# synnada-ai/datafusion-upstream

Hardware: AMD Instinct MI355X
Metric: rows/sec hash-join+agg, TPC-H SF100 Q3 (higher is better)
Workload: dtype int64; 1 GPU; TPC-H SF100 Q3 (3-way hash join + group-by SUM + sort), int64 keys, Decimal128(15,2) money, resident in HBM; input_rows=765043119, parallelism=1 GPU

## Files before the change

datafusion-upstream_amd/capi.py:

```python
from __future__ import annotations

import ctypes as C
import os

_HERE = os.path.dirname(os.path.abspath(__file__))
LIB_PATH = os.path.join(_HERE, "libdfgpu.so")

BOOL, INT8, INT16, INT32, INT64, UINT8, UINT16, UINT32, UINT64 = 1, 2, 3, 4, 5, 6, 7, 8, 9
FLOAT32, FLOAT64, DATE32, DECIMAL128, UTF8, DICTIONARY = 10, 11, 12, 13, 14, 15
OP_ADD, OP_SUB, OP_MUL, OP_DIV, OP_REM = 0, 1, 2, 3, 4
OP_EQ, OP_NEQ, OP_LT, OP_LTEQ, OP_GT, OP_GTEQ, OP_DISTINCT, OP_NOT_DISTINCT = 10, 11, 12, 13, 14, 15, 16, 17
OP_AND, OP_OR = 20, 21
JOIN_INNER, JOIN_LEFT, JOIN_RIGHT, JOIN_FULL, JOIN_LEFT_SEMI, JOIN_RIGHT_SEMI, JOIN_LEFT_ANTI, JOIN_RIGHT_ANTI = range(8)
AGG_SUM, AGG_AVG, AGG_COUNT, AGG_MIN, AGG_MAX = range(5)

STATUS_NAMES = {0: "Ok", 1: "Execution", 2: "Internal", 3: "ResourcesExhausted", 4: "NotImplemented", 5: "InvalidArgument"}


class DfgpuError(RuntimeError):

    def __init__(self, status: int, message: str):
        self.status = status
        self.kind = STATUS_NAMES.get(status, str(status))
        super().__init__(f"{self.kind} error: {message}")
# ... 67 lines not shown
    "dfgpu_array_import_arrow": (C.c_int32, [_P, C.POINTER(ArrowArray), C.POINTER(ArrowSchema), _PP]),
    "dfgpu_array_export_arrow": (C.c_int32, [_P, _P, C.POINTER(ArrowArray), C.POINTER(ArrowSchema)]),
    "dfgpu_array_retain": (None, [_P]),
    "dfgpu_array_release": (None, [_P]),
    "dfgpu_array_is_identity": (C.c_int32, [_P]),
    "dfgpu_array_length": (C.c_int64, [_P]),
    "dfgpu_array_null_count": (C.c_int64, [_P, _P]),
    "dfgpu_array_slice": (C.c_int32, [_P, _P, C.c_int64, C.c_int64, _PP]),
    "dfgpu_concat": (C.c_int32, [_P, _PP, C.c_int32, _PP]),
    "dfgpu_list_from_counts": (C.c_int32, [_P, _P, _P, _PP]),
    "dfgpu_list_flatten": (C.c_int32, [_P, _P, C.c_int32, C.c_int32, C.c_int32, _PP, _PP]),
    "dfgpu_array_new_null": (C.c_int32, [_P, C.c_int32, C.c_int32, C.c_int32, C.c_int64, _PP]),
    "dfgpu_array_new_zeros": (C.c_int32, [_P, C.c_int32, C.c_int32, C.c_int32, C.c_int64, _PP]),
    "dfgpu_array_make_dictionary": (C.c_int32, [_P, _P, _P, _PP]),
    "dfgpu_hash_columns": (C.c_int32, [_P, _PP, C.c_int32, C.c_uint64, _PP]),
    "dfgpu_take": (C.c_int32, [_P, _P, _P, _PP]),
    "dfgpu_filter": (C.c_int32, [_P, _P, _P, _PP]),
    "dfgpu_mask_to_indices": (C.c_int32, [_P, _P, _PP]),
    "dfgpu_binary": (C.c_int32, [_P, C.c_int32, _P, C.c_int32, _P, C.c_int32, _PP]),
    "dfgpu_binary_fused2": (C.c_int32, [_P, C.c_int32, _P, C.c_int32, _P, _P, C.c_int32, C.c_int32, _PP]),
    "dfgpu_not": (C.c_int32, [_P, _P, _PP]),
    "dfgpu_is_null": (C.c_int32, [_P, _P, C.c_int32, _PP]),
    "dfgpu_negative": (C.c_int32, [_P, _P, _PP]),
    "dfgpu_cast": (C.c_int32, [_P, _P, C.c_int32, C.c_int32, C.c_int32, _PP]),
    "dfgpu_in_list": (C.c_int32, [_P, _P, _P, C.c_int32, _PP]),
    "dfgpu_join_build": (C.c_int32, [_P, _PP, C.c_int32, _P, C.c_int32, _PP]),
    "dfgpu_join_table_free": (None, [_P]),
    "dfgpu_join_table_num_rows": (C.c_int64, [_P]),
    "dfgpu_join_table_memory": (C.c_int64, [_P]),
    "dfgpu_join_probe": (C.c_int32, [_P, _P, _PP, C.c_int32, _P, _PP, _PP]),
    "dfgpu_join_probe_deferred": (C.c_int32, [_P, _P, _PP, C.c_int32, _P, _PP, _PP]),
    "dfgpu_join_lookup": (C.c_int32, [_P, _P, _PP, C.c_int32, _P, _PP]),
    "dfgpu_join_probe_selection": (C.c_int32, [_P, _P, _PP, C.c_int32, _P, _PP]),
    "dfgpu_join_mark_visited": (C.c_int32, [_P, _P, _P]),
    "dfgpu_join_adjust_indices": (C.c_int32, [_P, _P, _P, C.c_int64, C.c_int64, C.c_int32, _PP, _PP]),
    "dfgpu_join_final_indices": (C.c_int32, [_P, _P, C.c_int32, _PP]),
    "dfgpu_groups_new": (C.c_int32, [_P, C.c_int32, _PP]),
    "dfgpu_groups_free": (None, [_P]),
    "dfgpu_groups_intern": (C.c_int32, [_P, _P, _PP, C.c_int32, _P, _PP]),
    "dfgpu_groups_intern_deferred": (C.c_int32, [_P, _P, _PP, C.c_int32, _P, _PP]),
    "dfgpu_groups_len": (C.c_int64, [_P]),
    "dfgpu_groups_size": (C.c_int64, [_P]),
    "dfgpu_groups_emit": (C.c_int32, [_P, _P, _PP]),
    "dfgpu_groups_emit_deferred": (C.c_int32, [_P, _P, _PP, _PP]),
    "dfgpu_acc_new": (C.c_int32, [_P, C.c_int32, C.c_int32, C.c_int32, C.c_int32, _PP]),
    "dfgpu_acc_free": (None, [_P]),
    "dfgpu_acc_update_batch": (C.c_int32, [_P, _P, _P, _P, _P, C.c_int64]),
    "dfgpu_acc_update_batch_multi": (C.c_int32, [_P, _PP, _PP, _PP, C.c_int32, _P, C.c_int64]),
    "dfgpu_acc_merge_batch": (C.c_int32, [_P, _P, _PP, C.c_int32, _P, _P, C.c_int64]),
    "dfgpu_acc_evaluate": (C.c_int32, [_P, _P, _PP]),
    "dfgpu_acc_state": (C.c_int32, [_P, _P, _PP, C.POINTER(C.c_int32)]),
    "dfgpu_acc_size": (C.c_int64, [_P]),
    "dfgpu_acc_emit_first": (C.c_int32, [_P, _P, C.c_int64, C.c_int32, _PP, C.POINTER(C.c_int32)]),
    "dfgpu_groups_emit_first": (C.c_int32, [_P, _P, C.c_int64, _PP]),
    "dfgpu_array_iota": (C.c_int32, [_P, C.c_int64, _PP]),
    "dfgpu_cross_join_indices": (C.c_int32, [_P, C.c_int64, C.c_int64, C.c_int64, C.c_int32, _PP, _PP]),
    "dfgpu_sort_to_indices": (C.c_int32, [_P, _PP, C.c_char_p, C.c_char_p, C.c_int32, C.c_int64, _PP]),
    "dfgpu_sort_to_indices_keys": (C.c_int32, [_P, _PP, C.c_char_p, C.c_char_p, C.c_int32, C.c_int64, _PP, _PP]),
    "dfgpu_hash_partition": (C.c_int32, [_P, _PP, C.c_int32, C.c_int32, _PP, C.POINTER(C.c_int64)]),
    "dfgpu_comm_unique_id": (C.c_int32, [C.c_char_p]),
    "dfgpu_comm_create_rccl": (C.c_int32, [_P, C.c_char_p, C.c_int32, C.c_int32, _PP]),
    "dfgpu_comm_create_custom": (C.c_int32, [_P, _PP]),
    "dfgpu_comm_free": (None, [_P]),
    "dfgpu_comm_rank": (C.c_int32, [_P]),
    "dfgpu_comm_world": (C.c_int32, [_P]),
    "dfgpu_exchange": (C.c_int32, [_P, _P, _PP, C.c_int32, _PP, C.c_int32, _P, _PP, C.POINTER(C.c_int64)]),
# ... 95 lines not shown
```

datafusion-upstream_amd/csrc/core.hip:

```cpp
#include "device_utils.h"
#include <mutex>

namespace dfgpu {

void fail(dfgpu_status code, const char* fmt, ...) {
  char buf[1024]; va_list ap; va_start(ap, fmt); vsnprintf(buf, sizeof buf, fmt, ap); va_end(ap);
  throw Error(code, buf);
}

struct CtxRefs { std::atomic<int64_t> n{1}; };
static std::mutex g_mu;
static std::vector<std::pair<dfgpu_ctx*, CtxRefs*>> g_ctx;
static CtxRefs* refs_of(dfgpu_ctx* c) { std::lock_guard<std::mutex> l(g_mu); for (auto& p : g_ctx) if (p.first == c) return p.second; return nullptr; }
static void ctx_unref(dfgpu_ctx* c) {
  CtxRefs* r = refs_of(c);
  if (!r || r->n.fetch_sub(1) != 1) return;
  { std::lock_guard<std::mutex> l(g_mu); for (size_t i = 0; i < g_ctx.size(); i++) if (g_ctx[i].first == c) { g_ctx.erase(g_ctx.begin() + i); break; } }
  (void)hipSetDevice(c->device);
  (void)hipStreamSynchronize(c->stream);
  if (c->free_blocks) { for (auto& b : *c->free_blocks) (void)hipFree(b.second); delete c->free_blocks; }
  delete c->alloc_mu;
  if (c->d_flags) (void)hipFree(c->d_flags);
  if (c->d_scratch64) (void)hipFree(c->d_scratch64);
  if (c->h_pinned) (void)hipHostFree(c->h_pinned);
// ... 316 lines not shown
}
__global__ void __launch_bounds__(BLOCK) k_slist_walk(const int32_t* loff, const uint8_t* lbytes, int64_t n, const uint32_t* vstart, uint32_t* cnt, uint32_t* lens, uint32_t* spos, uint32_t* row_of, uint32_t* flags) {
  const int64_t i = (int64_t)blockIdx.x * BLOCK + threadIdx.x; if (i >= n) return;
  int64_t at = loff[i]; const int64_t end = loff[i + 1]; uint32_t k = 0;
  while (at < end) {
    if (at + 4 > end) { atomicOr(flags, DFGPU_FLAG_OOB); break; }
    const uint32_t len = (uint32_t)lbytes[at] | ((uint32_t)lbytes[at + 1] << 8) | ((uint32_t)lbytes[at + 2] << 16) | ((uint32_t)lbytes[at + 3] << 24);
    if (at + 4 + (int64_t)len > end) { atomicOr(flags, DFGPU_FLAG_OOB); break; }
    if (lens) { const uint32_t v = vstart[i] + k; lens[v] = len; spos[v] = (uint32_t)(at + 4); row_of[v] = (uint32_t)i; }
    k++; at += 4 + (int64_t)len;
  }
  if (cnt) cnt[i] = k;
}
__global__ void __launch_bounds__(BLOCK) k_slist_copy(const uint8_t* lbytes, const uint32_t* spos, const int32_t* voff, int64_t nv, uint8_t* out) {
  const int64_t j = (int64_t)blockIdx.x * BLOCK + threadIdx.x; if (j >= nv) return;
  const uint32_t len = (uint32_t)(voff[j + 1] - voff[j]); const uint8_t* src = lbytes + spos[j]; uint8_t* o = out + voff[j];
  for (uint32_t b = 0; b < len; b++) o[b] = src[b];
}

struct CtxOption { const char* name; int64_t (*get)(const dfgpu_ctx*); void (*set)(dfgpu_ctx*, int64_t); };
#define OPT_GET(M) [](const dfgpu_ctx* c) -> int64_t { return (int64_t)c->M; }
#define OPT_BOOL(M) OPT_GET(M), [](dfgpu_ctx* c, int64_t v) { c->M = v != 0; }
#define OPT_INT(M) OPT_GET(M), [](dfgpu_ctx* c, int64_t v) { c->M = v; }
#define OPT_MIN(M, LO) OPT_GET(M), [](dfgpu_ctx* c, int64_t v) { c->M = v < LO ? LO : v; }
#define OPT_RANGE(M, LO, HI) OPT_GET(M), [](dfgpu_ctx* c, int64_t v) { if (v < LO || v > HI) fail(DFGPU_INVALID_ARGUMENT, #M ": " #LO " .. " #HI); c->M = v; }
#define OPT_READ(M) OPT_GET(M), nullptr
static const CtxOption kCtxOptions[] = {
  { "force_hash_collisions", OPT_BOOL(force_hash_collisions) },
  { "first_seen_group_order", OPT_BOOL(first_seen_group_order) },
  { "join_rank_index", OPT_BOOL(join_rank_index) },
  { "join_rank_index_unsorted", OPT_BOOL(join_rank_index_unsorted) },
  { "join_lazy_build_rows", OPT_BOOL(join_lazy_build_rows) },
  { "join_selection_output", OPT_BOOL(join_selection_output) },
  { "join_key_packing", OPT_BOOL(join_key_packing) },
  { "join_swap_small_semi", OPT_BOOL(join_swap_small_semi) },
  { "join_partitioned", OPT_BOOL(join_partitioned) },
  { "join_partitioned_min_build", OPT_INT(join_partitioned_min_build) },
  { "join_partitioned_min_probe", OPT_INT(join_partitioned_min_probe) },
  { "join_partitioned_big", OPT_BOOL(join_partitioned_big) },
  { "join_partitioned_hashed", OPT_BOOL(join_partitioned_hashed) },
  { "join_partitioned_hash_mask", [](const dfgpu_ctx* c) -> int64_t { return c->join_partitioned_hash_mask == ~0ull ? 0 : (int64_t)c->join_partitioned_hash_mask; },
                                  [](dfgpu_ctx* c, int64_t v) { c->join_partitioned_hash_mask = v <= 0 ? ~0ull : (uint64_t)v; } },
  { "join_partition_rows", OPT_INT(join_partition_rows) },
  { "group_run_detection", OPT_BOOL(group_run_detection) },
  { "group_lazy_keys", OPT_BOOL(group_lazy_keys) },
  { "group_dictionary_canon", OPT_BOOL(group_dictionary_canon) },
  { "fused_aggregate_min_rows", OPT_INT(fused_aggregate_min_rows) },
  { "agg_order_inverse_map", OPT_BOOL(agg_order_inverse_map) },
  { "agg_partitioned", OPT_BOOL(agg_partitioned) },
  { "agg_partitioned_force", OPT_BOOL(agg_partitioned_force) },
  { "agg_partitioned_min_rows", OPT_INT(agg_partitioned_min_rows) },
  { "agg_pack_estimate_min_rows", OPT_INT(agg_pack_estimate_min_rows) },
  { "agg_preaggregate_distinct", OPT_READ(pa_last_distinct) },
  { "agg_spill_state_bytes", OPT_INT(agg_spill_state_bytes) },
  { "agg_spill_ranges", OPT_RANGE(agg_spill_ranges, 1, 4096) },
  { "sort_packed_keys", OPT_BOOL(sort_packed_keys) },
  { "sort_packed_min_rows", OPT_MIN(sort_packed_min_rows, 2) },
  { "sort_estimate_ranges", OPT_BOOL(sort_estimate_ranges) },
  { "sort_topk_words_min_rows", OPT_MIN(sort_topk_words_min_rows, 2) },
  { "sort_one_block_max_rows", OPT_MIN(sort_one_block_max_rows, 0) },
  { "sort_onesweep_min_rows", OPT_MIN(sort_onesweep_min_rows, 2) },
  { "sort_onesweep_rows", OPT_GET(sort_onesweep_rows), [](dfgpu_ctx* c, int64_t v) { c->sort_onesweep_rows = v == 16 ? 16 : v > 0 ? 8 : 0; } },
  { "sort_onesweep_fused_finish", OPT_BOOL(sort_onesweep_fused_finish) },
  { "sort_fused_small_passes", OPT_BOOL(sort_fused_small_passes) },
  { "sort_spill_bytes", OPT_INT(sort_spill_bytes) },
  { "sort_spill_ranges", OPT_RANGE(sort_spill_ranges, 1, 4096) },
// ... 423 lines not shown
```

datafusion-upstream_amd/csrc/dfgpu_internal.h:

```cpp
#pragma once
#include <hip/hip_runtime.h>
#include <atomic>
#include <cstdarg>
#include <cstdint>
#include <cstdio>
#include <cstring>
#include <memory>
#include <mutex>
#include <stdexcept>
#include <string>
#include <vector>
#include "../../include/dfgpu.h"

namespace dfgpu {

struct Error : std::exception {
  dfgpu_status code; std::string msg;
  Error(dfgpu_status c, std::string m) : code(c), msg(std::move(m)) {}
  const char* what() const noexcept override { return msg.c_str(); }
};
[[noreturn]] void fail(dfgpu_status code, const char* fmt, ...);

#define HIP_CHECK(expr)                                                                         \
  do { hipError_t e_ = (expr);                                                                  \
    if (e_ != hipSuccess) ::dfgpu::fail(e_ == hipErrorOutOfMemory ? DFGPU_RESOURCES_EXHAUSTED : DFGPU_INTERNAL, \
                                        "%s failed: %s (%s:%d)", #expr, hipGetErrorString(e_), __FILE__, __LINE__); } while (0)
#define KERNEL_CHECK() HIP_CHECK(hipGetLastError())

}

enum : uint32_t { DFGPU_FLAG_DIV_ZERO = 1, DFGPU_FLAG_OVERFLOW = 2, DFGPU_FLAG_CAST = 4, DFGPU_FLAG_OOB = 8, DFGPU_FLAG_TABLE_FULL = 16, DFGPU_FLAG_STALLED = 32 };

namespace dfgpu { struct Buffer; }
struct dfgpu_ctx {
  int device = 0;
  hipStream_t stream = nullptr;
  bool own_stream = false;
  hipStream_t copy_stream = nullptr;
  std::string err;
  bool force_hash_collisions = false;
  bool first_seen_group_order = true;
  bool join_rank_index = true;
  bool join_lazy_build_rows = true;
  bool join_selection_output = true;
  bool join_rank_index_unsorted = true;
  bool join_key_packing = true;
  bool group_run_detection = true;
  bool group_lazy_keys = true;
  bool group_dictionary_canon = true;
  bool join_swap_small_semi = true;
  uint64_t join_partitioned_hash_mask = ~0ull;
  bool join_partitioned_hashed = true;
  bool join_partitioned_big = true;
  bool join_partitioned = true; int64_t join_partitioned_min_build = 1 << 20, join_partitioned_min_probe = 1 << 22, join_partition_rows = 14000;
  int64_t fused_aggregate_min_rows = 1 << 20;
  bool sort_packed_keys = true;
  bool agg_partitioned = true, agg_partitioned_force = false; int64_t agg_partitioned_min_rows = 1 << 22;
  bool agg_order_inverse_map = true;
  int64_t agg_pack_estimate_min_rows = 1 << 22;
  bool pa_last_distinct = false;
  const void* pa_sample_key = nullptr; const void* pa_sample_mask = nullptr; int64_t pa_sample_n = 0; uint64_t pa_sample[3] = {0, 0, 0};
  std::shared_ptr<dfgpu::Buffer> pa_pack; int pa_pack_n = 0; int64_t pa_pack_min[4] = {0, 0, 0, 0}; uint64_t pa_pack_stride[4] = {0, 0, 0, 0}, pa_pack_range[4] = {0, 0, 0, 0}; bool pa_pack_nullable[4] = {false, false, false, false};
  std::shared_ptr<dfgpu::Buffer> row_selection; int64_t row_selection_len = 0;
  int defer_flag_checks = 0; bool flags_pending = false; std::string flags_what;
  uint32_t* d_flags = nullptr;
  uint64_t* d_scratch64 = nullptr;
  uint64_t* h_pinned = nullptr;
  static constexpr int MAIL_SEQ = 384, MAIL_WORDS = 256, PINNED_WORDS = 512;
  bool mailbox_readback = true; uint64_t mail_seq = 0;
  int num_cus = 256;
  std::mutex* alloc_mu = nullptr;
  std::vector<std::pair<size_t, void*>>* free_blocks = nullptr;
  size_t cached_bytes = 0, live_bytes = 0;
  int64_t sort_packed_min_rows = 1 << 20;
  int64_t sort_topk_words_min_rows = 1 << 23;
  int64_t sort_one_block_max_rows = 8192;
  int64_t sort_onesweep_min_rows = 1 << 20;
// ... 164 lines not shown
```

datafusion-upstream_amd/csrc/exec/exec.cpp:

```cpp
#include "../../../include/dfgpu_exec.h"

#include <algorithm>
#include <cstdarg>
#include <cstdio>
#include <cstring>
#include <memory>
#include <mutex>
#include <atomic>
#include <deque>
#include <map>
#include <tuple>
#include <set>
#include <stdexcept>
#include <string>
#include <vector>

namespace dfx {

struct Err : std::exception {
  dfgpu_status code; std::string msg;
  Err(dfgpu_status c, std::string m) : code(c), msg(std::move(m)) {}
  const char* what() const noexcept override { return msg.c_str(); }
};
[[noreturn]] static void fail(dfgpu_status code, const char* fmt, ...) {
// ... 52 lines not shown
  }
};
struct Col {
  ArrayRef arr, source; std::vector<ArrayRef> chain; MemoPtr memo; std::shared_ptr<LazyLookup> lookup;
  int64_t len() const { return arr ? arr.len() : !chain.empty() ? chain.back().len() : lookup ? lookup->m : 0; }
};
static const ArrayRef& col_indices(const TaskContext& tc, Col& c) {
  while (c.chain.size() > 1) {
    ArrayRef outer = std::move(c.chain.back()); c.chain.pop_back();
    ArrayRef& inner = c.chain.back();
    if (c.memo) {
      auto key = std::make_pair((const dfgpu_array*)inner.a, (const dfgpu_array*)outer.a);
      auto it = c.memo->composed.find(key);
      if (it == c.memo->composed.end()) it = c.memo->composed.emplace(key, Composed{inner, outer, take(tc, inner, outer)}).first;
      inner = it->second.out;
    } else inner = take(tc, inner, outer);
  }
  if (c.lookup) { ArrayRef b = c.lookup->resolve(tc, c.chain.empty() ? ArrayRef() : c.chain[0]); c.chain.clear(); c.chain.push_back(b); c.lookup.reset(); }
  return c.chain[0];
}
static const ArrayRef& col_get(const TaskContext& tc, Col& c) {
  if (!c.arr) { c.arr = take(tc, c.source, col_indices(tc, c)); c.source = ArrayRef(); c.chain.clear(); c.memo.reset(); }
  return c.arr;
}
static Col col_take(const Col& c, const ArrayRef& idx, const MemoPtr& memo = nullptr) {
  if (dfgpu_array_is_identity(idx.a) && idx.len() == c.len()) return c;
  Col o; o.memo = memo;
  if (c.arr) { o.source = c.arr; o.chain.push_back(idx); return o; }
  o.source = c.source; o.chain = c.chain; o.lookup = c.lookup; o.chain.push_back(idx);
  return o;
}
static Col col_of(ArrayRef a) { Col c; c.arr = std::move(a); return c; }

struct Batch {
  SchemaPtr schema; std::vector<Col> cols; ArrayRef selection; int64_t base_rows = 0;
  const ArrayRef& column(const TaskContext& tc, int i) {
    Col& c = cols.at((size_t)i);
    if (!c.arr && c.source && !c.chain.empty() && base_rows <= ((int64_t)1 << 20) && base_rows > 0) {
      std::vector<size_t> sib;
      for (size_t k = 0; k < cols.size(); k++) { const Col& o = cols[k]; if (k == (size_t)i || o.arr || !o.source || o.lookup.get() != c.lookup.get() || o.chain.size() != c.chain.size()) continue;
        bool same = true; for (size_t q = 0; q < c.chain.size(); q++) same = same && o.chain[q].a == c.chain[q].a; if (same) sib.push_back(k); }
      if (!sib.empty()) {
        const ArrayRef idx = col_indices(tc, c);
        std::vector<const dfgpu_array*> vals{ c.source.a }; for (size_t k : sib) vals.push_back(cols[k].source.a);
        std::vector<dfgpu_array*> outs(vals.size(), nullptr);
        tc.check(dfgpu_take_multi(tc.ctx, vals.data(), (int32_t)vals.size(), idx.a, outs.data()));
        auto settle = [](Col& x, dfgpu_array* a) { x.arr = ArrayRef::adopt(a); x.source = ArrayRef(); x.chain.clear(); x.memo.reset(); x.lookup.reset(); };
        settle(c, outs[0]); for (size_t u = 0; u < sib.size(); u++) settle(cols[sib[u]], outs[u + 1]);
        return c.arr;
      }
    }
    return col_get(tc, c);
  }
};
static ArrayRef mask_indices(const TaskContext& tc, const ArrayRef& mask) { dfgpu_array* o = nullptr; tc.check(dfgpu_mask_to_indices(tc.ctx, mask.a, &o)); return ArrayRef::adopt(o); }
static Batch materialize(const TaskContext& tc, const Batch& b) {
  if (!b.selection) return b;
  ArrayRef sel = mask_indices(tc, b.selection);
  Batch o; o.schema = b.schema; o.base_rows = sel.len();
  MemoPtr memo = std::make_shared<TakeMemo>(); for (auto& c : b.cols) o.cols.push_back(col_take(c, sel, memo));
  return o;
}
static int64_t num_rows(const TaskContext& tc, const Batch& b) { return b.selection ? mask_indices(tc, b.selection).len() : b.base_rows; }
static ArrayRef concat_arrays(const TaskContext& tc, std::vector<ArrayRef>& parts) {
  std::vector<const dfgpu_array*> p; for (auto& x : parts) p.push_back(x.a);
  dfgpu_array* o = nullptr; tc.check(dfgpu_concat(tc.ctx, p.data(), (int32_t)p.size(), &o)); return ArrayRef::adopt(o);
}
static bool concat_batches(const TaskContext& tc, std::vector<Batch>& in, Batch* out) {
  std::vector<Batch> m;
  for (auto& b : in) { Batch x = materialize(tc, b); if (x.base_rows > 0) m.push_back(std::move(x)); }
  if (m.empty()) { if (in.empty()) return false; *out = materialize(tc, in[0]); return true; }
  if (m.size() == 1) { *out = std::move(m[0]); return true; }
  Batch o; o.schema = m[0].schema;
  for (size_t c = 0; c < m[0].cols.size(); c++) {
    std::vector<ArrayRef> parts; for (auto& b : m) parts.push_back(col_get(tc, b.cols[c]));
    o.cols.push_back(col_of(concat_arrays(tc, parts)));
  }
  for (auto& b : m) o.base_rows += b.base_rows;
  *out = std::move(o); return true;
}

struct Value { ArrayRef arr; bool scalar = false; };
struct Expr {
  virtual ~Expr() = default;
  virtual Value eval(const TaskContext& tc, Batch& b) const = 0;
  virtual bool safe() const { return false; }
  virtual void columns(std::set<int>& out) const {}
  virtual int column_index() const { return -1; }
};
using ExprPtr = std::shared_ptr<const Expr>;

static ArrayRef into_array(const TaskContext& tc, const Value& v, int64_t n) {
  if (!v.scalar) return v.arr;
  dfgpu_array* idx = nullptr; tc.check(dfgpu_array_new_zeros(tc.ctx, DFGPU_UINT32, 0, 0, n, &idx));
  ArrayRef i = ArrayRef::adopt(idx);
  return take(tc, v.arr, i);
// ... 70 lines not shown
};

struct Stream { virtual ~Stream() = default; virtual bool next(Batch& out) = 0; };
struct Plan;
using PlanPtr = std::shared_ptr<const Plan>;
struct Metrics {
  std::mutex mu; int64_t output_rows = 0, output_batches = 0;
  int64_t spill_count = 0, spilled_bytes = 0, spilled_rows = 0;
  struct Open { dfgpu_ctx* c; int64_t id; int which; };
  std::vector<Open> open; int64_t ns[4] = {0, 0, 0, 0};
  void resolve() {
    std::lock_guard<std::mutex> l(mu);
    for (auto& o : open) { int64_t t = 0; if (dfgpu_span_elapsed_ns(o.c, o.id, &t) == DFGPU_OK) ns[o.which] += t; }
    open.clear();
  }
  ~Metrics() { resolve(); }
};
struct SpanGuard {
  dfgpu_ctx* c = nullptr; int64_t id = -1; Metrics* m = nullptr; int which = 0;
  SpanGuard(const TaskContext& tc, Metrics* met, int w) { if (tc.metrics && met && dfgpu_span_begin(tc.ctx, &id) == DFGPU_OK) { c = tc.ctx; m = met; which = w; } else id = -1; }
  ~SpanGuard() { if (id >= 0) { dfgpu_span_end(c, id); std::lock_guard<std::mutex> l(m->mu); m->open.push_back(Metrics::Open{c, id, which}); } }
};
struct Plan : std::enable_shared_from_this<Plan> {
  virtual ~Plan() = default;
  mutable std::shared_ptr<Metrics> met = std::make_shared<Metrics>();
  virtual std::vector<std::shared_ptr<const Plan>> children() const { return {}; }
  std::unique_ptr<Stream> run(int partition, const TaskContext& tc) const;
  virtual const char* name() const = 0;
  virtual SchemaPtr schema() const = 0;
  virtual int partitions() const = 0;
  virtual std::unique_ptr<Stream> execute(int partition, const TaskContext& tc) const = 0;
  virtual PlanPtr fresh() const = 0;
};
static int64_t metric_rows(const TaskContext& tc, const Batch& b) { if (!b.selection) return b.base_rows; int64_t k = 0; tc.check(dfgpu_mask_count(tc.ctx, b.selection.a, &k)); return k; }
struct MeteredStream : Stream {
  const Plan* op; PlanPtr keep; std::unique_ptr<Stream> in; TaskContext tc;
  MeteredStream(PlanPtr k, std::unique_ptr<Stream> i, TaskContext t) : op(k.get()), keep(std::move(k)), in(std::move(i)), tc(t) {}
  bool next(Batch& out) override {
    bool ok; { SpanGuard sp(tc, op->met.get(), 0); ok = in->next(out); }
    if (ok) { int64_t r = metric_rows(tc, out); std::lock_guard<std::mutex> l(op->met->mu); op->met->output_rows += r; op->met->output_batches++; }
    return ok;
  }
};
std::unique_ptr<Stream> Plan::run(int partition, const TaskContext& tc) const {
  if (!tc.metrics) return execute(partition, tc);
  std::unique_ptr<Stream> s; { SpanGuard sp(tc, met.get(), 0); s = execute(partition, tc); }
  return std::unique_ptr<Stream>(new MeteredStream(shared_from_this(), std::move(s), tc));
}
static void drain(const PlanPtr& p, int partition, const TaskContext& tc, std::vector<Batch>& out) {
  auto s = p->run(partition, tc); Batch b; while (s->next(b)) out.push_back(std::move(b));
}

struct VecStream : Stream {
  std::vector<Batch> v; size_t i = 0;
  explicit VecStream(std::vector<Batch> x) : v(std::move(x)) {}
  bool next(Batch& out) override { if (i >= v.size()) return false; out = std::move(v[i++]); return true; }
};

struct MemoryExec : Plan {
  mutable std::mutex mu; mutable std::vector<std::vector<Batch>> parts; SchemaPtr sch;
  const char* name() const override { return "MemoryExec"; }
  PlanPtr fresh() const override { return shared_from_this(); }
  SchemaPtr schema() const override { return sch; }
  int partitions() const override { std::lock_guard<std::mutex> l(mu); return (int)parts.size(); }
  std::unique_ptr<Stream> execute(int p, const TaskContext&) const override {
    std::lock_guard<std::mutex> l(mu);
    if (p < 0 || p >= (int)parts.size()) fail(DFGPU_INTERNAL, "MemoryExec invalid partition %d (expected less than %zu)", p, parts.size());
// ... 47 lines not shown
    for (int64_t i = 0; i < len; i++) { const uint8_t c = bytes[i]; if (escape > 0 && c == (uint8_t)escape && inside && i + 1 < len) { i++; continue; } if (c == (uint8_t)quote) inside = !inside; else if (c == '\n' && !inside && i + 1 >= next && i + 1 < len) { cuts.push_back(i + 1); next = i + 1 + batch_bytes; } }
    cuts.push_back(len);
  }
  struct S : Stream {
    const CsvExec* op; TaskContext tc; int next_piece, end_piece;
    S(const CsvExec* o, TaskContext t, int a, int b) : op(o), tc(t), next_piece(a), end_piece(b) {}
    bool next(Batch& out) override {
      if (next_piece >= end_piece) return false;
      const int i = next_piece++; std::vector<dfgpu_array*> cols(op->proj.size(), nullptr); int64_t rows = 0;
      tc.check(dfgpu_csv_read(tc.ctx, op->bytes + op->cuts[(size_t)i], op->cuts[(size_t)i + 1] - op->cuts[(size_t)i], 0, op->delim, op->quote, op->escape, i == 0 && op->header ? 1 : 0, op->ncols_file,
                              op->proj.data(), op->types.data(), (int32_t)op->proj.size(), cols.data(), &rows));
      Batch b; b.schema = op->sch; b.base_rows = rows;
      for (auto* a : cols) b.cols.push_back(col_of(ArrayRef::adopt(a)));
      out = std::move(b); return true;
    }
  };
  std::unique_ptr<Stream> execute(int p, const TaskContext& tc) const override {
    if (p < 0 || p >= nparts) fail(DFGPU_INTERNAL, "CsvExec invalid partition %d (expected less than %d)", p, nparts);
    const int64_t P = (int64_t)cuts.size() - 1;
    return std::unique_ptr<Stream>(new S(this, tc, (int)(P * p / nparts), (int)(P * (p + 1) / nparts)));
  }
};

static ArrayRef known_mask(const TaskContext& tc, const ArrayRef& m) {
  dfgpu_array_desc d; dfgpu_array_describe(m.a, &d);
  if (!d.validity) return m;
  dfgpu_array *nn = nullptr, *o = nullptr;
  tc.check(dfgpu_is_null(tc.ctx, m.a, 1, &nn)); ArrayRef n1 = ArrayRef::adopt(nn);
  tc.check(dfgpu_binary(tc.ctx, DFGPU_OP_AND, m.a, 0, n1.a, 0, &o)); return ArrayRef::adopt(o);
}

struct FilterExec : Plan {
  ExprPtr pred; PlanPtr input;
  PlanPtr fresh() const override { auto f = std::make_shared<FilterExec>(); f->pred = pred; f->input = input->fresh(); return f; }
  std::vector<std::shared_ptr<const Plan>> children() const override { return {input}; }
  const char* name() const override { return "FilterExec"; }
  SchemaPtr schema() const override { return input->schema(); }
  int partitions() const override { return input->partitions(); }
  struct S : Stream {
    const FilterExec* op; std::unique_ptr<Stream> in; TaskContext tc;
    S(const FilterExec* o, std::unique_ptr<Stream> i, TaskContext t) : op(o), in(std::move(i)), tc(t) {}
    bool next(Batch& out) override {
      Batch b; if (!in->next(b)) return false;
      if (b.selection && !op->pred->safe()) b = materialize(tc, b);
      Value v = op->pred->eval(tc, b);
      ArrayRef mask = into_array(tc, v, b.base_rows);
      dfgpu_array_desc d; dfgpu_array_describe(mask.a, &d);
      if (d.type != DFGPU_BOOL) fail(DFGPU_INTERNAL, "Cannot create filter_array from non-boolean predicates");
      if (b.selection) { ArrayRef km = known_mask(tc, mask); dfgpu_array* o = nullptr; tc.check(dfgpu_binary(tc.ctx, DFGPU_OP_AND, km.a, 0, b.selection.a, 0, &o)); mask = ArrayRef::adopt(o); }
      b.selection = mask; out = std::move(b); return true;
    }
  };
  std::unique_ptr<Stream> execute(int p, const TaskContext& tc) const override { return std::unique_ptr<Stream>(new S(this, input->run(p, tc), tc)); }
};

static Batch materialize_subset(const TaskContext& tc, Batch& b, const std::set<int>& needed) {
  ArrayRef sel = mask_indices(tc, b.selection);
  Batch o; o.schema = b.schema; o.base_rows = sel.len();
  ArrayRef filler; MemoPtr memo = std::make_shared<TakeMemo>();
  for (size_t i = 0; i < b.cols.size(); i++) {
    if (needed.count((int)i)) o.cols.push_back(col_take(b.cols[i], sel, memo));
    else { if (!filler) { dfgpu_array* f = nullptr; tc.check(dfgpu_array_new_null(tc.ctx, DFGPU_INT8, 0, 0, o.base_rows, &f)); filler = ArrayRef::adopt(f); } o.cols.push_back(col_of(filler)); }
  }
  return o;
}

struct ProjectionExec : Plan {
  std::vector<ExprPtr> exprs; std::vector<std::string> names; PlanPtr input; mutable SchemaPtr sch; mutable std::mutex mu;
  PlanPtr fresh() const override { auto p = std::make_shared<ProjectionExec>(); p->exprs = exprs; p->names = names; p->input = input->fresh(); return p; }
  std::vector<std::shared_ptr<const Plan>> children() const override { return {input}; }
  const char* name() const override { return "ProjectionExec"; }
  SchemaPtr schema() const override {
    std::lock_guard<std::mutex> l(mu);
    if (!sch) { auto s = std::make_shared<Schema>(); auto in = input->schema();
      for (size_t i = 0; i < exprs.size(); i++) { int ci = exprs[i]->column_index(); Field f = (ci >= 0 && in && ci < (int)in->f.size()) ? in->f[(size_t)ci] : Field{}; f.name = names[i]; s->f.push_back(f); }
      sch = s; }
    return sch;
  }
  int partitions() const override { return input->partitions(); }
  struct RowSel { dfgpu_ctx* c = nullptr; ~RowSel() { if (c) dfgpu_ctx_set_row_selection(c, nullptr); } };
  bool only_columns() const { bool oc = true; for (auto& e : exprs) oc &= e->column_index() >= 0; return oc; }
  Batch project(const TaskContext& tc, Batch b, std::vector<bool>* defer = nullptr) const {
    RowSel rowsel;
    if (b.selection && !only_columns() && !defer) {
      int64_t kept = 0; tc.check(dfgpu_mask_count(tc.ctx, b.selection.a, &kept));
      if (kept * 4 >= b.base_rows) { tc.check(dfgpu_ctx_set_row_selection(tc.ctx, b.selection.a)); rowsel.c = tc.ctx; }
      else { std::set<int> need; for (auto& e : exprs) e->columns(need); b = materialize_subset(tc, b, need); if (defer) defer->assign(exprs.size(), false); defer = nullptr; }
    }
    Batch o; o.base_rows = b.base_rows; o.selection = b.selection; auto s = std::make_shared<Schema>();
    if (defer) defer->assign(exprs.size(), false);
    for (size_t i = 0; i < exprs.size(); i++) {
      int ci = exprs[i]->column_index();
      if (ci >= 0) {
        if (ci >= (int)b.cols.size()) fail(DFGPU_INTERNAL, "PhysicalExpr Column references column at index %d but input schema only has %zu columns", ci, b.cols.size());
        o.cols.push_back(b.cols[(size_t)ci]); Field f = b.schema->f[(size_t)ci]; f.name = names[i]; s->f.push_back(f);
      } else if (defer) { (*defer)[i] = true; o.cols.push_back(Col()); s->f.push_back(Field{names[i]}); }
      else { ArrayRef a = into_array(tc, exprs[i]->eval(tc, b), b.base_rows); s->f.push_back(field_of(names[i], a.a)); o.cols.push_back(col_of(a)); }
    }
    o.schema = s; if (!defer) { std::lock_guard<std::mutex> l(mu); sch = s; }
    return o;
  }
  void evaluate_deferred(const TaskContext& tc, Batch& raw, Batch& projected, size_t i) const {
    RowSel rowsel;
    if (raw.selection) { tc.check(dfgpu_ctx_set_row_selection(tc.ctx, raw.selection.a)); rowsel.c = tc.ctx; }
    ArrayRef a = into_array(tc, exprs[i]->eval(tc, raw), raw.base_rows);
    projected.schema->f[i] = field_of(names[i], a.a); projected.cols[i] = col_of(a);
  }
  struct S : Stream {
    const ProjectionExec* op; std::unique_ptr<Stream> in; TaskContext tc;
    S(const ProjectionExec* o, std::unique_ptr<Stream> i, TaskContext t) : op(o), in(std::move(i)), tc(t) {}
    bool next(Batch& out) override {
      Batch b; if (!in->next(b)) return false;
      out = op->project(tc, std::move(b)); return true;
    }
  };
  std::unique_ptr<Stream> execute(int p, const TaskContext& tc) const override { return std::unique_ptr<Stream>(new S(this, input->run(p, tc), tc)); }
};

struct CoalesceBatchesExec : Plan {
  PlanPtr input; int64_t target;
  PlanPtr fresh() const override { auto c = std::make_shared<CoalesceBatchesExec>(); c->input = input->fresh(); c->target = target; return c; }
  std::vector<std::shared_ptr<const Plan>> children() const override { return {input}; }
  const char* name() const override { return "CoalesceBatchesExec"; }
  SchemaPtr schema() const override { return input->schema(); }
  int partitions() const override { return input->partitions(); }
  struct S : Stream {
    const CoalesceBatchesExec* op; std::unique_ptr<Stream> in; TaskContext tc; std::vector<Batch> buf; int64_t rows = 0; bool done = false;
    S(const CoalesceBatchesExec* o, std::unique_ptr<Stream> i, TaskContext t) : op(o), in(std::move(i)), tc(t) {}
    bool flush(Batch& out) { bool ok = concat_batches(tc, buf, &out); buf.clear(); rows = 0; return ok; }
    bool next(Batch& out) override {
      while (!done) {
        Batch b; if (!in->next(b)) { done = true; break; }
        if (b.selection) { if (b.base_rows >= op->target) { out = std::move(b); return true; } b = materialize(tc, b); }
        if (b.base_rows == 0) continue;
        if (b.base_rows >= op->target && buf.empty()) { out = std::move(b); return true; }
        rows += b.base_rows; buf.push_back(std::move(b));
        if (rows >= op->target) return flush(out);
      }
      if (!buf.empty()) return flush(out);
      return false;
    }
  };
  std::unique_ptr<Stream> execute(int p, const TaskContext& tc) const override { return std::unique_ptr<Stream>(new S(this, input->run(p, tc), tc)); }
};

struct CoalescePartitionsExec : Plan {
  PlanPtr input;
  PlanPtr fresh() const override { auto c = std::make_shared<CoalescePartitionsExec>(); c->input = input->fresh(); return c; }
  std::vector<std::shared_ptr<const Plan>> children() const override { return {input}; }
  const char* name() const override { return "CoalescePartitionsExec"; }
  SchemaPtr schema() const override { return input->schema(); }
  int partitions() const override { return 1; }
  std::unique_ptr<Stream> execute(int, const TaskContext& tc) const override {
    std::vector<Batch> all; for (int p = 0; p < input->partitions(); p++) drain(input, p, tc, all);
    return std::unique_ptr<Stream>(new VecStream(std::move(all)));
  }
};

static void partition_batch(const TaskContext& tc, Batch& b, const std::vector<ExprPtr>& exprs, int n, std::vector<std::vector<Batch>>& outs) {
  if (b.base_rows == 0) return;
  bool safe_keys = true; for (auto& e : exprs) safe_keys &= e->safe();
  if (n <= 256 && (!b.selection || safe_keys)) {
    Batch kb = b; kb.selection = ArrayRef();
    std::vector<ArrayRef> keys; std::vector<const dfgpu_array*> kp;
    for (auto& e : exprs) { keys.push_back(into_array(tc, e->eval(tc, kb), kb.base_rows)); kp.push_back(keys.back().a); }
    std::vector<const dfgpu_array*> cp; for (auto& c : b.cols) cp.push_back(c.arr ? c.arr.a : nullptr);
    std::vector<dfgpu_array*> oc(b.cols.size(), nullptr); std::vector<int64_t> counts((size_t)n); dfgpu_array* idx = nullptr;
    tc.check(dfgpu_partition_columns(tc.ctx, kp.data(), (int32_t)kp.size(), n, cp.data(), (int32_t)cp.size(), b.selection.a, oc.data(), &idx, counts.data()));
    ArrayRef indices = ArrayRef::adopt(idx); std::vector<ArrayRef> moved; for (auto* x : oc) moved.push_back(ArrayRef::adopt(x));
    int64_t off = 0;
    for (int d = 0; d < n; d++) {
      const int64_t cnt = counts[(size_t)d];
      if (cnt) {
        auto slice = [&](const ArrayRef& a) { dfgpu_array* s = nullptr; tc.check(dfgpu_array_slice(tc.ctx, a.a, off, cnt, &s)); return ArrayRef::adopt(s); };
        ArrayRef rows;
        Batch o; o.schema = b.schema; o.base_rows = cnt; MemoPtr memo = std::make_shared<TakeMemo>();
        for (size_t c = 0; c < b.cols.size(); c++) {
          if (moved[c]) o.cols.push_back(col_of(slice(moved[c])));
          else { if (!rows) rows = slice(indices); o.cols.push_back(col_take(b.cols[c], rows, memo)); }
        }
        outs[(size_t)d].push_back(std::move(o));
      }
      off += cnt;
    }
    return;
  }
  ArrayRef sel; Batch kb = b;
  if (b.selection) { std::set<int> need; for (auto& e : exprs) e->columns(need); sel = mask_indices(tc, b.selection); kb = materialize_subset(tc, b, need); }
  if (kb.base_rows == 0) return;
  std::vector<ArrayRef> keys; std::vector<const dfgpu_array*> kp;
  for (auto& e : exprs) { keys.push_back(into_array(tc, e->eval(tc, kb), kb.base_rows)); kp.push_back(keys.back().a); }
  std::vector<int64_t> counts((size_t)n); dfgpu_array* idx = nullptr;
  tc.check(dfgpu_hash_partition(tc.ctx, kp.data(), (int32_t)kp.size(), n, &idx, counts.data()));
  ArrayRef indices = ArrayRef::adopt(idx); int64_t off = 0;
  for (int d = 0; d < n; d++) {
    if (counts[(size_t)d]) {
      dfgpu_array* s = nullptr; tc.check(dfgpu_array_slice(tc.ctx, indices.a, off, counts[(size_t)d], &s)); ArrayRef part = ArrayRef::adopt(s);
      ArrayRef rows = sel ? take(tc, sel, part) : part;
      Batch o; o.schema = b.schema; o.base_rows = counts[(size_t)d];
      MemoPtr memo = std::make_shared<TakeMemo>(); for (auto& c : b.cols) o.cols.push_back(col_take(c, rows, memo));
      outs[(size_t)d].push_back(std::move(o));
    }
    off += counts[(size_t)d];
  }
}

struct RepartitionExec : Plan {
  PlanPtr input; std::vector<ExprPtr> exprs; int n;
  mutable std::mutex mu; mutable bool ran = false; mutable std::vector<std::vector<Batch>> outs;
  PlanPtr fresh() const override { auto r = std::make_shared<RepartitionExec>(); r->input = input->fresh(); r->exprs = exprs; r->n = n; return r; }
  std::vector<std::shared_ptr<const Plan>> children() const override { return {input}; }
  const char* name() const override { return "RepartitionExec"; }
  SchemaPtr schema() const override { return input->schema(); }
  int partitions() const override { return n; }
  std::unique_ptr<Stream> execute(int p, const TaskContext& tc) const override {
    std::lock_guard<std::mutex> l(mu);
    if (!ran) {
      outs.assign((size_t)n, {});
      for (int ip = 0; ip < input->partitions(); ip++) {
        std::vector<Batch> in; drain(input, ip, tc, in);
        int rr = 0;
// ... 7 lines not shown
    if (p < 0 || p >= n) fail(DFGPU_INTERNAL, "RepartitionExec invalid partition %d", p);
    return std::unique_ptr<Stream>(new VecStream(outs[(size_t)p]));
  }
};

struct JoinTableRef { dfgpu_join_table* t = nullptr; ~JoinTableRef() { if (t) dfgpu_join_table_free(t); } };
struct BuildSide { Batch batch; std::shared_ptr<JoinTableRef> table; std::vector<int64_t> segments; bool empty = true; };

struct HashJoinExec : Plan {
  PlanPtr left, right; std::vector<ExprPtr> on_l, on_r; ExprPtr filter; std::vector<int> f_side, f_index;
  int join_type, mode; bool null_equals_null; bool swap_small_right = true;
  mutable bool selection_consumer = false;
  mutable std::mutex mu; mutable std::shared_ptr<BuildSide> shared;
  PlanPtr fresh() const override {
    auto j = std::make_shared<HashJoinExec>(); j->left = left->fresh(); j->right = right->fresh(); j->on_l = on_l; j->on_r = on_r; j->filter = filter; j->f_side = f_side; j->f_index = f_index;
    j->join_type = join_type; j->mode = mode; j->null_equals_null = null_equals_null; j->swap_small_right = swap_small_right; j->selection_consumer = selection_consumer; return j;
  }
  std::vector<std::shared_ptr<const Plan>> children() const override { return {left, right}; }
  const char* name() const override { return "HashJoinExec"; }
  bool swap_allowed(const TaskContext& tc) const { int64_t v = 1; dfgpu_ctx_get_option(tc.ctx, "join_swap_small_semi", &v); return swap_small_right && v != 0; }
  bool left_only() const { return join_type == DFGPU_JOIN_LEFT_SEMI || join_type == DFGPU_JOIN_LEFT_ANTI; }
  bool right_only() const { return join_type == DFGPU_JOIN_RIGHT_SEMI || join_type == DFGPU_JOIN_RIGHT_ANTI; }
  SchemaPtr schema() const override {
    auto s = std::make_shared<Schema>(); auto l = left->schema(), r = right->schema();
    if (!right_only() && l) s->f.insert(s->f.end(), l->f.begin(), l->f.end());
    if (!left_only() && r) s->f.insert(s->f.end(), r->f.begin(), r->f.end());
    return s;
  }
  int partitions() const override { return right->partitions(); }
  std::shared_ptr<BuildSide> collect_left(int partition, const TaskContext& tc, ArrayRef* fused) const {
    auto bs = std::make_shared<BuildSide>();
    std::vector<Batch> in;
    if (partition < 0) { for (int p = 0; p < left->partitions(); p++) drain(left, p, tc, in); } else drain(left, partition, tc, in);
    if (in.size() == 1 && in[0].selection) { bs->batch = in[0]; *fused = in[0].selection; bs->batch.selection = ArrayRef(); bs->segments = { bs->batch.base_rows }; bs->empty = false; }
    else {
      std::vector<Batch> m; for (auto& b : in) { Batch x = materialize(tc, b); if (x.base_rows) { bs->segments.push_back(x.base_rows); m.push_back(std::move(x)); } }
      if (m.empty()) return bs;
      concat_batches(tc, m, &bs->batch); bs->empty = false;
    }
    return bs;
  }
  void build_table(const std::shared_ptr<BuildSide>& bs, const ArrayRef& fused, const TaskContext& tc) const {
    if (bs->empty) return;
    std::vector<ArrayRef> keys; std::vector<const dfgpu_array*> kp;
    for (auto& e : on_l) { keys.push_back(into_array(tc, e->eval(tc, bs->batch), bs->batch.base_rows)); kp.push_back(keys.back().a); }
    bs->table = std::make_shared<JoinTableRef>();
    tc.check(dfgpu_join_build(tc.ctx, kp.data(), (int32_t)kp.size(), fused.a, null_equals_null ? 1 : 0, &bs->table->t));
  }
  std::shared_ptr<BuildSide> collect_build(int partition, const TaskContext& tc) const {
    SpanGuard sp(tc, met.get(), 1);
    ArrayRef fused; auto bs = collect_left(partition, tc, &fused); build_table(bs, fused, tc); return bs;
  }
  struct S : Stream {
    const HashJoinExec* op; TaskContext tc; int partition; std::unique_ptr<Stream> probe; std::shared_ptr<BuildSide> bs; Batch swapped; int state = 0;
    Batch chunk_pb; ArrayRef chunk_b, chunk_p; int64_t chunk_k = -1, chunk_total = 0, chunk_joined = -1; std::vector<uint32_t> chunk_last;
    SchemaPtr out_schema;
    bool lazy_build_rows = true, selection_output = true;
    S(const HashJoinExec* o, int p, TaskContext t) : op(o), tc(t), partition(p) { int64_t v = 1; if (dfgpu_ctx_get_option(tc.ctx, "join_lazy_build_rows", &v) == DFGPU_OK) lazy_build_rows = v != 0;
      v = 1; if (dfgpu_ctx_get_option(tc.ctx, "join_selection_output", &v) == DFGPU_OK) selection_output = v != 0; }
    int64_t last_u32(const ArrayRef& a) {
      int64_t n = a.len(); if (!n) return -1;
      dfgpu_array* s1 = nullptr; tc.check(dfgpu_array_slice(tc.ctx, a.a, n - 1, 1, &s1)); ArrayRef one = ArrayRef::adopt(s1);
      uint32_t v = 0; tc.check(dfgpu_array_export_host(tc.ctx, one.a, &v, nullptr, nullptr)); return (int64_t)v;
    }
    void chunk_last_rows(const ArrayRef& pidx, int64_t bsz) {
      const int64_t m = pidx.len(); chunk_last.clear(); if (!m) return;
      std::vector<uint32_t> pos; for (int64_t e = bsz; ; e += bsz) { pos.push_back((uint32_t)((e < m ? e : m) - 1)); if (e >= m) break; }
// ... 54 lines not shown
      if (!op->right_only()) for (size_t i = 0; i < (lf ? lf->f.size() : 0); i++) {
        if (build && alias[i] >= 0) o.cols.push_back(col_take(probe_b.cols[(size_t)alias[i]], pidx, memo));
        else if (build && lazy) { Col c; c.source = build->cols[i].arr; c.lookup = lazy; c.memo = memo; o.cols.push_back(std::move(c)); }
        else if (build) o.cols.push_back(col_take(build->cols[i], bidx, memo));
        else { dfgpu_array* nn = nullptr; tc.check(dfgpu_array_new_null(tc.ctx, lf->f[i].type, lf->f[i].precision, lf->f[i].scale, o.base_rows, &nn)); o.cols.push_back(col_of(ArrayRef::adopt(nn))); }
      }
      if (!op->left_only()) for (auto& c : probe_b.cols) o.cols.push_back(col_take(c, pidx, memo));
      return o;
    }
    bool next(Batch& out) override {
      if (state == 0) {
        if (op->left_only() && op->swap_allowed(tc) && (op->mode != 0 || op->right->partitions() == 1)) {
          ArrayRef fused; bs = op->collect_left(op->mode == 0 ? -1 : partition, tc, &fused);
          std::vector<Batch> rin; drain(op->right, partition, tc, rin);
          Batch rb; bool have_right = concat_batches(tc, rin, &rb) && rb.base_rows > 0;
          out_schema = op->schema();
          if (!bs->empty && rb.base_rows * 8 <= bs->batch.base_rows) { swapped = semi_by_probing_left(fused, have_right ? &rb : nullptr); state = 4; }
          else { op->build_table(bs, fused, tc); std::vector<Batch> one; if (have_right) one.push_back(std::move(rb)); probe.reset(new VecStream(std::move(one))); state = 1; }
        }
        else if (op->mode == 0) { std::lock_guard<std::mutex> l(op->mu); if (!op->shared) op->shared = op->collect_build(-1, tc); bs = op->shared; }
        else bs = op->collect_build(partition, tc);
        if (state == 0) { probe = op->right->run(partition, tc); out_schema = op->schema(); state = 1; }
      }
      if (state == 4) { state = 3; if (swapped.base_rows == 0) return false; out = std::move(swapped); return true; }
      bool need_final = op->join_type == DFGPU_JOIN_LEFT || op->join_type == DFGPU_JOIN_FULL || op->left_only();
      if (need_final && op->mode == 0 && op->right->partitions() > 1 && state != 4)
        fail(DFGPU_NOT_IMPLEMENTED, "HashJoinExec mode=CollectLeft with %d probe partitions and a join type that emits build rows in a final pass; repartition both sides (Partitioned) or coalesce the probe side", op->right->partitions());
      while (state == 1) {
        if (chunk_k >= 0) { SpanGuard join_span(tc, op->met.get(), 2); emit_chunk(out, need_final); return true; }
        Batch pb; if (!probe->next(pb)) { state = 2; break; }
        if (pb.base_rows == 0) continue;
        SpanGuard join_span(tc, op->met.get(), 2);
        const bool chunked = pb.base_rows <= (tc.batch_size > 8192 ? tc.batch_size : 8192);
        if (chunked && pb.selection) { pb = materialize(tc, pb); if (pb.base_rows == 0) continue; }
        if (pb.selection && (op->join_type == DFGPU_JOIN_RIGHT || op->join_type == DFGPU_JOIN_FULL || op->right_only())) { pb = materialize(tc, pb); if (pb.base_rows == 0) continue; }
        ArrayRef mask = pb.selection; pb.selection = ArrayRef();
        ArrayRef bidx, pidx;
        if (bs->empty) { dfgpu_array *a = nullptr, *b = nullptr; dfgpu_array_desc d{}; d.type = DFGPU_UINT64; d.values = &d; tc.check(dfgpu_array_import_host(tc.ctx, &d, &a)); d.type = DFGPU_UINT32; tc.check(dfgpu_array_import_host(tc.ctx, &d, &b)); bidx = ArrayRef::adopt(a); pidx = ArrayRef::adopt(b); }
        else {
          std::vector<ArrayRef> keys; std::vector<const dfgpu_array*> kp;
          for (auto& e : op->on_r) { keys.push_back(into_array(tc, e->eval(tc, pb), pb.base_rows)); kp.push_back(keys.back().a); }
          dfgpu_array *b = nullptr, *p = nullptr;
          bool defer = !chunked && op->join_type == DFGPU_JOIN_INNER && !op->filter && !need_final && kp.size() == 1 && lazy_build_rows;
          if (defer && selection_output && op->selection_consumer) {
            std::vector<int> al = key_aliases(&bs->batch, pb); bool all = !al.empty(); for (int a : al) all = all && a >= 0;
            if (all) {
              dfgpu_array* s = nullptr; dfgpu_status st = dfgpu_join_probe_selection(tc.ctx, bs->table->t, kp.data(), 1, mask.a, &s);
              if (st == DFGPU_OK) {
                Batch o; o.schema = out_schema; o.base_rows = pb.base_rows; o.selection = ArrayRef::adopt(s);
                for (int a : al) o.cols.push_back(pb.cols[(size_t)a]);
                for (auto& c : pb.cols) o.cols.push_back(c);
                out = std::move(o); return true;
              }
              if (st != DFGPU_NOT_IMPLEMENTED) tc.check(st);
            }
          }
          for (auto& c : bs->batch.cols) defer = defer && (bool)c.arr;
          if (defer) {
            tc.check(dfgpu_join_probe_deferred(tc.ctx, bs->table->t, kp.data(), 1, mask.a, &b, &p)); pidx = ArrayRef::adopt(p);
            if (!b) {
              auto lz = std::make_shared<LazyLookup>(); lz->keep = bs; lz->table = bs->table->t; lz->probe_key = keys[0]; lz->rows = pidx; lz->m = pidx.len();
              bool wanted = false; { std::vector<int> al = key_aliases(&bs->batch, pb); for (int a : al) wanted |= a < 0; }
              if (!wanted || (dfgpu_array_is_identity(pidx.a) && pidx.len() == pb.base_rows)) { out = build_batch(&bs->batch, pb, ArrayRef(), pidx, lz); return true; }
              bidx = lz->resolve(tc, ArrayRef());
            } else bidx = ArrayRef::adopt(b);
          } else { tc.check(dfgpu_join_probe(tc.ctx, bs->table->t, kp.data(), (int32_t)kp.size(), mask.a, &b, &p)); bidx = ArrayRef::adopt(b); pidx = ArrayRef::adopt(p); }
          if (!chunked) { apply_filter(pb, bidx, pidx); if (need_final) tc.check(dfgpu_join_mark_visited(tc.ctx, bs->table->t, bidx.a)); }
        }
        if (chunked) {
          const int64_t bsz = tc.batch_size > 0 ? tc.batch_size : 8192, m = bidx.len();
          chunk_total = m == 0 ? 1 : (m + bsz - 1) / bsz;
          chunk_last_rows(pidx, bsz);
          if (m > 0 && m % bsz == 0 && (int64_t)chunk_last.back() != pb.base_rows - 1) chunk_total++;
          chunk_pb = std::move(pb); chunk_b = bidx; chunk_p = pidx; chunk_k = 0; chunk_joined = -1;
          continue;
        }
        int jt = op->join_type;
        if (jt == DFGPU_JOIN_RIGHT || jt == DFGPU_JOIN_FULL || op->right_only()) {
          dfgpu_array *b2 = nullptr, *p2 = nullptr;
          tc.check(dfgpu_join_adjust_indices(tc.ctx, bidx.a, pidx.a, 0, pb.base_rows, jt, &b2, &p2)); bidx = ArrayRef::adopt(b2); pidx = ArrayRef::adopt(p2);
        } else if (op->left_only()) continue;
        out = build_batch(bs->empty ? nullptr : &bs->batch, pb, bidx, pidx); return true;
      }
      if (state == 2) {
        state = 3;
        if (!need_final || bs->empty) return false;
        dfgpu_array* f = nullptr; tc.check(dfgpu_join_final_indices(tc.ctx, bs->table->t, op->join_type, &f)); ArrayRef fidx = ArrayRef::adopt(f);
        fidx = reference_final_order(fidx);
        Batch o; o.schema = out_schema; o.base_rows = fidx.len();
        MemoPtr memo = std::make_shared<TakeMemo>(); for (auto& c : bs->batch.cols) o.cols.push_back(col_take(c, fidx, memo));
        if (!op->left_only()) { auto rf = op->right->schema(); for (auto& fd : rf->f) { dfgpu_array* nn = nullptr; tc.check(dfgpu_array_new_null(tc.ctx, fd.type, fd.precision, fd.scale, o.base_rows, &nn)); o.cols.push_back(col_of(ArrayRef::adopt(nn))); } }
        out = std::move(o); return true;
      }
      return false;
    }
    Batch semi_by_probing_left(ArrayRef fused, Batch* right_rows) {
      Batch o; o.schema = out_schema;
      const bool have_right = right_rows != nullptr; Batch none; Batch& rb = have_right ? *right_rows : none;
      Batch& lb = bs->batch;
      const bool anti = op->join_type == DFGPU_JOIN_LEFT_ANTI;
      if (anti && fused) {
        Batch sel = lb; sel.selection = fused; lb = materialize(tc, sel); fused = ArrayRef(); bs->segments = { lb.base_rows };
      }
      ArrayRef lidx;
      if (!have_right) {
        if (!anti) return o;
        dfgpu_array *e0 = nullptr, *e1 = nullptr; dfgpu_array_desc d{}; d.type = DFGPU_UINT64; d.values = &d; tc.check(dfgpu_array_import_host(tc.ctx, &d, &e0)); ArrayRef b0 = ArrayRef::adopt(e0);
        d.type = DFGPU_UINT32; tc.check(dfgpu_array_import_host(tc.ctx, &d, &e1)); ArrayRef p0 = ArrayRef::adopt(e1);
        dfgpu_array *b2 = nullptr, *p2 = nullptr; tc.check(dfgpu_join_adjust_indices(tc.ctx, b0.a, p0.a, 0, lb.base_rows, DFGPU_JOIN_RIGHT_ANTI, &b2, &p2)); ArrayRef drop = ArrayRef::adopt(b2); lidx = ArrayRef::adopt(p2);
      } else {
        std::vector<ArrayRef> rk, lk; std::vector<const dfgpu_array*> rp, lp;
        for (auto& e : op->on_r) { rk.push_back(into_array(tc, e->eval(tc, rb), rb.base_rows)); rp.push_back(rk.back().a); }
        JoinTableRef table; tc.check(dfgpu_join_build(tc.ctx, rp.data(), (int32_t)rp.size(), nullptr, op->null_equals_null ? 1 : 0, &table.t));
        for (auto& e : op->on_l) { lk.push_back(into_array(tc, e->eval(tc, lb), lb.base_rows)); lp.push_back(lk.back().a); }
        dfgpu_array *b = nullptr, *p = nullptr;
        tc.check(dfgpu_join_probe(tc.ctx, table.t, lp.data(), (int32_t)lp.size(), fused.a, &b, &p)); ArrayRef ridx = ArrayRef::adopt(b); lidx = ArrayRef::adopt(p);
        if (op->filter && ridx.len()) {
          Batch inter; inter.schema = std::make_shared<Schema>(); inter.base_rows = ridx.len();
          for (size_t i = 0; i < op->f_side.size(); i++) {
            Col src = op->f_side[i] == 0 ? lb.cols.at((size_t)op->f_index[i]) : rb.cols.at((size_t)op->f_index[i]);
            Col t = col_take(src, op->f_side[i] == 0 ? lidx : ridx); inter.cols.push_back(col_of(col_get(tc, t))); inter.schema->f.push_back(Field{"x"});
          }
          ArrayRef m = into_array(tc, op->filter->eval(tc, inter), inter.base_rows);
          ArrayRef nr = filter_idx(ridx, m), nl = filter_idx(lidx, m); ridx = nr; lidx = nl;
        }
        dfgpu_array *b2 = nullptr, *p2 = nullptr;
        tc.check(dfgpu_join_adjust_indices(tc.ctx, ridx.a, lidx.a, 0, lb.base_rows, anti ? DFGPU_JOIN_RIGHT_ANTI : DFGPU_JOIN_RIGHT_SEMI, &b2, &p2));
        ArrayRef drop = ArrayRef::adopt(b2); lidx = ArrayRef::adopt(p2);
      }
      if (bs->segments.size() > 1 && lidx.len()) {
        dfgpu_array* w = nullptr; tc.check(dfgpu_cast(tc.ctx, lidx.a, DFGPU_UINT64, 0, 0, &w)); lidx = reference_final_order(ArrayRef::adopt(w));
      }
      o.base_rows = lidx.len();
      MemoPtr memo = std::make_shared<TakeMemo>(); for (auto& c : lb.cols) o.cols.push_back(col_take(c, lidx, memo));
      return o;
// ... 505 lines not shown
      if (aggs[i].kind == DFGPU_AGG_COUNT_DISTINCT) { cds[i].init(tc); continue; }
      int32_t t = aggs[i].kind == DFGPU_AGG_COUNT ? DFGPU_INT64 : aggs[i].type;
      tc.check(dfgpu_acc_new(tc.ctx, aggs[i].kind, t, aggs[i].precision, aggs[i].scale, &accs[i].a));
    }
    { int64_t lim = 0, ranges = 16; dfgpu_ctx_get_option(tc.ctx, "agg_spill_state_bytes", &lim); dfgpu_ctx_get_option(tc.ctx, "agg_spill_ranges", &ranges);
      if (lim > 0 && grouped && !specials && sets.empty()) { S.spill = std::make_shared<SpillState>(); S.spill->limit = lim; S.spill->ranges = ranges; } }
    if (order_mode != 0) preagg_min_rows = INT64_MAX;
    S.pj = pj; S.src = src; S.grouped = grouped; S.specials = specials; S.fuse_min_rows = fuse_min_rows; S.preagg_min_rows = preagg_min_rows;
    return SP;
  }
  void consume(AggState& S, Batch& b_in) const {
    const TaskContext& tc = S.tc; const ProjectionExec* pj = S.pj; const bool grouped = S.grouped, specials = S.specials; const int64_t fuse_min_rows = S.fuse_min_rows, preagg_min_rows = S.preagg_min_rows;
    GroupsRef& groups = S.groups; std::vector<AccRef>& accs = S.accs; std::vector<StringMinMax>& smm = S.smm; std::vector<CountDistinct>& cds = S.cds; ArrayRef& pending = S.pending;
    auto settle_pending = [&]() {
      if (!pending) return;
      const dfgpu_array* kp = pending.a; dfgpu_array* ids = nullptr; tc.check(dfgpu_groups_intern(tc.ctx, groups.g, &kp, 1, nullptr, &ids)); ArrayRef drop = ArrayRef::adopt(ids);
      if (dfgpu_groups_len(groups.g) != pending.len()) fail(DFGPU_INTERNAL, "AggregateExec: pre-aggregated keys were not distinct");
      pending = ArrayRef();
    };
    {
      if (b_in.base_rows == 0) return;
      if (S.spill && order_mode == 0 && mode != 0 && !pending && dfgpu_groups_len(groups.g) > 0 && state_bytes(S) > S.spill->limit) spill(S, *S.spill);
      settle_pending();
      Batch raw; std::vector<bool> deferred;
      if (pj) { raw = b_in; b_in = pj->project(tc, raw, &deferred); }
      Batch& b = b_in;
      bool any_deferred = false; for (bool d : deferred) any_deferred |= d;
      auto ensure = [&](int ci) { if (ci >= 0 && ci < (int)deferred.size() && deferred[(size_t)ci]) { pj->evaluate_deferred(tc, raw, b, (size_t)ci); deferred[(size_t)ci] = false; } };
      if (any_deferred) {
        std::set<int> need; for (auto& e : gexprs) e->columns(need); for (auto& a : aggs) if (a.filter) a.filter->columns(need);
        for (int ci : need) ensure(ci);
      }
      if (b.base_rows == 0) return;
      ArrayRef mask = b.selection; b.selection = ArrayRef();
      if (!sets.empty()) { if (specials) fail(DFGPU_NOT_IMPLEMENTED, "This feature is not implemented: COUNT(DISTINCT) / string MIN-MAX under grouping sets on the device"); for (size_t ci = 0; ci < deferred.size(); ci++) ensure((int)ci); group_aggregate_sets(tc, b, mask, groups, accs); return; }
      ArrayRef gids; int64_t total = 1;
      if (grouped) {
        std::vector<ArrayRef> gc; std::vector<const dfgpu_array*> gp;
        for (auto& e : gexprs) {
          int ci = e->column_index();
          if (ci >= 0 && ci < (int)b.cols.size() && !b.cols[(size_t)ci].arr && b.cols[(size_t)ci].source && b.cols[(size_t)ci].source.len() * 4 <= b.base_rows) {
            Col& c = b.cols[(size_t)ci]; dfgpu_array_desc sd; dfgpu_array_describe(c.source.a, &sd);
            if (sd.type != DFGPU_DICTIONARY) {
              dfgpu_array* d = nullptr; tc.check(dfgpu_array_make_dictionary(tc.ctx, col_indices(tc, c).a, c.source.a, &d));
              gc.push_back(ArrayRef::adopt(d)); gp.push_back(gc.back().a); continue;
            }
          }
          gc.push_back(into_array(tc, e->eval(tc, b), b.base_rows)); gp.push_back(gc.back().a);
        }
        if (!specials && !merging() && gp.size() >= 1 && gp.size() <= 4 && b.base_rows >= preagg_min_rows && preaggregate(tc, pj, raw, b, deferred, ensure, gp, mask, groups, accs, S.spill ? nullptr : &pending)) return;
        dfgpu_array* ids = nullptr; tc.check(specials || order_mode == 1 ? dfgpu_groups_intern(tc.ctx, groups.g, gp.data(), (int32_t)gp.size(), mask.a, &ids) : dfgpu_groups_intern_deferred(tc.ctx, groups.g, gp.data(), (int32_t)gp.size(), mask.a, &ids)); gids = ArrayRef::adopt(ids);
        total = dfgpu_groups_len(groups.g);
        if (order_mode == 1 && !specials) note_sort_prefix(S, gp, gids, mask);
      } else { dfgpu_array* z = nullptr; tc.check(dfgpu_array_new_zeros(tc.ctx, DFGPU_UINT32, 0, 0, b.base_rows, &z)); gids = ArrayRef::adopt(z); }
      if (!specials && !merging() && total <= 8 && fuse_min_rows >= 0 && b.base_rows >= fuse_min_rows && try_fused(tc, pj, raw, b, deferred, accs, gids, grouped ? ArrayRef() : mask, total)) return;
      for (size_t ci = 0; ci < deferred.size(); ci++) ensure((int)ci);
      size_t col = gexprs.size();
      std::vector<ArrayRef> uvals(aggs.size()), ufilt(aggs.size());
      for (size_t i = 0; i < aggs.size(); i++) {
        if (merging() && is_string_minmax(i)) {
          ArrayRef stv = b.column(tc, (int)col); col += 1;
          smm[i].update(tc, gids, stv, mask);
        } else if (merging() && aggs[i].kind == DFGPU_AGG_COUNT_DISTINCT) {
          ArrayRef stv = b.column(tc, (int)col); col += 1;
          cds[i].merge(tc, gids, stv, mask, total, aggs[i].type, aggs[i].precision, aggs[i].scale);
        } else if (merging()) {
          int nst = aggs[i].kind == DFGPU_AGG_AVG ? 2 : 1; const dfgpu_array* st[2];
// ... 436 lines not shown
struct dfgpu_stream { std::unique_ptr<Stream> s; PlanPtr keep; TaskContext tc; };

template <typename F> static dfgpu_status guard(F&& f) {
  try { f(); return DFGPU_OK; }
  catch (const Err& e) { g_err = e.msg; return e.code; }
  catch (const std::bad_alloc&) { g_err = "host allocation failed"; return DFGPU_RESOURCES_EXHAUSTED; }
  catch (const std::exception& e) { g_err = e.what(); return DFGPU_INTERNAL; }
}
static ExprPtr ex(const dfgpu_expr* e) { if (!e) fail(DFGPU_INVALID_ARGUMENT, "null expression"); return e->e; }
static PlanPtr pl(const dfgpu_plan* p) { if (!p) fail(DFGPU_INVALID_ARGUMENT, "null plan"); return p->p; }

extern "C" {

const char* dfgpu_exec_last_error(void) { return g_err.c_str(); }

dfgpu_status dfgpu_batch_new(const char* const* names, const dfgpu_array* const* columns, int32_t ncols, dfgpu_batch** out) {
  return guard([&] {
    if (ncols < 0 || !out) fail(DFGPU_INVALID_ARGUMENT, "batch_new: bad arguments");
    auto* b = new dfgpu_batch(); b->b.schema = std::make_shared<Schema>();
    for (int i = 0; i < ncols; i++) {
      if (!columns[i]) { delete b; fail(DFGPU_INVALID_ARGUMENT, "batch_new: null column"); }
      if (i && dfgpu_array_length(columns[i]) != dfgpu_array_length(columns[0])) { delete b; fail(DFGPU_INVALID_ARGUMENT, "batch_new: columns differ in length"); }
      b->b.cols.push_back(col_of(ArrayRef::share(columns[i]))); b->b.schema->f.push_back(field_of(names && names[i] ? names[i] : "", columns[i]));
    }
    b->b.base_rows = ncols ? dfgpu_array_length(columns[0]) : 0;
    *out = b;
  });
}
void dfgpu_batch_free(dfgpu_batch* b) { delete b; }
int32_t dfgpu_batch_num_columns(const dfgpu_batch* b) { return b ? (int32_t)b->b.cols.size() : 0; }
const char* dfgpu_batch_column_name(const dfgpu_batch* b, int32_t i) { return (b && i >= 0 && i < (int)b->b.schema->f.size()) ? b->b.schema->f[(size_t)i].name.c_str() : ""; }
dfgpu_status dfgpu_batch_num_rows(dfgpu_ctx* ctx, dfgpu_batch* b, int64_t* out) { return guard([&] { if (!ctx || !b || !out) fail(DFGPU_INVALID_ARGUMENT, "batch_num_rows: null argument"); TaskContext tc{ctx, 8192}; *out = num_rows(tc, b->b); }); }
static void materialize_all(const TaskContext& tc, Batch& b) {
  if (b.selection) b = materialize(tc, b);
  std::map<const dfgpu_array*, std::vector<size_t>> groups;
  for (size_t i = 0; i < b.cols.size(); i++) { Col& c = b.cols[i]; if (!c.arr && c.source && !c.chain.empty()) groups[col_indices(tc, c).a].push_back(i); }
  for (auto& g : groups) {
    if (g.second.size() < 2) continue;
    std::vector<const dfgpu_array*> vals; for (size_t i : g.second) vals.push_back(b.cols[i].source.a);
    std::vector<dfgpu_array*> outs(vals.size(), nullptr);
    ArrayRef idx = b.cols[g.second[0]].chain[0];
    tc.check(dfgpu_take_multi(tc.ctx, vals.data(), (int32_t)vals.size(), idx.a, outs.data()));
    for (size_t k = 0; k < g.second.size(); k++) { Col& c = b.cols[g.second[k]]; c.arr = ArrayRef::adopt(outs[k]); c.source = ArrayRef(); c.chain.clear(); c.memo.reset(); }
  }
  for (auto& c : b.cols) (void)col_get(tc, c);
}
dfgpu_status dfgpu_batch_materialize(dfgpu_ctx* ctx, dfgpu_batch* b) {
  return guard([&] { if (!ctx || !b) fail(DFGPU_INVALID_ARGUMENT, "batch_materialize: null argument"); TaskContext tc{ctx, 8192}; materialize_all(tc, b->b); });
}
dfgpu_status dfgpu_batch_column(dfgpu_ctx* ctx, dfgpu_batch* b, int32_t i, dfgpu_array** out) {
  return guard([&] {
    if (!ctx || !b || !out) fail(DFGPU_INVALID_ARGUMENT, "batch_column: null argument");
    TaskContext tc{ctx, 8192};
    if (b->b.selection) b->b = materialize(tc, b->b);
    const ArrayRef& a = b->b.column(tc, i); dfgpu_array_retain(a.a); *out = a.a;
  });
}

dfgpu_status dfgpu_expr_column(const char* name, int32_t index, dfgpu_expr** out) { return guard([&] { if (!out) fail(DFGPU_INVALID_ARGUMENT, "expr_column: null argument"); *out = new dfgpu_expr{std::make_shared<ColumnExpr>(name ? name : "", index)}; }); }
dfgpu_status dfgpu_expr_literal(const dfgpu_array* s, dfgpu_expr** out) {
  return guard([&] { if (!s || dfgpu_array_length(s) != 1) fail(DFGPU_INVALID_ARGUMENT, "literal must be a length-1 array"); *out = new dfgpu_expr{std::make_shared<LiteralExpr>(ArrayRef::share(s))}; });
}
dfgpu_status dfgpu_expr_binary(const dfgpu_expr* l, int32_t op, const dfgpu_expr* r, dfgpu_expr** out) { return guard([&] { *out = new dfgpu_expr{std::make_shared<BinaryExpr>(ex(l), op, ex(r))}; }); }
static dfgpu_status unary(const dfgpu_expr* e, int kind, int a0, int a1, int a2, const dfgpu_array* list, dfgpu_expr** out) {
  return guard([&] { auto u = std::make_shared<UnaryExpr>(); u->e = ex(e); u->kind = kind; u->a0 = a0; u->a1 = a1; u->a2 = a2; if (list) u->list = ArrayRef::share(list); *out = new dfgpu_expr{u}; });
}
dfgpu_status dfgpu_expr_not(const dfgpu_expr* e, dfgpu_expr** out) { return unary(e, 0, 0, 0, 0, nullptr, out); }
dfgpu_status dfgpu_expr_is_null(const dfgpu_expr* e, int32_t negated, dfgpu_expr** out) { return unary(e, negated ? 2 : 1, 0, 0, 0, nullptr, out); }
dfgpu_status dfgpu_expr_negative(const dfgpu_expr* e, dfgpu_expr** out) { return unary(e, 3, 0, 0, 0, nullptr, out); }
dfgpu_status dfgpu_expr_cast(const dfgpu_expr* e, int32_t t, int32_t p, int32_t s, dfgpu_expr** out) { return unary(e, 4, t, p, s, nullptr, out); }
dfgpu_status dfgpu_expr_in_list(const dfgpu_expr* e, const dfgpu_array* list, int32_t negated, dfgpu_expr** out) { return unary(e, negated ? 6 : 5, 0, 0, 0, list, out); }
void dfgpu_expr_free(dfgpu_expr* e) { delete e; }

dfgpu_status dfgpu_plan_memory(const dfgpu_batch* const* batches, const int32_t* sizes, int32_t nparts, dfgpu_plan** out) {
  return guard([&] {
    if (!out || nparts < 0 || (nparts > 0 && (!sizes || !batches))) fail(DFGPU_INVALID_ARGUMENT, "plan_memory: null argument");
    auto m = std::make_shared<MemoryExec>(); int k = 0;
    for (int p = 0; p < nparts; p++) { m->parts.emplace_back(); for (int i = 0; i < sizes[p]; i++) { const dfgpu_batch* b = batches[k++]; if (!b) fail(DFGPU_INVALID_ARGUMENT, "null batch"); if (!m->sch) m->sch = b->b.schema; m->parts.back().push_back(b->b); } }
    if (!m->sch) m->sch = std::make_shared<Schema>();
    *out = new dfgpu_plan{m};
  });
}
dfgpu_status dfgpu_plan_parquet(dfgpu_parquet* file, const int32_t* columns, int32_t ncols, int32_t npartitions, int32_t row_groups_per_batch, dfgpu_plan** out) {
  return guard([&] {
    if (!file || !out || (ncols > 0 && !columns) || npartitions < 1) fail(DFGPU_INVALID_ARGUMENT, "plan_parquet: bad argument");
    auto n = std::make_shared<ParquetExec>(); n->file = file; n->nparts = npartitions; n->per_batch = row_groups_per_batch > 0 ? row_groups_per_batch : 1; n->sch = std::make_shared<Schema>();
    for (int32_t i = 0; i < ncols; i++) {
// ... 14 lines not shown
    for (int32_t i = 0; i < ncols; i++) {
      const int32_t c = columns[i];
      if (c < 0 || c >= ncols_file || (i && c <= columns[i - 1])) fail(DFGPU_INVALID_ARGUMENT, "plan_csv: projected columns must be ascending file column indices");
      n->proj.push_back(c); n->types.insert(n->types.end(), {types[3 * c], types[3 * c + 1], types[3 * c + 2]});
      n->sch->f.push_back(Field{names[c] ? names[c] : "", types[3 * c], types[3 * c + 1], types[3 * c + 2]});
    }
    n->cut(batch_bytes > 0 ? batch_bytes : (int64_t)256 << 20);
    *out = new dfgpu_plan{n};
  });
}
dfgpu_status dfgpu_plan_parquet_prune(dfgpu_plan* p, int32_t column, int64_t min_value, int64_t max_value) {
  return guard([&] {
    auto* n = p ? dynamic_cast<const ParquetExec*>(p->p.get()) : nullptr;
    if (!n) fail(DFGPU_INVALID_ARGUMENT, "plan_parquet_prune: not a ParquetExec");
    std::lock_guard<std::mutex> l(n->mu); n->bounds.push_back(ParquetExec::Bound{column, min_value, max_value});
  });
}
int64_t dfgpu_plan_parquet_pruned(const dfgpu_plan* p) { auto* n = p ? dynamic_cast<const ParquetExec*>(p->p.get()) : nullptr; return n ? n->pruned.load() : -1; }
dfgpu_status dfgpu_plan_memory_replace(dfgpu_plan* p, const dfgpu_batch* const* batches, const int32_t* sizes, int32_t nparts) {
  return guard([&] {
    auto* m = p ? dynamic_cast<const MemoryExec*>(p->p.get()) : nullptr;
    if (!m) fail(DFGPU_INVALID_ARGUMENT, "plan_memory_replace: not a MemoryExec");
    std::vector<std::vector<Batch>> np; int k = 0;
    for (int i = 0; i < nparts; i++) { np.emplace_back(); for (int j = 0; j < sizes[i]; j++) { const dfgpu_batch* b = batches[k++]; if (!b) fail(DFGPU_INVALID_ARGUMENT, "null batch"); np.back().push_back(b->b); } }
    std::lock_guard<std::mutex> l(m->mu); m->parts = std::move(np);
  });
}
dfgpu_status dfgpu_plan_filter(const dfgpu_expr* pred, const dfgpu_plan* input, dfgpu_plan** out) { return guard([&] { auto f = std::make_shared<FilterExec>(); f->pred = ex(pred); f->input = pl(input); *out = new dfgpu_plan{f}; }); }
dfgpu_status dfgpu_plan_projection(const dfgpu_expr* const* exprs, const char* const* names, int32_t n, const dfgpu_plan* input, dfgpu_plan** out) {
  return guard([&] { auto p = std::make_shared<ProjectionExec>(); for (int i = 0; i < n; i++) { p->exprs.push_back(ex(exprs[i])); p->names.push_back(names[i] ? names[i] : ""); } p->input = pl(input); *out = new dfgpu_plan{p}; });
}
dfgpu_status dfgpu_plan_coalesce_batches(const dfgpu_plan* input, int64_t target, dfgpu_plan** out) { return guard([&] { auto c = std::make_shared<CoalesceBatchesExec>(); c->input = pl(input); c->target = target; *out = new dfgpu_plan{c}; }); }
dfgpu_status dfgpu_plan_coalesce_partitions(const dfgpu_plan* input, dfgpu_plan** out) { return guard([&] { auto c = std::make_shared<CoalescePartitionsExec>(); c->input = pl(input); *out = new dfgpu_plan{c}; }); }
static void mark_selection_consumer(const PlanPtr& p) {
  const Plan* q = p.get();
  while (q) {
    if (auto* hj = dynamic_cast<const HashJoinExec*>(q)) { hj->selection_consumer = true; return; }
    if (auto* cb = dynamic_cast<const CoalesceBatchesExec*>(q)) q = cb->input.get();
    else if (auto* pr = dynamic_cast<const ProjectionExec*>(q)) { if (!pr->only_columns()) return; q = pr->input.get(); }
    else return;
  }
}
dfgpu_status dfgpu_plan_repartition(const dfgpu_plan* input, const dfgpu_expr* const* exprs, int32_t nexprs, int32_t n, dfgpu_plan** out) {
  return guard([&] { if (n < 1) fail(DFGPU_INVALID_ARGUMENT, "repartition: partition count must be positive"); auto r = std::make_shared<RepartitionExec>(); r->input = pl(input); r->n = n; if (nexprs > 0) mark_selection_consumer(r->input); for (int i = 0; i < nexprs; i++) r->exprs.push_back(ex(exprs[i])); *out = new dfgpu_plan{r}; });
}
dfgpu_status dfgpu_plan_hash_join(const dfgpu_plan* left, const dfgpu_plan* right, const dfgpu_expr* const* on_left, const dfgpu_expr* const* on_right, int32_t non,
                                  const dfgpu_expr* filter, const int32_t* fs, const int32_t* fi, int32_t nf, int32_t join_type, int32_t mode, int32_t nen, dfgpu_plan** out) {
  return guard([&] {
    if (!left || !right || !out) fail(DFGPU_INVALID_ARGUMENT, "plan_hash_join: null argument");
    if (non < 1) fail(DFGPU_EXECUTION, "Plan error: On constraints in HashJoinExec should be non-empty");
    if (join_type < 0 || join_type > DFGPU_JOIN_RIGHT_ANTI) fail(DFGPU_INVALID_ARGUMENT, "unknown join type %d", join_type);
    auto j = std::make_shared<HashJoinExec>(); j->left = pl(left); j->right = pl(right);
    for (int i = 0; i < non; i++) { j->on_l.push_back(ex(on_left[i])); j->on_r.push_back(ex(on_right[i])); }
    if (filter) { j->filter = ex(filter); for (int i = 0; i < nf; i++) { j->f_side.push_back(fs[i]); j->f_index.push_back(fi[i]); } }
    j->join_type = join_type; j->mode = mode; j->null_equals_null = nen != 0;
    mark_selection_consumer(j->left); mark_selection_consumer(j->right);
    *out = new dfgpu_plan{j};
  });
}
dfgpu_status dfgpu_plan_sort_merge_join(const dfgpu_plan* left, const dfgpu_plan* right, const dfgpu_expr* const* on_left, const dfgpu_expr* const* on_right, int32_t non, const dfgpu_expr* filter,
                                        const int32_t* fs, const int32_t* fi, int32_t nf, int32_t join_type, int32_t null_equals_null, dfgpu_plan** out) {
  return guard([&] {
    if (!left || !right || !out) fail(DFGPU_INVALID_ARGUMENT, "plan_sort_merge_join: null argument");
    if (non < 1) fail(DFGPU_EXECUTION, "Plan error: On constraints in SortMergeJoinExec should be non-empty");
    if (join_type == DFGPU_JOIN_RIGHT_SEMI) fail(DFGPU_NOT_IMPLEMENTED, "This feature is not implemented: SortMergeJoinExec does not support JoinType::RightSemi");
    if (join_type < 0 || join_type > DFGPU_JOIN_RIGHT_ANTI) fail(DFGPU_NOT_IMPLEMENTED, "This feature is not implemented: SortMergeJoinExec join type %d on the device", join_type);
    if (filter && (join_type == DFGPU_JOIN_LEFT_SEMI || join_type == DFGPU_JOIN_LEFT_ANTI || join_type == DFGPU_JOIN_RIGHT_ANTI))
      fail(DFGPU_NOT_IMPLEMENTED, "This feature is not implemented: SortMergeJoinExec %s with a JoinFilter on the device (Inner, Left, Right and Full take one)", join_type == DFGPU_JOIN_LEFT_SEMI ? "LeftSemi" : join_type == DFGPU_JOIN_LEFT_ANTI ? "LeftAnti" : "RightAnti");
    if (filter && nf > 0 && (!fs || !fi)) fail(DFGPU_INVALID_ARGUMENT, "sort_merge_join: JoinFilter without column indices");
    auto j = std::make_shared<SortMergeJoinExec>(); j->left = pl(left); j->right = pl(right);
    if (filter) { j->filter = ex(filter); for (int i = 0; i < nf; i++) { j->f_side.push_back(fs[i]); j->f_index.push_back(fi[i]); } }
    for (int i = 0; i < non; i++) { j->on_l.push_back(ex(on_left[i])); j->on_r.push_back(ex(on_right[i])); }
    j->join_type = join_type; j->null_equals_null = null_equals_null != 0;
    *out = new dfgpu_plan{j};
  });
}
dfgpu_status dfgpu_plan_nested_loop_join(const dfgpu_plan* left, const dfgpu_plan* right, const dfgpu_expr* filter, const int32_t* fs, const int32_t* fi, int32_t nf, int32_t join_type, dfgpu_plan** out) {
  return guard([&] {
    if (join_type < 0 || join_type > DFGPU_JOIN_RIGHT_ANTI) fail(DFGPU_INVALID_ARGUMENT, "unknown join type %d", join_type);
    auto j = std::make_shared<NestedLoopJoinExec>(); j->left = pl(left); j->right = pl(right); j->join_type = join_type;
    if (filter) { j->filter = ex(filter); for (int i = 0; i < nf; i++) { j->f_side.push_back(fs[i]); j->f_index.push_back(fi[i]); } }
    *out = new dfgpu_plan{j};
  });
}
dfgpu_status dfgpu_plan_aggregate(int32_t mode, const dfgpu_expr* const* gexprs, const char* const* gnames, int32_t ng, const int32_t* kinds, const dfgpu_expr* const* args,
                                  const dfgpu_expr* const* filters, const char* const* names, const int32_t* types, int32_t na, const dfgpu_plan* input, dfgpu_plan** out) {
  return guard([&] {
    if (mode < 0 || mode > 4) fail(DFGPU_INVALID_ARGUMENT, "unknown AggregateMode %d", mode);
    auto a = std::make_shared<AggregateExec>(); a->mode = mode; a->input = pl(input);
// ... 136 lines not shown
```

datafusion-upstream_amd/csrc/join.hip:

```cpp
#include "join_table.h"

namespace dfgpu {
constexpr uint64_t SLOT_EMPTY = ~0ull;
constexpr uint32_t NO_SLOT = 0xFFFFFFFFu;
}
using namespace dfgpu;


namespace dfgpu {

__device__ inline bool row_selected(const uint64_t* mask, int64_t i) { return mask == nullptr || bit_get(mask, i); }

__global__ void __launch_bounds__(BLOCK) k_join_build(KeySet ks, int64_t n, const uint64_t* mask, int null_eq, int force_zero,
                                                      uint64_t* slots, uint32_t* slot_count, uint64_t cap_mask, uint32_t* row_slot,
                                                      unsigned long long* counters ) {
  int64_t i = (int64_t)blockIdx.x * BLOCK + threadIdx.x;
  if (i >= n) return;
  uint32_t my_slot = NO_SLOT;
  if (row_selected(mask, i)) {
    bool any_null; uint64_t h = keyset_hash(ks, i, 0, &any_null);
    if (force_zero) h = 0;
    if (!any_null || null_eq) {
      uint64_t tag = h >> 32, s = h & cap_mask, mine = (tag << 32) | (uint64_t)i;
      for (uint64_t step = 0; step <= cap_mask; step++) {
// ... 67 lines not shown
  for (int q = 0; q < HP_ROWS; q++) {
    bool hit = false;
    if (on[q]) {
      uint64_t c = cur[q], s2 = sl[q];
      if (c != SLOT_EMPTY && (c >> 32) == tag[q] && v0[q] == k0[q] && (NK == 1 || v1[q] == k1[q])) hit = true;
      else if (c != SLOT_EMPTY) {
        for (uint64_t step = 0; step < cap_mask; step++) {
          s2 = (s2 + 1) & cap_mask; c = slots[s2];
          if (c == SLOT_EMPTY) break;
          if ((c >> 32) == tag[q]) { uint64_t r = c & 0xFFFFFFFFull; if (b0[r] == k0[q] && (NK == 1 || b1[r] == k1[q])) { hit = true; break; } }
        }
      }
      if (hit) found_slot[base + (int64_t)q * BLOCK] = (uint32_t)s2;
    }
    int64_t i = base + (int64_t)q * BLOCK;
    uint64_t m = ballot64(hit);
    if (lane_id() == 0 && (i >> 6) < ((n + 63) >> 6)) match_bits[i >> 6] = m;
  }
}
__global__ void __launch_bounds__(BLOCK) k_probe_found(const uint32_t* rows, int64_t m, const uint32_t* found_slot, const uint64_t* slots, const uint32_t* slot_count, int unique,
                                                       uint64_t* out_build, uint32_t* out_slot, uint32_t* out_cnt) {
  int64_t i = (int64_t)blockIdx.x * BLOCK + threadIdx.x;
  if (i >= m) return;
  uint32_t s2 = found_slot[rows[i]];
  if (unique) out_build[i] = slots[s2] & 0xFFFFFFFFull;
  else { out_slot[i] = s2; out_cnt[i] = slot_count[s2]; }
}
constexpr int PM_ROWS = 8;
__device__ inline uint64_t spread32(uint64_t x) {
  x &= 0xFFFFFFFFull;
  x = (x | (x << 16)) & 0x0000FFFF0000FFFFull; x = (x | (x << 8)) & 0x00FF00FF00FF00FFull; x = (x | (x << 4)) & 0x0F0F0F0F0F0F0F0Full;
  x = (x | (x << 2)) & 0x3333333333333333ull; x = (x | (x << 1)) & 0x5555555555555555ull; return x;
}
template <typename T, bool HAS_MASK, bool HAS_VALID, bool FULL>
__device__ inline void probe_match_chunk(const T* keys, const uint64_t* key_valid, const uint64_t* mask, int64_t n, int64_t kmin, uint64_t range,
                                         const uint64_t* bitmap, uint64_t* match_bits, int64_t base, int lane) {
  T k[PM_ROWS / 2][2];
#pragma unroll
  for (int r = 0; r < PM_ROWS / 2; r++) {
    int64_t j = base + r * 2 * WAVE + 2 * lane;
    if (FULL || j + 1 < n) { struct alignas(2 * sizeof(T)) P { T a, b; }; P p = *(const P*)(keys + j); k[r][0] = p.a; k[r][1] = p.b; }
    else { k[r][0] = j < n ? keys[j] : (T)0; k[r][1] = 0; }
  }
  uint64_t mws[PM_ROWS / 2];
#pragma unroll
  for (int r = 0; r < PM_ROWS / 2; r++) { int64_t j = base + r * 2 * WAVE + 2 * lane; mws[r] = (HAS_MASK && (FULL || j < n)) ? mask[j >> 6] >> (j & 63) : 3ull; }
  uint64_t d0 = (uint64_t)((int64_t)k[0][0] - kmin);
  d0 = (uint64_t)__builtin_amdgcn_readfirstlane((uint32_t)d0) | ((uint64_t)__builtin_amdgcn_readfirstlane((uint32_t)(d0 >> 32)) << 32);
  int64_t w0i = d0 < range ? (int64_t)(d0 >> 6) : 0;
  uint64_t win = (uint64_t)(w0i + lane) * 64 < range ? bitmap[w0i + lane] : 0ull;
#pragma unroll
  for (int r = 0; r < PM_ROWS / 2; r++) {
    int64_t j = base + r * 2 * WAVE + 2 * lane;
    const uint64_t mw = mws[r];
    bool h[2];
#pragma unroll
    for (int e = 0; e < 2; e++) {
      uint64_t d = (uint64_t)((int64_t)k[r][e] - kmin);
      bool go = (FULL || j + e < n) && ((mw >> e) & 1) && (!HAS_VALID || valid_at(key_valid, j + e)) && d < range;
      int64_t rel = (int64_t)(d >> 6) - w0i;
      uint64_t word = __shfl(win, (int)(rel & 63), 64);
      if (go && (rel < 0 || rel >= WAVE)) word = bitmap[d >> 6];
      h[e] = go && ((word >> (d & 63)) & 1ull);
    }
    uint64_t be = ballot64(h[0]), bo = ballot64(h[1]);
    uint64_t w0 = spread32(be) | (spread32(bo) << 1), w1 = spread32(be >> 32) | (spread32(bo >> 32) << 1);
    int64_t wbase = (base >> 6) + 2 * r;
    if (lane == 0) { if (FULL || base + r * 2 * WAVE < n) match_bits[wbase] = w0; if (FULL || base + r * 2 * WAVE + WAVE < n) match_bits[wbase + 1] = w1; }
  }
}
template <typename T, bool HAS_MASK, bool HAS_VALID>
__global__ void __launch_bounds__(BLOCK) k_probe_match_bitmap(const T* keys, const uint64_t* key_valid, const uint64_t* mask, int64_t n, int64_t kmin, uint64_t range,
                                                              const uint64_t* bitmap, uint64_t* match_bits) {
  int lane = lane_id();
  int64_t base = ((int64_t)blockIdx.x * (BLOCK / WAVE) + (threadIdx.x >> 6)) * (WAVE * PM_ROWS);
  if (base + WAVE * PM_ROWS <= n) probe_match_chunk<T, HAS_MASK, HAS_VALID, true>(keys, key_valid, mask, n, kmin, range, bitmap, match_bits, base, lane);
  else if (base < n) probe_match_chunk<T, HAS_MASK, HAS_VALID, false>(keys, key_valid, mask, n, kmin, range, bitmap, match_bits, base, lane);
}
__global__ void __launch_bounds__(BLOCK) k_probe_lookup(KeySet bks, KeySet pks, const uint32_t* rows, int64_t m, int null_eq, int force_zero,
                                                        const uint64_t* slots, const uint32_t* slot_count, uint64_t cap_mask, int unique,
                                                        uint64_t* out_build, uint32_t* out_slot, uint32_t* out_cnt, uint32_t* flags) {
  int64_t i = (int64_t)blockIdx.x * BLOCK + threadIdx.x;
  if (i >= m) return;
  int64_t j = rows[i];
  bool any_null; uint64_t h = keyset_hash(pks, j, 0, &any_null);
  if (force_zero) h = 0;
  uint64_t tag = h >> 32, s = h & cap_mask; bool found = false;
  for (uint64_t step = 0; step <= cap_mask; step++) {
    uint64_t cur = slots[s];
    if (cur == SLOT_EMPTY) break;
    if ((cur >> 32) == tag && keyset_equal(bks, (int64_t)(cur & 0xFFFFFFFFull), pks, j, null_eq != 0)) { found = true; break; }
    s = (s + 1) & cap_mask;
  }
  if (!found) { atomicOr(flags, DFGPU_FLAG_TABLE_FULL); s = 0; }
  if (unique) out_build[i] = found ? (slots[s] & 0xFFFFFFFFull) : 0;
  else { out_slot[i] = (uint32_t)s; out_cnt[i] = found ? slot_count[s] : 0; }
}
__global__ void __launch_bounds__(BLOCK) k_probe_expand(const uint32_t* rows, const uint32_t* slot_of, const uint32_t* cnt, const uint64_t* offsets, int64_t m,
                                                        const uint32_t* slot_start, const uint32_t* csr_rows, uint64_t* out_build, uint32_t* out_probe) {
  const int lane = lane_id(); const int64_t w0 = ((int64_t)blockIdx.x * BLOCK + threadIdx.x) - lane;
  if (w0 >= m) return;
  const int64_t i = w0 + lane; const bool on = i < m;
  const uint32_t c = on ? cnt[i] : 0u, st = on ? slot_start[slot_of[i]] : 0u, j = on ? rows[i] : 0u;
  const uint64_t o = on ? offsets[i] : 0ull;
  const uint64_t base = (uint64_t)__shfl((long long)o, 0, 64);
  const uint64_t rel = o - base;
  const int last = 63 - __clzll((long long)ballot64(on));
  const uint64_t total = (uint64_t)__shfl((long long)(rel + c), last, 64);
  for (uint64_t k0 = 0; k0 < total; k0 += WAVE) {
    const uint64_t k = k0 + lane;
// ... 457 lines not shown
  if (hsc[0] != 0) return false;
  const int64_t nsel = (int64_t)hsc[1];
  ArrayHolder rows(new_fixed(ctx, DFGPU_UINT32, nsel));
  DFGPU_INT_KEY_DISPATCH(key0->type, hipLaunchKernelGGL((k_rank_rows<T>), dim3(lgrid), dim3(BLOCK), 0, ctx->stream, (const T*)key0->values->ptr, mk, rl, dcount, n, (int64_t)lo, (const uint64_t*)bitmap->ptr,
                                                        (const uint32_t*)prefix->ptr, (uint32_t*)rows.get()->values->ptr, (const T*)ckp));
  KERNEL_CHECK();
  t->key_min = lo; t->range = range; t->rep = JoinRep::RANK; t->unique = true; t->rank_identity = false;
  t->bitmap = bitmap; t->rank_prefix = prefix; t->sel_rows = rows.release();
  t->mem += (int64_t)bitmap_bytes((int64_t)range) + nw * 4 + nsel * 4;
  return true;
}
void selected_key_range(dfgpu_ctx* ctx, const dfgpu_join_table* t, const char* sync, long long* lo, long long* hi) {
  const dfgpu_array* key0 = t->keys[0]; const int64_t n = t->n_build;
  const long long* mm = key_ranges(ctx, 4, 1, sync, [&](long long* w) {
    DFGPU_INT_KEY_DISPATCH(key0->type, hipLaunchKernelGGL((k_key_minmax_masked<T>), dim3(grid_for(n, BLOCK * 8, ctx->num_cus * 4)), dim3(BLOCK), 0, ctx->stream, (const T*)key0->values->ptr,
                                                          key0->validity ? (const uint64_t*)key0->validity->ptr : nullptr, t->build_mask ? (const uint64_t*)t->build_mask->ptr : nullptr, n, w, w + 1)); });
  *lo = mm[0]; *hi = mm[1];
}

static bool rank_lookup_ok(const dfgpu_join_table* t, const dfgpu_array* const* probe_keys, int32_t nkeys) {
  return t->rep == JoinRep::RANK && !t->pack_n && nkeys == 1 && probe_keys[0]->type == t->keys[0]->type && !probe_keys[0]->validity;
}
static void lookup_rank(dfgpu_ctx* ctx, const dfgpu_join_table* t, const dfgpu_array* pk, const uint32_t* rows, const uint64_t* rows_valid, int64_t m, bool all, uint64_t* out_build) {
  if (!m) return;
  KernelTimer kt_(ctx, "k_probe_lookup_rank");
  const bool sel = t->sel_rows != nullptr;
#define LR(ALL, SEL) DFGPU_INT_KEY_DISPATCH(pk->type, hipLaunchKernelGGL((k_probe_lookup_rank<T, ALL, SEL>), dim3(grid_for(m, BLOCK * LR_ROWS)), dim3(BLOCK), 0, ctx->stream, (const T*)pk->values->ptr, rows, m, t->key_min, \
                                                          (const uint64_t*)t->bitmap->ptr, t->rank_prefix ? (const uint32_t*)t->rank_prefix->ptr : nullptr, \
                                                          sel ? (const uint32_t*)t->sel_rows->values->ptr : nullptr, t->rank_identity ? 1 : 0, out_build, rows_valid, pk->length))
  if (all && sel) { LR(true, true); } else if (all) { LR(true, false); } else if (sel) { LR(false, true); } else { LR(false, false); }
#undef LR
  KERNEL_CHECK();
}
static bool match_bits_by_bitmap(dfgpu_ctx* ctx, const dfgpu_join_table* t, const dfgpu_array* pk, int64_t n, const uint64_t* mk, uint64_t* match_bits) {
  const dfgpu_array* key0 = t->keys[0];
  if (pk->type != key0->type) return false;
  if (t->lazy_row_slot && t->range <= (uint64_t)n * 16) {
    KernelTimer kt_(ctx, "join_build_bitmap");
    t->bitmap = alloc_buffer(ctx, bitmap_bytes((int64_t)t->range), true); t->mem += (int64_t)bitmap_bytes((int64_t)t->range);
    DFGPU_INT_KEY_DISPATCH(key0->type, hipLaunchKernelGGL((k_key_setbits<T>), dim3(grid_for(t->n_build, BLOCK)), dim3(BLOCK), 0, ctx->stream, (const T*)key0->values->ptr,
                                                          (const uint32_t*)t->lazy_row_slot->ptr, t->n_build, t->key_min, (uint64_t*)t->bitmap->ptr));
    KERNEL_CHECK();
    t->lazy_row_slot.reset();
  }
  if (!t->bitmap) return false;
  KernelTimer kt_(ctx, "k_probe_match_bitmap");
  int64_t rows_per_block = (int64_t)BLOCK * PM_ROWS;
  const uint64_t* kvp = pk->validity ? (const uint64_t*)pk->validity->ptr : nullptr;
  const void* kptr = pk->values->ptr; BufferPtr aligned_keys; const size_t kw = (size_t)type_width(pk->type);
  if ((uintptr_t)kptr % (2 * kw)) { aligned_keys = alloc_buffer(ctx, (size_t)n * kw); HIP_CHECK(hipMemcpyAsync(aligned_keys->ptr, kptr, (size_t)n * kw, hipMemcpyDeviceToDevice, ctx->stream)); kptr = aligned_keys->ptr; }
#define PM_LAUNCH(HM, HV) DFGPU_INT_KEY_DISPATCH(pk->type, hipLaunchKernelGGL((k_probe_match_bitmap<T, HM, HV>), dim3(grid_for(n, (int)rows_per_block)), dim3(BLOCK), 0, ctx->stream, (const T*)kptr, \
                                                          kvp, mk, n, t->key_min, t->range, (const uint64_t*)t->bitmap->ptr, match_bits))
  if (mk && kvp) { PM_LAUNCH(true, true); } else if (mk) { PM_LAUNCH(true, false); } else if (kvp) { PM_LAUNCH(false, true); } else { PM_LAUNCH(false, false); }
#undef PM_LAUNCH
  return true;
}
static BufferPtr match_bits_by_hash(dfgpu_ctx* ctx, const dfgpu_join_table* t, const dfgpu_array* const* probe_keys, int32_t nkeys, const KeySet& pks, int64_t n, const uint64_t* mk, uint64_t* match_bits) {
  if (!t->slots) build_hash_table(ctx, t, false);
  KernelTimer kt_(ctx, "k_probe_match_hash");
  auto plain8 = [](const dfgpu_array* a) { return (a->type == DFGPU_INT64 || a->type == DFGPU_UINT64) && !a->validity; };
  bool fast_hash = (nkeys == 1 || nkeys == 2) && !t->null_equals_null && !ctx->force_hash_collisions && t->n_build > 0;
  for (int c = 0; c < nkeys && fast_hash; c++) fast_hash = plain8(probe_keys[c]) && plain8(t->keys[(size_t)c]);
  BufferPtr found_slot;
  if (fast_hash) {
    found_slot = alloc_buffer(ctx, (size_t)n * 4);
    const uint64_t *b0 = (const uint64_t*)t->keys[0]->values->ptr, *b1 = nkeys == 2 ? (const uint64_t*)t->keys[1]->values->ptr : nullptr;
    const uint64_t *p0 = (const uint64_t*)probe_keys[0]->values->ptr, *p1 = nkeys == 2 ? (const uint64_t*)probe_keys[1]->values->ptr : nullptr;
    dim3 hgrid(grid_for(n, BLOCK * HP_ROWS));
#define HP(NK, HM) hipLaunchKernelGGL((k_probe_hash_i64<NK, HM>), hgrid, dim3(BLOCK), 0, ctx->stream, b0, b1, p0, p1, n, mk, (const uint64_t*)t->slots->ptr, t->capacity - 1, match_bits, (uint32_t*)found_slot->ptr)
    if (nkeys == 1) { if (mk) HP(1, true); else HP(1, false); } else { if (mk) HP(2, true); else HP(2, false); }
#undef HP
  } else
  hipLaunchKernelGGL(k_probe_match_hash, dim3(grid_for(n, BLOCK)), dim3(BLOCK), 0, ctx->stream, t->ks, pks, n, mk, t->null_equals_null ? 1 : 0, ctx->force_hash_collisions ? 1 : 0,
                     (const uint64_t*)t->slots->ptr, t->capacity - 1, match_bits);
  return found_slot;
}
static void rank_pairs(dfgpu_ctx* ctx, const dfgpu_join_table* t, const dfgpu_array* pk, ArrayHolder& rows, int64_t n, bool defer, ArrayHolder& ob, ArrayHolder& op) {
  if (!defer) {
    const int64_t m = rows.get()->length;
    ob.a = new_fixed(ctx, DFGPU_UINT64, m);
    lookup_rank(ctx, t, pk, (const uint32_t*)rows.get()->values->ptr, nullptr, m, rows.get()->identity && m == n, (uint64_t*)ob.get()->values->ptr);
  }
  op.a = rows.release();
}
static void rank_runs_pairs(dfgpu_ctx* ctx, const dfgpu_join_table* t, const dfgpu_array* pk, const dfgpu_array* rows, ArrayHolder& ob, ArrayHolder& op) {
// ... 35 lines not shown
}

}

template <typename L, typename R>
__global__ void __launch_bounds__(BLOCK) k_cross_indices(int64_t first, int64_t n_right, int64_t total, L* __restrict__ left, R* __restrict__ right) {
  int64_t k = (int64_t)blockIdx.x * BLOCK + threadIdx.x; if (k >= total) return;
  int64_t i = k / n_right; left[k] = (L)(first + i); right[k] = (R)(k - i * n_right);
}

extern "C" {

dfgpu_status dfgpu_join_build(dfgpu_ctx* ctx, const dfgpu_array* const* keys, int32_t nkeys, const dfgpu_array* opt_mask,
                              int32_t null_equals_null, dfgpu_join_table** out) {
  return guard(ctx, [&] {
    if (!keys || !out) fail(DFGPU_INVALID_ARGUMENT, "join_build: null argument");
    std::unique_ptr<dfgpu_join_table> t(new dfgpu_join_table());
    t->ctx = ctx; t->nkeys = nkeys; t->null_equals_null = null_equals_null != 0;
    int64_t n = keys[0]->length; t->n_build = n;
    if (dfgpu_array* packed = pack_build_keys(ctx, t.get(), keys, nkeys)) { t->nkeys = 1; t->keys.push_back(packed); }
    else for (int c = 0; c < nkeys; c++) { t->keys.push_back(const_cast<dfgpu_array*>(keys[c])); dfgpu_array_retain(t->keys.back()); }
    t->ks = make_keyset(t->keys.data(), t->nkeys);
    t->build_mask = effective_mask(ctx, opt_mask, n);
    t->mem = (int64_t)bitmap_bytes(n);
    if (!build_rank_index(ctx, t.get()) && !build_rank_index_unsorted(ctx, t.get()) && !pj_build(ctx, t.get())) build_hash_table(ctx, t.get(), true);
    *out = t.release();
  });
}
void dfgpu_join_table_free(dfgpu_join_table* t) { delete t; }
int64_t dfgpu_join_table_num_rows(const dfgpu_join_table* t) { return t ? t->n_build : 0; }
int64_t dfgpu_join_table_memory(const dfgpu_join_table* t) { return t ? t->mem : 0; }

static dfgpu_status join_probe_impl(dfgpu_ctx* ctx, const dfgpu_join_table* t, const dfgpu_array* const* probe_keys, int32_t nkeys,
                                    const dfgpu_array* opt_mask, dfgpu_array** out_build_idx, dfgpu_array** out_probe_idx, bool may_defer, dfgpu_array** out_selection);
dfgpu_status dfgpu_join_probe(dfgpu_ctx* ctx, const dfgpu_join_table* t, const dfgpu_array* const* probe_keys, int32_t nkeys,
                              const dfgpu_array* opt_mask, dfgpu_array** out_build_idx, dfgpu_array** out_probe_idx) {
  return join_probe_impl(ctx, t, probe_keys, nkeys, opt_mask, out_build_idx, out_probe_idx, false, nullptr);
}
dfgpu_status dfgpu_join_probe_deferred(dfgpu_ctx* ctx, const dfgpu_join_table* t, const dfgpu_array* const* probe_keys, int32_t nkeys,
                                       const dfgpu_array* opt_mask, dfgpu_array** out_build_idx, dfgpu_array** out_probe_idx) {
  return join_probe_impl(ctx, t, probe_keys, nkeys, opt_mask, out_build_idx, out_probe_idx, true, nullptr);
}
dfgpu_status dfgpu_join_probe_selection(dfgpu_ctx* ctx, const dfgpu_join_table* t, const dfgpu_array* const* probe_keys, int32_t nkeys, const dfgpu_array* opt_mask, dfgpu_array** out_selection) {
  if (!out_selection) return DFGPU_INVALID_ARGUMENT;
  return join_probe_impl(ctx, t, probe_keys, nkeys, opt_mask, nullptr, nullptr, false, out_selection);
}
dfgpu_status dfgpu_join_lookup(dfgpu_ctx* ctx, const dfgpu_join_table* t, const dfgpu_array* const* probe_keys, int32_t nkeys, const dfgpu_array* rows, dfgpu_array** out_build_idx) {
  return guard(ctx, [&] {
    if (!t || !probe_keys || !out_build_idx) fail(DFGPU_INVALID_ARGUMENT, "join_lookup: null argument");
    if (!rank_lookup_ok(t, probe_keys, nkeys))
      fail(DFGPU_INVALID_ARGUMENT, "join_lookup: only after dfgpu_join_probe_deferred left the build indices out (a unique rank-indexed build, one integer key column without NULLs)");
    if (rows && rows->type != DFGPU_UINT32) fail(DFGPU_INVALID_ARGUMENT, "join_lookup: rows must be UInt32");
    const dfgpu_array* pk = probe_keys[0];
    const int64_t m = rows ? rows->length : pk->length;
    ArrayHolder ob(new_fixed(ctx, DFGPU_UINT64, m));
    const uint64_t* rv = rows && rows->validity ? (const uint64_t*)rows->validity->ptr : nullptr;
    lookup_rank(ctx, t, pk, rows ? (const uint32_t*)rows->values->ptr : nullptr, rv, m, !rv && (rows == nullptr || (rows->identity && rows->length == pk->length)), (uint64_t*)ob.get()->values->ptr);
    if (rv) { ob.get()->validity = rows->validity; ob.get()->null_count = rows->null_count; }
    *out_build_idx = ob.release();
  });
}
static dfgpu_status join_probe_impl(dfgpu_ctx* ctx, const dfgpu_join_table* t, const dfgpu_array* const* probe_keys, int32_t nkeys,
                                    const dfgpu_array* opt_mask, dfgpu_array** out_build_idx, dfgpu_array** out_probe_idx, bool may_defer, dfgpu_array** out_selection) {
  return guard(ctx, [&] {
    if (!t || !probe_keys || (!out_selection && (!out_build_idx || !out_probe_idx))) fail(DFGPU_INVALID_ARGUMENT, "join_probe: null argument");
    check_key_types(t, probe_keys, nkeys);
    const bool lookup_ok = rank_lookup_ok(t, probe_keys, nkeys);
    if (out_selection && !lookup_ok) fail(DFGPU_NOT_IMPLEMENTED, "join_probe_selection: only a unique rank-indexed build probed by one integer key column of the build's type without NULLs");
    ArrayHolder packed_probe; const dfgpu_array* pk1 = nullptr;
    if (t->pack_n) {
      for (int c = 0; c < nkeys; c++) if (probe_keys[c]->type == DFGPU_DICTIONARY || probe_keys[c]->length != probe_keys[0]->length) fail(DFGPU_NOT_IMPLEMENTED, "probe of a packed multi-key table with dictionary-encoded keys");
      packed_probe.a = pack_key_array(ctx, t, probe_keys, true);
      pk1 = packed_probe.get(); probe_keys = &pk1; nkeys = 1;
    }
    KeySet pks = make_keyset(probe_keys, nkeys);
    int64_t n = probe_keys[0]->length;
    BufferPtr mask = effective_mask(ctx, opt_mask, n);
    const uint64_t* mk = mask ? (const uint64_t*)mask->ptr : nullptr;
    if (!out_selection && pj_probe_eligible(ctx, t, probe_keys, nkeys, n)) {
      pj_probe(ctx, t, probe_keys, nkeys, mk, out_build_idx, out_probe_idx);
      check_flags(ctx, "join_probe");
      return;
    }
    BufferPtr match_bits = alloc_buffer(ctx, bitmap_bytes(n), n == 0);
    const bool use_bitmap = n && match_bits_by_bitmap(ctx, t, probe_keys[0], n, mk, (uint64_t*)match_bits->ptr);
    const BufferPtr found_slot = n && !use_bitmap ? match_bits_by_hash(ctx, t, probe_keys, nkeys, pks, n, mk, (uint64_t*)match_bits->ptr) : nullptr;
    KERNEL_CHECK();
    if (out_selection) {
      ArrayHolder sel(new_array(ctx, DFGPU_BOOL, n)); sel.get()->values = match_bits; sel.get()->null_count = 0;
      check_flags(ctx, "join_probe");
      *out_selection = sel.release();
      return;
    }
    ArrayHolder rows(mask_to_indices_impl(ctx, (const uint64_t*)match_bits->ptr, n)), ob, op;
    if (use_bitmap && t->rep == JoinRep::RANK_RUNS) rank_runs_pairs(ctx, t, probe_keys[0], rows.get(), ob, op);
    else if (use_bitmap && t->rep == JoinRep::RANK) rank_pairs(ctx, t, probe_keys[0], rows, n, may_defer && lookup_ok, ob, op);
    else hash_pairs(ctx, t, pks, rows, found_slot, ob, op);
    check_flags(ctx, "join_probe");
    *out_build_idx = ob.release(); *out_probe_idx = op.release();
  });
}

dfgpu_status dfgpu_join_mark_visited(dfgpu_ctx* ctx, dfgpu_join_table* t, const dfgpu_array* build_idx) {
  return guard(ctx, [&] {
    if (!t || !build_idx || build_idx->type != DFGPU_UINT64) fail(DFGPU_INVALID_ARGUMENT, "mark_visited: UINT64 build indices expected");
    int64_t n = build_idx->length; if (!n) return;
    if (!t->visited) t->visited = alloc_buffer(ctx, bitmap_bytes(t->n_build), true);
    hipLaunchKernelGGL(k_mark_bits_u64idx, dim3(grid_for(n, BLOCK)), dim3(BLOCK), 0, ctx->stream, (const uint64_t*)build_idx->values->ptr,
                       build_idx->validity ? (const uint64_t*)build_idx->validity->ptr : nullptr, n, (uint64_t*)t->visited->ptr, t->n_build, ctx->d_flags);
    KERNEL_CHECK();
    check_flags(ctx, "join_mark_visited");
  });
}

dfgpu_status dfgpu_join_final_indices(dfgpu_ctx* ctx, const dfgpu_join_table* t, int32_t join_type, dfgpu_array** out_build_idx) {
  return guard(ctx, [&] {
    if (!t || !out_build_idx) fail(DFGPU_INVALID_ARGUMENT, "final_indices: null argument");
    bool semi = join_type == DFGPU_JOIN_LEFT_SEMI;
// ... 94 lines not shown
```

datafusion-upstream_amd/device.py:

```python
from __future__ import annotations

import ctypes as C
from typing import List, Optional, Sequence

from . import capi
from .capi import DfgpuError


_OWNERS = {}
_OWNER_SEQ = 0


def _release_owner(cookie):
    try:
        _OWNERS.pop(int(cookie), None)
    except Exception:
        pass


_RELEASE_CB = C.CFUNCTYPE(None, C.c_void_p)(_release_owner)


def lent_memory_owners() -> int:
    return len(_OWNERS)
# ... 273 lines not shown
                self.ctx.lib.dfgpu_join_table_free(self.h)
                self.h = None
        except Exception:
            pass

    @property
    def num_rows(self) -> int:
        return self.ctx.lib.dfgpu_join_table_num_rows(self.h)

    @property
    def memory(self) -> int:
        return self.ctx.lib.dfgpu_join_table_memory(self.h)

    def probe(self, keys: Sequence[Array], mask: Optional[Array] = None):
        hs, n = capi.handle_array([a.h.value for a in keys])
        ob, op = C.c_void_p(), C.c_void_p()
        self.ctx.check(self.ctx.lib.dfgpu_join_probe(self.ctx.h, self.h, hs, n, mask.h if mask is not None else None, C.byref(ob), C.byref(op)))
        return Array(self.ctx, ob), Array(self.ctx, op)

    def probe_deferred(self, keys: Sequence[Array], mask: Optional[Array] = None):
        hs, n = capi.handle_array([a.h.value for a in keys])
        ob, op = C.c_void_p(), C.c_void_p()
        self.ctx.check(self.ctx.lib.dfgpu_join_probe_deferred(self.ctx.h, self.h, hs, n, mask.h if mask is not None else None, C.byref(ob), C.byref(op)))
        return (Array(self.ctx, ob) if ob.value else None), Array(self.ctx, op)

    def probe_selection(self, keys: Sequence[Array], mask: Optional[Array] = None) -> Optional[Array]:
        hs, n = capi.handle_array([a.h.value for a in keys])
        out = C.c_void_p()
        st = self.ctx.lib.dfgpu_join_probe_selection(self.ctx.h, self.h, hs, n, mask.h if mask is not None else None, C.byref(out))
        if st == 4:
            return None
        self.ctx.check(st)
        return Array(self.ctx, out)

    def lookup(self, keys: Sequence[Array], rows: Optional[Array] = None) -> Array:
        hs, n = capi.handle_array([a.h.value for a in keys])
        out = C.c_void_p()
        self.ctx.check(self.ctx.lib.dfgpu_join_lookup(self.ctx.h, self.h, hs, n, rows.h if rows is not None else None, C.byref(out)))
        return Array(self.ctx, out)

    def mark_visited(self, build_idx: Array):
        self.ctx.check(self.ctx.lib.dfgpu_join_mark_visited(self.ctx.h, self.h, build_idx.h))

    def final_indices(self, join_type: int) -> Array:
        out = C.c_void_p()
        self.ctx.check(self.ctx.lib.dfgpu_join_final_indices(self.ctx.h, self.h, join_type, C.byref(out)))
        return Array(self.ctx, out)


def join_adjust_indices(ctx: Context, build_idx: Array, probe_idx: Array, range_start: int, range_end: int, join_type: int):
    ob, op = C.c_void_p(), C.c_void_p()
    ctx.check(ctx.lib.dfgpu_join_adjust_indices(ctx.h, build_idx.h, probe_idx.h, range_start, range_end, join_type, C.byref(ob), C.byref(op)))
    return Array(ctx, ob), Array(ctx, op)


def agg_preaggregate(ctx: Context, key, kinds: Sequence[int], values: Sequence[Optional[Array]], mask: Optional[Array] = None, any_order: bool = False, casts: Optional[Sequence[int]] = None):
    n = len(kinds)
    keys = [key] if isinstance(key, Array) else list(key)
    kh = (C.c_void_p * len(keys))(*[k.h for k in keys])
    kk = (C.c_int32 * max(1, n))(*kinds)
    vh = (C.c_void_p * max(1, n))(*[(v.h if v is not None else None) for v in values])
    ok = (C.c_void_p * 4)()
    os_ = (C.c_void_p * (2 * max(1, n)))()
    cc = (C.c_int32 * max(1, n))(*[int(c) for c in casts]) if casts is not None else None
    ctx.check(ctx.lib.dfgpu_agg_preaggregate_flags(ctx.h, kh, len(keys), kk, vh, cc, n, mask.h if mask is not None else None, 1 if any_order else 0, ok, os_))
    states = [[Array(ctx, C.c_void_p(os_[2 * i + j])) for j in range(2) if os_[2 * i + j]] for i in range(n)]
# ... 116 lines not shown
```

include/dfgpu.h:

```cpp
#ifndef DFGPU_H
#define DFGPU_H
#include <stdint.h>
#include <stddef.h>

#ifdef __cplusplus
extern "C" {
#endif

#define DFGPU_API __attribute__((visibility("default")))

typedef int32_t dfgpu_status;
enum { DFGPU_OK = 0, DFGPU_EXECUTION = 1, DFGPU_INTERNAL = 2, DFGPU_RESOURCES_EXHAUSTED = 3,
       DFGPU_NOT_IMPLEMENTED = 4, DFGPU_INVALID_ARGUMENT = 5 };

enum { DFGPU_BOOL = 1, DFGPU_INT8 = 2, DFGPU_INT16 = 3, DFGPU_INT32 = 4, DFGPU_INT64 = 5,
       DFGPU_UINT8 = 6, DFGPU_UINT16 = 7, DFGPU_UINT32 = 8, DFGPU_UINT64 = 9,
       DFGPU_FLOAT32 = 10, DFGPU_FLOAT64 = 11, DFGPU_DATE32 = 12, DFGPU_DECIMAL128 = 13,
       DFGPU_UTF8 = 14, DFGPU_DICTIONARY = 15 };

typedef struct dfgpu_array_desc {
  int32_t type;
  int32_t precision;
  int32_t scale;
  int32_t key_type;
// ... 70 lines not shown
DFGPU_API dfgpu_status dfgpu_take_multi(dfgpu_ctx *ctx, const dfgpu_array *const *values, int32_t n, const dfgpu_array *indices, dfgpu_array **out);
DFGPU_API dfgpu_status dfgpu_filter(dfgpu_ctx *ctx, const dfgpu_array *values, const dfgpu_array *mask, dfgpu_array **out);
DFGPU_API dfgpu_status dfgpu_mask_to_indices(dfgpu_ctx *ctx, const dfgpu_array *mask, dfgpu_array **out);

enum { DFGPU_OP_ADD = 0, DFGPU_OP_SUB = 1, DFGPU_OP_MUL = 2, DFGPU_OP_DIV = 3, DFGPU_OP_REM = 4,
       DFGPU_OP_EQ = 10, DFGPU_OP_NEQ = 11, DFGPU_OP_LT = 12, DFGPU_OP_LTEQ = 13, DFGPU_OP_GT = 14,
       DFGPU_OP_GTEQ = 15, DFGPU_OP_DISTINCT = 16, DFGPU_OP_NOT_DISTINCT = 17,
       DFGPU_OP_AND = 20, DFGPU_OP_OR = 21 };
DFGPU_API dfgpu_status dfgpu_binary(dfgpu_ctx *ctx, int32_t op, const dfgpu_array *lhs, int32_t lhs_is_scalar,
                                    const dfgpu_array *rhs, int32_t rhs_is_scalar, dfgpu_array **out);
DFGPU_API dfgpu_status dfgpu_binary_fused2(dfgpu_ctx *ctx, int32_t op_outer, const dfgpu_array *x, int32_t op_inner, const dfgpu_array *scalar, const dfgpu_array *y,
                                           int32_t scalar_on_left, int32_t inner_on_left, dfgpu_array **out);
DFGPU_API dfgpu_status dfgpu_not(dfgpu_ctx *ctx, const dfgpu_array *a, dfgpu_array **out);
DFGPU_API dfgpu_status dfgpu_is_null(dfgpu_ctx *ctx, const dfgpu_array *a, int32_t negate, dfgpu_array **out);
DFGPU_API dfgpu_status dfgpu_negative(dfgpu_ctx *ctx, const dfgpu_array *a, dfgpu_array **out);
DFGPU_API dfgpu_status dfgpu_cast(dfgpu_ctx *ctx, const dfgpu_array *a, int32_t to_type, int32_t precision, int32_t scale, dfgpu_array **out);
DFGPU_API dfgpu_status dfgpu_in_list(dfgpu_ctx *ctx, const dfgpu_array *a, const dfgpu_array *list, int32_t negated, dfgpu_array **out);

enum { DFGPU_JOIN_INNER = 0, DFGPU_JOIN_LEFT = 1, DFGPU_JOIN_RIGHT = 2, DFGPU_JOIN_FULL = 3,
       DFGPU_JOIN_LEFT_SEMI = 4, DFGPU_JOIN_RIGHT_SEMI = 5, DFGPU_JOIN_LEFT_ANTI = 6,
       DFGPU_JOIN_RIGHT_ANTI = 7 };
DFGPU_API dfgpu_status dfgpu_join_build(dfgpu_ctx *ctx, const dfgpu_array *const *keys, int32_t nkeys,
                                        const dfgpu_array *opt_mask, int32_t null_equals_null, dfgpu_join_table **out);
DFGPU_API void dfgpu_join_table_free(dfgpu_join_table *t);
DFGPU_API int64_t dfgpu_join_table_num_rows(const dfgpu_join_table *t);
DFGPU_API int64_t dfgpu_join_table_memory(const dfgpu_join_table *t);
DFGPU_API dfgpu_status dfgpu_join_probe(dfgpu_ctx *ctx, const dfgpu_join_table *t, const dfgpu_array *const *probe_keys,
                                        int32_t nkeys, const dfgpu_array *opt_mask,
                                        dfgpu_array **out_build_idx, dfgpu_array **out_probe_idx);
DFGPU_API dfgpu_status dfgpu_join_probe_deferred(dfgpu_ctx *ctx, const dfgpu_join_table *table, const dfgpu_array *const *probe_keys, int32_t nkeys,
                                                 const dfgpu_array *opt_mask, dfgpu_array **out_build_idx, dfgpu_array **out_probe_idx);
DFGPU_API dfgpu_status dfgpu_join_probe_selection(dfgpu_ctx *ctx, const dfgpu_join_table *table, const dfgpu_array *const *probe_keys, int32_t nkeys,
                                                  const dfgpu_array *opt_mask, dfgpu_array **out_selection);
DFGPU_API dfgpu_status dfgpu_join_lookup(dfgpu_ctx *ctx, const dfgpu_join_table *table, const dfgpu_array *const *probe_keys, int32_t nkeys, const dfgpu_array *rows,
                                         dfgpu_array **out_build_idx);
DFGPU_API dfgpu_status dfgpu_join_mark_visited(dfgpu_ctx *ctx, dfgpu_join_table *t, const dfgpu_array *build_idx);
DFGPU_API dfgpu_status dfgpu_join_adjust_indices(dfgpu_ctx *ctx, const dfgpu_array *build_idx, const dfgpu_array *probe_idx,
                                                 int64_t range_start, int64_t range_end, int32_t join_type,
                                                 dfgpu_array **out_build_idx, dfgpu_array **out_probe_idx);
DFGPU_API dfgpu_status dfgpu_cross_join_indices(dfgpu_ctx *ctx, int64_t first_left, int64_t count_left, int64_t n_right, int32_t left_is_u64,
                                                dfgpu_array **out_left, dfgpu_array **out_right);
DFGPU_API dfgpu_status dfgpu_join_final_indices(dfgpu_ctx *ctx, const dfgpu_join_table *t, int32_t join_type, dfgpu_array **out_build_idx);

DFGPU_API dfgpu_status dfgpu_groups_new(dfgpu_ctx *ctx, int32_t nkeys, dfgpu_groups **out);
DFGPU_API void dfgpu_groups_free(dfgpu_groups *g);
DFGPU_API dfgpu_status dfgpu_groups_intern(dfgpu_ctx *ctx, dfgpu_groups *g, const dfgpu_array *const *cols, int32_t nkeys,
                                           const dfgpu_array *opt_mask, dfgpu_array **out_group_ids);
DFGPU_API dfgpu_status dfgpu_groups_intern_deferred(dfgpu_ctx *ctx, dfgpu_groups *g, const dfgpu_array *const *key_columns, int32_t nkeys,
                                                    const dfgpu_array *opt_mask, dfgpu_array **out_group_ids);
DFGPU_API int64_t dfgpu_groups_len(const dfgpu_groups *g);
DFGPU_API int64_t dfgpu_groups_size(const dfgpu_groups *g);
DFGPU_API dfgpu_status dfgpu_groups_emit(dfgpu_ctx *ctx, dfgpu_groups *g, dfgpu_array **out_cols );
DFGPU_API dfgpu_status dfgpu_groups_emit_deferred(dfgpu_ctx *ctx, dfgpu_groups *g, dfgpu_array **out_sources, dfgpu_array **out_rows);
DFGPU_API dfgpu_status dfgpu_groups_emit_first(dfgpu_ctx *ctx, dfgpu_groups *g, int64_t n, dfgpu_array **out_cols );

enum { DFGPU_AGG_SUM = 0, DFGPU_AGG_AVG = 1, DFGPU_AGG_COUNT = 2, DFGPU_AGG_MIN = 3, DFGPU_AGG_MAX = 4 };
DFGPU_API dfgpu_status dfgpu_acc_new(dfgpu_ctx *ctx, int32_t kind, int32_t in_type, int32_t in_precision, int32_t in_scale, dfgpu_acc **out);
DFGPU_API void dfgpu_acc_free(dfgpu_acc *a);
DFGPU_API dfgpu_status dfgpu_acc_update_batch(dfgpu_ctx *ctx, dfgpu_acc *a, const dfgpu_array *values, const dfgpu_array *group_ids,
                                              const dfgpu_array *opt_filter, int64_t total_num_groups);
DFGPU_API dfgpu_status dfgpu_acc_update_batch_multi(dfgpu_ctx *ctx, dfgpu_acc *const *accs, const dfgpu_array *const *values, const dfgpu_array *const *filters,
                                                    int32_t n_accs, const dfgpu_array *group_ids, int64_t total_num_groups);
typedef struct dfgpu_expr_node { int32_t op; int32_t lhs; int32_t rhs; } dfgpu_expr_node;
#define DFGPU_NODE_COLUMN (-1)
#define DFGPU_NODE_SCALAR (-2)
DFGPU_API dfgpu_status dfgpu_acc_update_batch_fused(dfgpu_ctx *ctx, dfgpu_acc *const *accs, const int32_t *acc_nodes, int32_t n_accs,
// ... 65 lines not shown
```

shim/src/ffi.rs:

```rust
use std::ffi::{c_char, c_void, CStr, CString};
use std::ptr::null_mut;
use std::sync::Arc;

use arrow::array::{make_array, Array, ArrayRef};
use arrow::ffi::{from_ffi, to_ffi, FFI_ArrowArray, FFI_ArrowSchema};
use datafusion_common::{DataFusionError, Result};

macro_rules! opaque { ($($n:ident),*) => { $(#[repr(C)] pub struct $n { _p: [u8; 0] })* } }
opaque!(dfgpu_ctx, dfgpu_array, dfgpu_expr, dfgpu_plan, dfgpu_batch, dfgpu_stream, dfgpu_comm, dfgpu_parquet, dfgpu_join_table);

#[repr(C)]
pub struct dfgpu_comm_vtable {
    pub user: *mut c_void, pub rank: i32, pub world: i32,
    pub all_gather_host: Option<unsafe extern "C" fn(*mut c_void, *const c_void, i64, *mut c_void) -> i32>,
    pub all_to_all_v: Option<unsafe extern "C" fn(*mut c_void, *const c_void, *const i64, *const i64, *mut c_void, *const i64, *const i64) -> i32>,
}

pub const OP_ADD: i32 = 0; pub const OP_SUB: i32 = 1; pub const OP_MUL: i32 = 2; pub const OP_DIV: i32 = 3; pub const OP_REM: i32 = 4;
pub const OP_EQ: i32 = 10; pub const OP_NEQ: i32 = 11; pub const OP_LT: i32 = 12; pub const OP_LTEQ: i32 = 13; pub const OP_GT: i32 = 14; pub const OP_GTEQ: i32 = 15;
pub const OP_DISTINCT: i32 = 16; pub const OP_NOT_DISTINCT: i32 = 17; pub const OP_AND: i32 = 20; pub const OP_OR: i32 = 21;
pub const AGG_SUM: i32 = 0; pub const AGG_AVG: i32 = 1; pub const AGG_COUNT: i32 = 2; pub const AGG_MIN: i32 = 3; pub const AGG_MAX: i32 = 4;

extern "C" {
    pub fn dfgpu_ctx_create(device_id: i32, stream: *mut c_void, out: *mut *mut dfgpu_ctx) -> i32;
    pub fn dfgpu_ctx_destroy(ctx: *mut dfgpu_ctx);
    pub fn dfgpu_last_error(ctx: *const dfgpu_ctx) -> *const c_char;
    pub fn dfgpu_ctx_set_option(ctx: *mut dfgpu_ctx, key: *const c_char, value: i64) -> i32;
    pub fn dfgpu_array_import_arrow(ctx: *mut dfgpu_ctx, a: *mut FFI_ArrowArray, s: *mut FFI_ArrowSchema, out: *mut *mut dfgpu_array) -> i32;
    pub fn dfgpu_array_export_arrow(ctx: *mut dfgpu_ctx, a: *const dfgpu_array, out_a: *mut FFI_ArrowArray, out_s: *mut FFI_ArrowSchema) -> i32;
    pub fn dfgpu_array_release(a: *mut dfgpu_array);
    pub fn dfgpu_array_wrap_device_owned(ctx: *mut dfgpu_ctx, desc: *const c_void , release: Option<unsafe extern "C" fn(*mut c_void)>, cookie: *mut c_void, out: *mut *mut dfgpu_array) -> i32;
    pub fn dfgpu_comm_unique_id(out_id128: *mut u8) -> i32;
    pub fn dfgpu_comm_create_rccl(ctx: *mut dfgpu_ctx, id128: *const u8, rank: i32, world: i32, out: *mut *mut dfgpu_comm) -> i32;
    pub fn dfgpu_comm_create_custom(vtable: *const dfgpu_comm_vtable, out: *mut *mut dfgpu_comm) -> i32;
    pub fn dfgpu_comm_free(comm: *mut dfgpu_comm);
    pub fn dfgpu_exchange(ctx: *mut dfgpu_ctx, comm: *mut dfgpu_comm, keys: *const *const dfgpu_array, nkeys: i32, cols: *const *const dfgpu_array, ncols: i32,
                          opt_mask: *const dfgpu_array, out_cols: *mut *mut dfgpu_array, out_counts: *mut i64) -> i32;
    pub fn dfgpu_parquet_open(ctx: *mut dfgpu_ctx, file_bytes: *const u8, len: i64, device_bytes: *const u8, out: *mut *mut dfgpu_parquet) -> i32;
    pub fn dfgpu_parquet_close(file: *mut dfgpu_parquet);
    pub fn dfgpu_parquet_num_row_groups(file: *const dfgpu_parquet) -> i32;
    pub fn dfgpu_parquet_column_stats(file: *const dfgpu_parquet, row_group: i32, column: i32, min_value: *mut i64, max_value: *mut i64, null_count: *mut i64, has_min_max: *mut i32) -> i32;
    pub fn dfgpu_parquet_read(ctx: *mut dfgpu_ctx, file: *mut dfgpu_parquet, first_row_group: i32, num_row_groups: i32, columns: *const i32, ncols: i32, out: *mut *mut dfgpu_array) -> i32;
    pub fn dfgpu_sort_to_indices_keys(ctx: *mut dfgpu_ctx, cols: *const *const dfgpu_array, descending: *const u8, nulls_first: *const u8, k: i32, fetch: i64, out: *mut *mut dfgpu_array, out_sorted: *mut *mut dfgpu_array) -> i32;
    pub fn dfgpu_agg_preaggregate_flags(ctx: *mut dfgpu_ctx, keys: *const *const dfgpu_array, nkeys: i32, kinds: *const i32, values: *const *const dfgpu_array, value_casts: *const i32, n_aggs: i32,
                                        opt_mask: *const dfgpu_array, flags: i32, out_keys: *mut *mut dfgpu_array, out_states: *mut *mut dfgpu_array) -> i32;
    pub fn dfgpu_csv_read(ctx: *mut dfgpu_ctx, bytes: *const u8, len: i64, bytes_on_device: i32, delimiter: i32, quote: i32, escape: i32, has_header: i32, ncols_file: i32, columns: *const i32, types: *const i32, ncols: i32, out: *mut *mut dfgpu_array, out_rows: *mut i64) -> i32;
    pub fn dfgpu_plan_aggregate_input_order(aggregate: *mut dfgpu_plan, input_order_mode: i32, order_indices: *const i32, n: i32) -> i32;
    pub fn dfgpu_plan_parquet(file: *mut dfgpu_parquet, columns: *const i32, ncols: i32, npartitions: i32, row_groups_per_batch: i32, out: *mut *mut dfgpu_plan) -> i32;
    pub fn dfgpu_plan_csv(bytes: *const u8, len: i64, delimiter: i32, quote: i32, escape: i32, has_header: i32, names: *const *const c_char, types: *const i32, ncols_file: i32, columns: *const i32, ncols: i32, npartitions: i32, batch_bytes: i64, out: *mut *mut dfgpu_plan) -> i32;
    pub fn dfgpu_plan_parquet_prune(parquet_exec: *mut dfgpu_plan, column: i32, min_value: i64, max_value: i64) -> i32;
    pub fn dfgpu_list_from_counts(ctx: *mut dfgpu_ctx, counts: *const dfgpu_array, values: *const dfgpu_array, out: *mut *mut dfgpu_array) -> i32;
    pub fn dfgpu_list_flatten(ctx: *mut dfgpu_ctx, list: *const dfgpu_array, value_type: i32, precision: i32, scale: i32, out_values: *mut *mut dfgpu_array, out_row_of: *mut *mut dfgpu_array) -> i32;
    pub fn dfgpu_join_probe_deferred(ctx: *mut dfgpu_ctx, table: *const dfgpu_join_table, probe_keys: *const *const dfgpu_array, nkeys: i32, opt_mask: *const dfgpu_array,
                                     out_build_idx: *mut *mut dfgpu_array, out_probe_idx: *mut *mut dfgpu_array) -> i32;
    pub fn dfgpu_join_probe_selection(ctx: *mut dfgpu_ctx, table: *const dfgpu_join_table, probe_keys: *const *const dfgpu_array, nkeys: i32, opt_mask: *const dfgpu_array, out_selection: *mut *mut dfgpu_array) -> i32;
    pub fn dfgpu_join_lookup(ctx: *mut dfgpu_ctx, table: *const dfgpu_join_table, probe_keys: *const *const dfgpu_array, nkeys: i32, rows: *const dfgpu_array, out_build_idx: *mut *mut dfgpu_array) -> i32;
    pub fn dfgpu_plan_sort_merge_join(left: *const dfgpu_plan, right: *const dfgpu_plan, on_l: *const *const dfgpu_expr, on_r: *const *const dfgpu_expr, non: i32, filter: *const dfgpu_expr,
                                      filter_sides: *const i32, filter_indices: *const i32, nfilter_cols: i32, join_type: i32, null_equals_null: i32, out: *mut *mut dfgpu_plan) -> i32;
    pub fn dfgpu_plan_nested_loop_join(left: *const dfgpu_plan, right: *const dfgpu_plan, filter: *const dfgpu_expr, filter_sides: *const i32, filter_indices: *const i32,
                                       nfilter_cols: i32, join_type: i32, out: *mut *mut dfgpu_plan) -> i32;
    pub fn dfgpu_plan_metrics(p: *const dfgpu_plan, buf: *mut c_char, capacity: i64) -> i32;
    pub fn dfgpu_exec_last_error() -> *const c_char;
    pub fn dfgpu_batch_new(names: *const *const c_char, columns: *const *const dfgpu_array, ncols: i32, out: *mut *mut dfgpu_batch) -> i32;
    pub fn dfgpu_batch_free(b: *mut dfgpu_batch);
    pub fn dfgpu_batch_num_columns(b: *const dfgpu_batch) -> i32;
    pub fn dfgpu_batch_column(ctx: *mut dfgpu_ctx, b: *mut dfgpu_batch, i: i32, out: *mut *mut dfgpu_array) -> i32;
    pub fn dfgpu_expr_column(name: *const c_char, index: i32, out: *mut *mut dfgpu_expr) -> i32;
    pub fn dfgpu_expr_literal(scalar_len1: *const dfgpu_array, out: *mut *mut dfgpu_expr) -> i32;
    pub fn dfgpu_expr_binary(l: *const dfgpu_expr, op: i32, r: *const dfgpu_expr, out: *mut *mut dfgpu_expr) -> i32;
    pub fn dfgpu_expr_not(e: *const dfgpu_expr, out: *mut *mut dfgpu_expr) -> i32;
    pub fn dfgpu_expr_is_null(e: *const dfgpu_expr, negated: i32, out: *mut *mut dfgpu_expr) -> i32;
    pub fn dfgpu_expr_negative(e: *const dfgpu_expr, out: *mut *mut dfgpu_expr) -> i32;
    pub fn dfgpu_expr_cast(e: *const dfgpu_expr, to_type: i32, precision: i32, scale: i32, out: *mut *mut dfgpu_expr) -> i32;
    pub fn dfgpu_expr_free(e: *mut dfgpu_expr);
    pub fn dfgpu_plan_memory(batches: *const *const dfgpu_batch, partition_sizes: *const i32, npartitions: i32, out: *mut *mut dfgpu_plan) -> i32;
    pub fn dfgpu_plan_filter(predicate: *const dfgpu_expr, input: *const dfgpu_plan, out: *mut *mut dfgpu_plan) -> i32;
    pub fn dfgpu_plan_projection(exprs: *const *const dfgpu_expr, names: *const *const c_char, n: i32, input: *const dfgpu_plan, out: *mut *mut dfgpu_plan) -> i32;
    pub fn dfgpu_plan_coalesce_batches(input: *const dfgpu_plan, target: i64, out: *mut *mut dfgpu_plan) -> i32;
    pub fn dfgpu_plan_coalesce_partitions(input: *const dfgpu_plan, out: *mut *mut dfgpu_plan) -> i32;
    pub fn dfgpu_plan_repartition(input: *const dfgpu_plan, exprs: *const *const dfgpu_expr, nexprs: i32, num_partitions: i32, out: *mut *mut dfgpu_plan) -> i32;
    pub fn dfgpu_plan_hash_join(left: *const dfgpu_plan, right: *const dfgpu_plan, on_l: *const *const dfgpu_expr, on_r: *const *const dfgpu_expr, non: i32,
                                filter: *const dfgpu_expr, filter_sides: *const i32, filter_indices: *const i32, nfilter_cols: i32,
                                join_type: i32, mode: i32, null_equals_null: i32, out: *mut *mut dfgpu_plan) -> i32;
    pub fn dfgpu_plan_aggregate(mode: i32, group_exprs: *const *const dfgpu_expr, group_names: *const *const c_char, ngroups: i32,
                                agg_kinds: *const i32, agg_args: *const *const dfgpu_expr, agg_filters: *const *const dfgpu_expr, agg_names: *const *const c_char,
                                agg_arg_types: *const i32, naggs: i32, input: *const dfgpu_plan, out: *mut *mut dfgpu_plan) -> i32;
    pub fn dfgpu_plan_sort(exprs: *const *const dfgpu_expr, descending: *const u8, nulls_first: *const u8, n: i32, fetch: i64, preserve_partitioning: i32,
                           input: *const dfgpu_plan, out: *mut *mut dfgpu_plan) -> i32;
// ... 67 lines not shown
```

Baseline: 228.3 billion rows/s.

## Fuse simple column-vs-scalar filter predicates into the hash join probe bitmap kernel

A FilterExec feeding a join probe now defers simple `column <op> literal` predicates on integer/date columns as a pending predicate on the batch instead of building a mask. The join probe then evaluates the predicate inside the membership-bitmap match kernel through a new dfgpu_join_probe_fused entry point, falling back to materialising the mask when the fused path is not implemented. This removes a separate comparison kernel, a mask allocation and an AND pass per large probe batch, such as the lineitem date filter in Q3. It adds lazy-selection plumbing across all Batch users, which risks extra evaluation when other operators force the selection.

Measured after the change: 262.1 billion rows/s (median of 6 runs). 14.8% higher.

```diff
diff --git a/datafusion-upstream_amd/capi.py b/datafusion-upstream_amd/capi.py
--- a/datafusion-upstream_amd/capi.py
+++ b/datafusion-upstream_amd/capi.py
@@ -123,6 +123,7 @@
     "dfgpu_join_probe_deferred": (C.c_int32, [_P, _P, _PP, C.c_int32, _P, _PP, _PP]),
     "dfgpu_join_lookup": (C.c_int32, [_P, _P, _PP, C.c_int32, _P, _PP]),
     "dfgpu_join_probe_selection": (C.c_int32, [_P, _P, _PP, C.c_int32, _P, _PP]),
+    "dfgpu_join_probe_fused": (C.c_int32, [_P, _P, _PP, C.c_int32, _P, _P, C.c_int32, _P, C.c_int32, _PP, _PP, _PP]),
     "dfgpu_join_mark_visited": (C.c_int32, [_P, _P, _P]),
     "dfgpu_join_adjust_indices": (C.c_int32, [_P, _P, _P, C.c_int64, C.c_int64, C.c_int32, _PP, _PP]),
     "dfgpu_join_final_indices": (C.c_int32, [_P, _P, C.c_int32, _PP]),
diff --git a/datafusion-upstream_amd/csrc/core.hip b/datafusion-upstream_amd/csrc/core.hip
--- a/datafusion-upstream_amd/csrc/core.hip
+++ b/datafusion-upstream_amd/csrc/core.hip
@@ -372,6 +372,7 @@
   { "join_rank_index_unsorted", OPT_BOOL(join_rank_index_unsorted) },
   { "join_lazy_build_rows", OPT_BOOL(join_lazy_build_rows) },
   { "join_selection_output", OPT_BOOL(join_selection_output) },
+  { "join_probe_fused_filter", OPT_BOOL(join_probe_fused_filter) },
   { "join_key_packing", OPT_BOOL(join_key_packing) },
   { "join_swap_small_semi", OPT_BOOL(join_swap_small_semi) },
   { "join_partitioned", OPT_BOOL(join_partitioned) },
diff --git a/datafusion-upstream_amd/csrc/dfgpu_internal.h b/datafusion-upstream_amd/csrc/dfgpu_internal.h
--- a/datafusion-upstream_amd/csrc/dfgpu_internal.h
+++ b/datafusion-upstream_amd/csrc/dfgpu_internal.h
@@ -43,6 +43,7 @@
   bool join_rank_index = true;
   bool join_lazy_build_rows = true;
   bool join_selection_output = true;
+  bool join_probe_fused_filter = true;
   bool join_rank_index_unsorted = true;
   bool join_key_packing = true;
   bool group_run_detection = true;
diff --git a/datafusion-upstream_amd/csrc/exec/exec.cpp b/datafusion-upstream_amd/csrc/exec/exec.cpp
--- a/datafusion-upstream_amd/csrc/exec/exec.cpp
+++ b/datafusion-upstream_amd/csrc/exec/exec.cpp
@@ -108,8 +108,26 @@
 }
 static Col col_of(ArrayRef a) { Col c; c.arr = std::move(a); return c; }
 
+struct PendingPredicate { ArrayRef column, scalar; int op = 0; explicit operator bool() const { return op != 0; } };
 struct Batch {
-  SchemaPtr schema; std::vector<Col> cols; ArrayRef selection; int64_t base_rows = 0;
+  SchemaPtr schema; std::vector<Col> cols; int64_t base_rows = 0;
+ private:
+  mutable ArrayRef sel_; mutable PendingPredicate pend_;
+ public:
+  bool filtered() const { return sel_ || pend_; }
+  bool has_pending() const { return (bool)pend_; }
+  const ArrayRef& selection(const TaskContext& tc) const {
+    if (pend_) {
+      dfgpu_array* o = nullptr; tc.check(dfgpu_binary(tc.ctx, pend_.op, pend_.column.a, 0, pend_.scalar.a, 1, &o)); ArrayRef mask = ArrayRef::adopt(o);
+      if (sel_) { dfgpu_array* a = nullptr; tc.check(dfgpu_binary(tc.ctx, DFGPU_OP_AND, mask.a, 0, sel_.a, 0, &a)); mask = ArrayRef::adopt(a); }
+      sel_ = mask; pend_ = PendingPredicate();
+    }
+    return sel_;
+  }
+  void set_selection(ArrayRef s) { sel_ = std::move(s); pend_ = PendingPredicate(); }
+  void set_pending(ArrayRef column, int op, ArrayRef scalar) { pend_.column = std::move(column); pend_.op = op; pend_.scalar = std::move(scalar); }
+  void filter_like(const Batch& o) { sel_ = o.sel_; pend_ = o.pend_; }
+  ArrayRef take_filter(PendingPredicate* pending) { *pending = pend_; pend_ = PendingPredicate(); ArrayRef m = std::move(sel_); sel_ = ArrayRef(); return m; }
   const ArrayRef& column(const TaskContext& tc, int i) {
     Col& c = cols.at((size_t)i);
     if (!c.arr && c.source && !c.chain.empty() && base_rows <= ((int64_t)1 << 20) && base_rows > 0) {
@@ -131,13 +149,13 @@
 };
 static ArrayRef mask_indices(const TaskContext& tc, const ArrayRef& mask) { dfgpu_array* o = nullptr; tc.check(dfgpu_mask_to_indices(tc.ctx, mask.a, &o)); return ArrayRef::adopt(o); }
 static Batch materialize(const TaskContext& tc, const Batch& b) {
-  if (!b.selection) return b;
-  ArrayRef sel = mask_indices(tc, b.selection);
+  if (!b.filtered()) return b;
+  ArrayRef sel = mask_indices(tc, b.selection(tc));
   Batch o; o.schema = b.schema; o.base_rows = sel.len();
   MemoPtr memo = std::make_shared<TakeMemo>(); for (auto& c : b.cols) o.cols.push_back(col_take(c, sel, memo));
   return o;
 }
-static int64_t num_rows(const TaskContext& tc, const Batch& b) { return b.selection ? mask_indices(tc, b.selection).len() : b.base_rows; }
+static int64_t num_rows(const TaskContext& tc, const Batch& b) { return b.filtered() ? mask_indices(tc, b.selection(tc)).len() : b.base_rows; }
 static ArrayRef concat_arrays(const TaskContext& tc, std::vector<ArrayRef>& parts) {
   std::vector<const dfgpu_array*> p; for (auto& x : parts) p.push_back(x.a);
   dfgpu_array* o = nullptr; tc.check(dfgpu_concat(tc.ctx, p.data(), (int32_t)p.size(), &o)); return ArrayRef::adopt(o);
@@ -274,7 +292,7 @@
   virtual std::unique_ptr<Stream> execute(int partition, const TaskContext& tc) const = 0;
   virtual PlanPtr fresh() const = 0;
 };
-static int64_t metric_rows(const TaskContext& tc, const Batch& b) { if (!b.selection) return b.base_rows; int64_t k = 0; tc.check(dfgpu_mask_count(tc.ctx, b.selection.a, &k)); return k; }
+static int64_t metric_rows(const TaskContext& tc, const Batch& b) { if (!b.filtered()) return b.base_rows; int64_t k = 0; tc.check(dfgpu_mask_count(tc.ctx, b.selection(tc).a, &k)); return k; }
 struct MeteredStream : Stream {
   const Plan* op; PlanPtr keep; std::unique_ptr<Stream> in; TaskContext tc;
   MeteredStream(PlanPtr k, std::unique_ptr<Stream> i, TaskContext t) : op(k.get()), keep(std::move(k)), in(std::move(i)), tc(t) {}
@@ -388,7 +406,21 @@
 
 struct FilterExec : Plan {
   ExprPtr pred; PlanPtr input;
-  PlanPtr fresh() const override { auto f = std::make_shared<FilterExec>(); f->pred = pred; f->input = input->fresh(); return f; }
+  mutable bool feeds_probe = false;
+  PlanPtr fresh() const override { auto f = std::make_shared<FilterExec>(); f->pred = pred; f->input = input->fresh(); f->feeds_probe = feeds_probe; return f; }
+  bool deferrable(const TaskContext& tc, const Batch& b, ArrayRef* column, int* op, ArrayRef* scalar) const {
+    if (!feeds_probe || b.has_pending() || b.base_rows <= (tc.batch_size > 8192 ? tc.batch_size : 8192)) return false;
+    auto* be = dynamic_cast<const BinaryExpr*>(pred.get()); if (!be || be->op < DFGPU_OP_EQ || be->op > DFGPU_OP_GTEQ) return false;
+    const bool col_left = be->l->column_index() >= 0;
+    auto* lit = dynamic_cast<const LiteralExpr*>((col_left ? be->r : be->l).get()); const int ci = (col_left ? be->l : be->r)->column_index();
+    if (!lit || ci < 0 || ci >= (int)b.cols.size() || !b.cols[(size_t)ci].arr) return false;
+    int64_t v = 1; if (dfgpu_ctx_get_option(tc.ctx, "join_probe_fused_filter", &v) == DFGPU_OK && v == 0) return false;
+    dfgpu_array_desc cd, sd; dfgpu_array_describe(b.cols[(size_t)ci].arr.a, &cd); dfgpu_array_describe(lit->scalar.a, &sd);
+    if ((cd.type != DFGPU_INT32 && cd.type != DFGPU_DATE32 && cd.type != DFGPU_INT64) || cd.validity || cd.length != b.base_rows || sd.type != cd.type || sd.length != 1 || sd.validity || sd.null_count != 0) return false;
+    static const int swapped[6] = { DFGPU_OP_EQ, DFGPU_OP_NEQ, DFGPU_OP_GT, DFGPU_OP_GTEQ, DFGPU_OP_LT, DFGPU_OP_LTEQ };
+    *column = b.cols[(size_t)ci].arr; *scalar = lit->scalar; *op = col_left ? be->op : swapped[be->op - DFGPU_OP_EQ];
+    return true;
+  }
   std::vector<std::shared_ptr<const Plan>> children() const override { return {input}; }
   const char* name() const override { return "FilterExec"; }
   SchemaPtr schema() const override { return input->schema(); }
@@ -398,20 +430,21 @@
     S(const FilterExec* o, std::unique_ptr<Stream> i, TaskContext t) : op(o), in(std::move(i)), tc(t) {}
     bool next(Batch& out) override {
       Batch b; if (!in->next(b)) return false;
-      if (b.selection && !op->pred->safe()) b = materialize(tc, b);
+      { ArrayRef column, scalar; int cmp = 0; if (op->deferrable(tc, b, &column, &cmp, &scalar)) { b.set_pending(column, cmp, scalar); out = std::move(b); return true; } }
+      if (b.filtered() && !op->pred->safe()) b = materialize(tc, b);
       Value v = op->pred->eval(tc, b);
       ArrayRef mask = into_array(tc, v, b.base_rows);
       dfgpu_array_desc d; dfgpu_array_describe(mask.a, &d);
       if (d.type != DFGPU_BOOL) fail(DFGPU_INTERNAL, "Cannot create filter_array from non-boolean predicates");
-      if (b.selection) { ArrayRef km = known_mask(tc, mask); dfgpu_array* o = nullptr; tc.check(dfgpu_binary(tc.ctx, DFGPU_OP_AND, km.a, 0, b.selection.a, 0, &o)); mask = ArrayRef::adopt(o); }
-      b.selection = mask; out = std::move(b); return true;
+      if (b.filtered()) { ArrayRef km = known_mask(tc, mask); dfgpu_array* o = nullptr; tc.check(dfgpu_binary(tc.ctx, DFGPU_OP_AND, km.a, 0, b.selection(tc).a, 0, &o)); mask = ArrayRef::adopt(o); }
+      b.set_selection(mask); out = std::move(b); return true;
     }
   };
   std::unique_ptr<Stream> execute(int p, const TaskContext& tc) const override { return std::unique_ptr<Stream>(new S(this, input->run(p, tc), tc)); }
 };
 
 static Batch materialize_subset(const TaskContext& tc, Batch& b, const std::set<int>& needed) {
-  ArrayRef sel = mask_indices(tc, b.selection);
+  ArrayRef sel = mask_indices(tc, b.selection(tc));
   Batch o; o.schema = b.schema; o.base_rows = sel.len();
   ArrayRef filler; MemoPtr memo = std::make_shared<TakeMemo>();
   for (size_t i = 0; i < b.cols.size(); i++) {
@@ -438,12 +471,12 @@
   bool only_columns() const { bool oc = true; for (auto& e : exprs) oc &= e->column_index() >= 0; return oc; }
   Batch project(const TaskContext& tc, Batch b, std::vector<bool>* defer = nullptr) const {
     RowSel rowsel;
-    if (b.selection && !only_columns() && !defer) {
-      int64_t kept = 0; tc.check(dfgpu_mask_count(tc.ctx, b.selection.a, &kept));
-      if (kept * 4 >= b.base_rows) { tc.check(dfgpu_ctx_set_row_selection(tc.ctx, b.selection.a)); rowsel.c = tc.ctx; }
+    if (b.filtered() && !only_columns() && !defer) {
+      int64_t kept = 0; tc.check(dfgpu_mask_count(tc.ctx, b.selection(tc).a, &kept));
+      if (kept * 4 >= b.base_rows) { tc.check(dfgpu_ctx_set_row_selection(tc.ctx, b.selection(tc).a)); rowsel.c = tc.ctx; }
       else { std::set<int> need; for (auto& e : exprs) e->columns(need); b = materialize_subset(tc, b, need); if (defer) defer->assign(exprs.size(), false); defer = nullptr; }
     }
-    Batch o; o.base_rows = b.base_rows; o.selection = b.selection; auto s = std::make_shared<Schema>();
+    Batch o; o.base_rows = b.base_rows; o.filter_like(b); auto s = std::make_shared<Schema>();
     if (defer) defer->assign(exprs.size(), false);
     for (size_t i = 0; i < exprs.size(); i++) {
       int ci = exprs[i]->column_index();
@@ -458,7 +491,7 @@
   }
   void evaluate_deferred(const TaskContext& tc, Batch& raw, Batch& projected, size_t i) const {
     RowSel rowsel;
-    if (raw.selection) { tc.check(dfgpu_ctx_set_row_selection(tc.ctx, raw.selection.a)); rowsel.c = tc.ctx; }
+    if (raw.filtered()) { tc.check(dfgpu_ctx_set_row_selection(tc.ctx, raw.selection(tc).a)); rowsel.c = tc.ctx; }
     ArrayRef a = into_array(tc, exprs[i]->eval(tc, raw), raw.base_rows);
     projected.schema->f[i] = field_of(names[i], a.a); projected.cols[i] = col_of(a);
   }
@@ -487,7 +520,7 @@
     bool next(Batch& out) override {
       while (!done) {
         Batch b; if (!in->next(b)) { done = true; break; }
-        if (b.selection) { if (b.base_rows >= op->target) { out = std::move(b); return true; } b = materialize(tc, b); }
+        if (b.filtered()) { if (b.base_rows >= op->target) { out = std::move(b); return true; } b = materialize(tc, b); }
         if (b.base_rows == 0) continue;
         if (b.base_rows >= op->target && buf.empty()) { out = std::move(b); return true; }
         rows += b.base_rows; buf.push_back(std::move(b));
@@ -516,13 +549,14 @@
 static void partition_batch(const TaskContext& tc, Batch& b, const std::vector<ExprPtr>& exprs, int n, std::vector<std::vector<Batch>>& outs) {
   if (b.base_rows == 0) return;
   bool safe_keys = true; for (auto& e : exprs) safe_keys &= e->safe();
-  if (n <= 256 && (!b.selection || safe_keys)) {
-    Batch kb = b; kb.selection = ArrayRef();
+  if (n <= 256 && (!b.filtered() || safe_keys)) {
+    const ArrayRef bsel = b.selection(tc);
+    Batch kb = b; kb.set_selection(ArrayRef());
     std::vector<ArrayRef> keys; std::vector<const dfgpu_array*> kp;
     for (auto& e : exprs) { keys.push_back(into_array(tc, e->eval(tc, kb), kb.base_rows)); kp.push_back(keys.back().a); }
     std::vector<const dfgpu_array*> cp; for (auto& c : b.cols) cp.push_back(c.arr ? c.arr.a : nullptr);
     std::vector<dfgpu_array*> oc(b.cols.size(), nullptr); std::vector<int64_t> counts((size_t)n); dfgpu_array* idx = nullptr;
-    tc.check(dfgpu_partition_columns(tc.ctx, kp.data(), (int32_t)kp.size(), n, cp.data(), (int32_t)cp.size(), b.selection.a, oc.data(), &idx, counts.data()));
+    tc.check(dfgpu_partition_columns(tc.ctx, kp.data(), (int32_t)kp.size(), n, cp.data(), (int32_t)cp.size(), bsel.a, oc.data(), &idx, counts.data()));
     ArrayRef indices = ArrayRef::adopt(idx); std::vector<ArrayRef> moved; for (auto* x : oc) moved.push_back(ArrayRef::adopt(x));
     int64_t off = 0;
     for (int d = 0; d < n; d++) {
@@ -542,7 +576,7 @@
     return;
   }
   ArrayRef sel; Batch kb = b;
-  if (b.selection) { std::set<int> need; for (auto& e : exprs) e->columns(need); sel = mask_indices(tc, b.selection); kb = materialize_subset(tc, b, need); }
+  if (b.filtered()) { std::set<int> need; for (auto& e : exprs) e->columns(need); sel = mask_indices(tc, b.selection(tc)); kb = materialize_subset(tc, b, need); }
   if (kb.base_rows == 0) return;
   std::vector<ArrayRef> keys; std::vector<const dfgpu_array*> kp;
   for (auto& e : exprs) { keys.push_back(into_array(tc, e->eval(tc, kb), kb.base_rows)); kp.push_back(keys.back().a); }
@@ -616,7 +650,7 @@
     auto bs = std::make_shared<BuildSide>();
     std::vector<Batch> in;
     if (partition < 0) { for (int p = 0; p < left->partitions(); p++) drain(left, p, tc, in); } else drain(left, partition, tc, in);
-    if (in.size() == 1 && in[0].selection) { bs->batch = in[0]; *fused = in[0].selection; bs->batch.selection = ArrayRef(); bs->segments = { bs->batch.base_rows }; bs->empty = false; }
+    if (in.size() == 1 && in[0].filtered()) { *fused = in[0].selection(tc); bs->batch = in[0]; bs->batch.set_selection(ArrayRef()); bs->segments = { bs->batch.base_rows }; bs->empty = false; }
     else {
       std::vector<Batch> m; for (auto& b : in) { Batch x = materialize(tc, b); if (x.base_rows) { bs->segments.push_back(x.base_rows); m.push_back(std::move(x)); } }
       if (m.empty()) return bs;
@@ -737,22 +771,33 @@
         if (pb.base_rows == 0) continue;
         SpanGuard join_span(tc, op->met.get(), 2);
         const bool chunked = pb.base_rows <= (tc.batch_size > 8192 ? tc.batch_size : 8192);
-        if (chunked && pb.selection) { pb = materialize(tc, pb); if (pb.base_rows == 0) continue; }
-        if (pb.selection && (op->join_type == DFGPU_JOIN_RIGHT || op->join_type == DFGPU_JOIN_FULL || op->right_only())) { pb = materialize(tc, pb); if (pb.base_rows == 0) continue; }
-        ArrayRef mask = pb.selection; pb.selection = ArrayRef();
+        if (chunked && pb.filtered()) { pb = materialize(tc, pb); if (pb.base_rows == 0) continue; }
+        if (pb.filtered() && (op->join_type == DFGPU_JOIN_RIGHT || op->join_type == DFGPU_JOIN_FULL || op->right_only())) { pb = materialize(tc, pb); if (pb.base_rows == 0) continue; }
+        PendingPredicate pend; ArrayRef mask;
+        if (pb.has_pending() && !bs->empty) mask = pb.take_filter(&pend); else { mask = pb.selection(tc); pb.set_selection(ArrayRef()); }
         ArrayRef bidx, pidx;
         if (bs->empty) { dfgpu_array *a = nullptr, *b = nullptr; dfgpu_array_desc d{}; d.type = DFGPU_UINT64; d.values = &d; tc.check(dfgpu_array_import_host(tc.ctx, &d, &a)); d.type = DFGPU_UINT32; tc.check(dfgpu_array_import_host(tc.ctx, &d, &b)); bidx = ArrayRef::adopt(a); pidx = ArrayRef::adopt(b); }
         else {
           std::vector<ArrayRef> keys; std::vector<const dfgpu_array*> kp;
           for (auto& e : op->on_r) { keys.push_back(into_array(tc, e->eval(tc, pb), pb.base_rows)); kp.push_back(keys.back().a); }
           dfgpu_array *b = nullptr, *p = nullptr;
+          auto probe_as = [&](int form, dfgpu_array** ob, dfgpu_array** opi, dfgpu_array** os) -> dfgpu_status {
+            if (pend) {
+              dfgpu_status st = dfgpu_join_probe_fused(tc.ctx, bs->table->t, kp.data(), (int32_t)kp.size(), mask.a, pend.column.a, pend.op, pend.scalar.a, form, ob, opi, os);
+              if (st != DFGPU_NOT_IMPLEMENTED) return st;
+              Batch r; r.base_rows = pb.base_rows; r.set_selection(mask); r.set_pending(pend.column, pend.op, pend.scalar); mask = r.selection(tc); pend = PendingPredicate();
+            }
+            if (form == DFGPU_PROBE_SELECTION) return dfgpu_join_probe_selection(tc.ctx, bs->table->t, kp.data(), (int32_t)kp.size(), mask.a, os);
+            if (form == DFGPU_PROBE_DEFERRED) return dfgpu_join_probe_deferred(tc.ctx, bs->table->t, kp.data(), (int32_t)kp.size(), mask.a, ob, opi);
+            return dfgpu_join_probe(tc.ctx, bs->table->t, kp.data(), (int32_t)kp.size(), mask.a, ob, opi);
+          };
           bool defer = !chunked && op->join_type == DFGPU_JOIN_INNER && !op->filter && !need_final && kp.size() == 1 && lazy_build_rows;
           if (defer && selection_output && op->selection_consumer) {
             std::vector<int> al = key_aliases(&bs->batch, pb); bool all = !al.empty(); for (int a : al) all = all && a >= 0;
             if (all) {
-              dfgpu_array* s = nullptr; dfgpu_status st = dfgpu_join_probe_selection(tc.ctx, bs->table->t, kp.data(), 1, mask.a, &s);
+              dfgpu_array* s = nullptr; dfgpu_status st = probe_as(DFGPU_PROBE_SELECTION, nullptr, nullptr, &s);
               if (st == DFGPU_OK) {
-                Batch o; o.schema = out_schema; o.base_rows = pb.base_rows; o.selection = ArrayRef::adopt(s);
+                Batch o; o.schema = out_schema; o.base_rows = pb.base_rows; o.set_selection(ArrayRef::adopt(s));
                 for (int a : al) o.cols.push_back(pb.cols[(size_t)a]);
                 for (auto& c : pb.cols) o.cols.push_back(c);
                 out = std::move(o); return true;
@@ -762,14 +807,14 @@
           }
           for (auto& c : bs->batch.cols) defer = defer && (bool)c.arr;
           if (defer) {
-            tc.check(dfgpu_join_probe_deferred(tc.ctx, bs->table->t, kp.data(), 1, mask.a, &b, &p)); pidx = ArrayRef::adopt(p);
+            tc.check(probe_as(DFGPU_PROBE_DEFERRED, &b, &p, nullptr)); pidx = ArrayRef::adopt(p);
             if (!b) {
               auto lz = std::make_shared<LazyLookup>(); lz->keep = bs; lz->table = bs->table->t; lz->probe_key = keys[0]; lz->rows = pidx; lz->m = pidx.len();
               bool wanted = false; { std::vector<int> al = key_aliases(&bs->batch, pb); for (int a : al) wanted |= a < 0; }
               if (!wanted || (dfgpu_array_is_identity(pidx.a) && pidx.len() == pb.base_rows)) { out = build_batch(&bs->batch, pb, ArrayRef(), pidx, lz); return true; }
               bidx = lz->resolve(tc, ArrayRef());
             } else bidx = ArrayRef::adopt(b);
-          } else { tc.check(dfgpu_join_probe(tc.ctx, bs->table->t, kp.data(), (int32_t)kp.size(), mask.a, &b, &p)); bidx = ArrayRef::adopt(b); pidx = ArrayRef::adopt(p); }
+          } else { tc.check(probe_as(DFGPU_PROBE_PAIRS, &b, &p, nullptr)); bidx = ArrayRef::adopt(b); pidx = ArrayRef::adopt(p); }
           if (!chunked) { apply_filter(pb, bidx, pidx); if (need_final) tc.check(dfgpu_join_mark_visited(tc.ctx, bs->table->t, bidx.a)); }
         }
         if (chunked) {
@@ -805,7 +850,7 @@
       Batch& lb = bs->batch;
       const bool anti = op->join_type == DFGPU_JOIN_LEFT_ANTI;
       if (anti && fused) {
-        Batch sel = lb; sel.selection = fused; lb = materialize(tc, sel); fused = ArrayRef(); bs->segments = { lb.base_rows };
+        Batch sel = lb; sel.set_selection(fused); lb = materialize(tc, sel); fused = ArrayRef(); bs->segments = { lb.base_rows };
       }
       ArrayRef lidx;
       if (!have_right) {
@@ -1377,7 +1422,7 @@
         for (int ci : need) ensure(ci);
       }
       if (b.base_rows == 0) return;
-      ArrayRef mask = b.selection; b.selection = ArrayRef();
+      ArrayRef mask = b.selection(tc); b.set_selection(ArrayRef());
       if (!sets.empty()) { if (specials) fail(DFGPU_NOT_IMPLEMENTED, "This feature is not implemented: COUNT(DISTINCT) / string MIN-MAX under grouping sets on the device"); for (size_t ci = 0; ci < deferred.size(); ci++) ensure((int)ci); group_aggregate_sets(tc, b, mask, groups, accs); return; }
       ArrayRef gids; int64_t total = 1;
       if (grouped) {
@@ -1880,7 +1925,7 @@
 const char* dfgpu_batch_column_name(const dfgpu_batch* b, int32_t i) { return (b && i >= 0 && i < (int)b->b.schema->f.size()) ? b->b.schema->f[(size_t)i].name.c_str() : ""; }
 dfgpu_status dfgpu_batch_num_rows(dfgpu_ctx* ctx, dfgpu_batch* b, int64_t* out) { return guard([&] { if (!ctx || !b || !out) fail(DFGPU_INVALID_ARGUMENT, "batch_num_rows: null argument"); TaskContext tc{ctx, 8192}; *out = num_rows(tc, b->b); }); }
 static void materialize_all(const TaskContext& tc, Batch& b) {
-  if (b.selection) b = materialize(tc, b);
+  if (b.filtered()) b = materialize(tc, b);
   std::map<const dfgpu_array*, std::vector<size_t>> groups;
   for (size_t i = 0; i < b.cols.size(); i++) { Col& c = b.cols[i]; if (!c.arr && c.source && !c.chain.empty()) groups[col_indices(tc, c).a].push_back(i); }
   for (auto& g : groups) {
@@ -1900,7 +1945,7 @@
   return guard([&] {
     if (!ctx || !b || !out) fail(DFGPU_INVALID_ARGUMENT, "batch_column: null argument");
     TaskContext tc{ctx, 8192};
-    if (b->b.selection) b->b = materialize(tc, b->b);
+    if (b->b.filtered()) b->b = materialize(tc, b->b);
     const ArrayRef& a = b->b.column(tc, i); dfgpu_array_retain(a.a); *out = a.a;
   });
 }
@@ -1981,10 +2026,11 @@
 }
 dfgpu_status dfgpu_plan_coalesce_batches(const dfgpu_plan* input, int64_t target, dfgpu_plan** out) { return guard([&] { auto c = std::make_shared<CoalesceBatchesExec>(); c->input = pl(input); c->target = target; *out = new dfgpu_plan{c}; }); }
 dfgpu_status dfgpu_plan_coalesce_partitions(const dfgpu_plan* input, dfgpu_plan** out) { return guard([&] { auto c = std::make_shared<CoalescePartitionsExec>(); c->input = pl(input); *out = new dfgpu_plan{c}; }); }
-static void mark_selection_consumer(const PlanPtr& p) {
+static void mark_selection_consumer(const PlanPtr& p, bool probe_side = false) {
   const Plan* q = p.get();
   while (q) {
     if (auto* hj = dynamic_cast<const HashJoinExec*>(q)) { hj->selection_consumer = true; return; }
+    if (auto* fe = dynamic_cast<const FilterExec*>(q)) { if (probe_side) fe->feeds_probe = true; return; }
     if (auto* cb = dynamic_cast<const CoalesceBatchesExec*>(q)) q = cb->input.get();
     else if (auto* pr = dynamic_cast<const ProjectionExec*>(q)) { if (!pr->only_columns()) return; q = pr->input.get(); }
     else return;
@@ -2003,7 +2049,7 @@
     for (int i = 0; i < non; i++) { j->on_l.push_back(ex(on_left[i])); j->on_r.push_back(ex(on_right[i])); }
     if (filter) { j->filter = ex(filter); for (int i = 0; i < nf; i++) { j->f_side.push_back(fs[i]); j->f_index.push_back(fi[i]); } }
     j->join_type = join_type; j->mode = mode; j->null_equals_null = nen != 0;
-    mark_selection_consumer(j->left); mark_selection_consumer(j->right);
+    mark_selection_consumer(j->left); mark_selection_consumer(j->right, true);
     *out = new dfgpu_plan{j};
   });
 }
diff --git a/datafusion-upstream_amd/csrc/join.hip b/datafusion-upstream_amd/csrc/join.hip
--- a/datafusion-upstream_amd/csrc/join.hip
+++ b/datafusion-upstream_amd/csrc/join.hip
@@ -123,50 +123,81 @@
   x = (x | (x << 16)) & 0x0000FFFF0000FFFFull; x = (x | (x << 8)) & 0x00FF00FF00FF00FFull; x = (x | (x << 4)) & 0x0F0F0F0F0F0F0F0Full;
   x = (x | (x << 2)) & 0x3333333333333333ull; x = (x | (x << 1)) & 0x5555555555555555ull; return x;
 }
-template <typename T, bool HAS_MASK, bool HAS_VALID, bool FULL>
-__device__ inline void probe_match_chunk(const T* keys, const uint64_t* key_valid, const uint64_t* mask, int64_t n, int64_t kmin, uint64_t range,
+template <int OP, typename P> __device__ inline bool probe_pred(P x, P s) {
+  switch (OP) { case 0: return true; case DFGPU_OP_EQ: return x == s; case DFGPU_OP_NEQ: return x != s; case DFGPU_OP_LT: return x < s;
+    case DFGPU_OP_LTEQ: return x <= s; case DFGPU_OP_GT: return x > s; default: return x >= s; }
+}
+template <typename T, typename P, int OP, bool HAS_MASK, bool HAS_VALID, bool FULL>
+__device__ inline void probe_match_chunk(const T* keys, const uint64_t* key_valid, const uint64_t* mask, const P* pred, P ps, int64_t n, int64_t kmin, uint64_t range,
                                          const uint64_t* bitmap, uint64_t* match_bits, int64_t base, int lane) {
-  T k[PM_ROWS / 2][2];
-#pragma unroll
-  for (int r = 0; r < PM_ROWS / 2; r++) {
+  constexpr int PAIRS = PM_ROWS / 2;
+  T k[PAIRS][2]; P pv[PAIRS][2]; uint64_t sw[PAIRS];
+#pragma unroll
+  for (int r = 0; r < PAIRS; r++) {
     int64_t j = base + r * 2 * WAVE + 2 * lane;
-    if (FULL || j + 1 < n) { struct alignas(2 * sizeof(T)) P { T a, b; }; P p = *(const P*)(keys + j); k[r][0] = p.a; k[r][1] = p.b; }
+    if (FULL || j + 1 < n) { struct alignas(2 * sizeof(T)) K2 { T a, b; }; K2 p = *(const K2*)(keys + j); k[r][0] = p.a; k[r][1] = p.b; }
     else { k[r][0] = j < n ? keys[j] : (T)0; k[r][1] = 0; }
   }
-  uint64_t mws[PM_ROWS / 2];
-#pragma unroll
-  for (int r = 0; r < PM_ROWS / 2; r++) { int64_t j = base + r * 2 * WAVE + 2 * lane; mws[r] = (HAS_MASK && (FULL || j < n)) ? mask[j >> 6] >> (j & 63) : 3ull; }
+  if (OP != 0) {
+#pragma unroll
+    for (int r = 0; r < PAIRS; r++) {
+      int64_t j = base + r * 2 * WAVE + 2 * lane;
+      if (FULL || j + 1 < n) { struct alignas(2 * sizeof(P)) P2 { P a, b; }; P2 p = *(const P2*)(pred + j); pv[r][0] = p.a; pv[r][1] = p.b; }
+      else { pv[r][0] = j < n ? pred[j] : ps; pv[r][1] = ps; }
+    }
+  }
+#pragma unroll
+  for (int r = 0; r < PAIRS; r++) {
+    int64_t j = base + r * 2 * WAVE + 2 * lane;
+    uint64_t w = 3ull;
+    if (HAS_MASK && (FULL || j < n)) w &= mask[j >> 6] >> (j & 63);
+    if (HAS_VALID && (FULL || j < n)) w &= key_valid[j >> 6] >> (j & 63);
+    sw[r] = w;
+  }
   uint64_t d0 = (uint64_t)((int64_t)k[0][0] - kmin);
   d0 = (uint64_t)__builtin_amdgcn_readfirstlane((uint32_t)d0) | ((uint64_t)__builtin_amdgcn_readfirstlane((uint32_t)(d0 >> 32)) << 32);
-  int64_t w0i = d0 < range ? (int64_t)(d0 >> 6) : 0;
-  uint64_t win = (uint64_t)(w0i + lane) * 64 < range ? bitmap[w0i + lane] : 0ull;
-#pragma unroll
-  for (int r = 0; r < PM_ROWS / 2; r++) {
+  const int64_t w0i = d0 < range ? (int64_t)(d0 >> 6) : 0;
+  uint64_t d[PAIRS][2]; bool go[PAIRS][2]; bool inwin = true;
+#pragma unroll
+  for (int r = 0; r < PAIRS; r++) {
     int64_t j = base + r * 2 * WAVE + 2 * lane;
-    const uint64_t mw = mws[r];
-    bool h[2];
 #pragma unroll
     for (int e = 0; e < 2; e++) {
-      uint64_t d = (uint64_t)((int64_t)k[r][e] - kmin);
-      bool go = (FULL || j + e < n) && ((mw >> e) & 1) && (!HAS_VALID || valid_at(key_valid, j + e)) && d < range;
-      int64_t rel = (int64_t)(d >> 6) - w0i;
-      uint64_t word = __shfl(win, (int)(rel & 63), 64);
-      if (go && (rel < 0 || rel >= WAVE)) word = bitmap[d >> 6];
-      h[e] = go && ((word >> (d & 63)) & 1ull);
-    }
-    uint64_t be = ballot64(h[0]), bo = ballot64(h[1]);
+      d[r][e] = (uint64_t)((int64_t)k[r][e] - kmin);
+      go[r][e] = (bool)((int)(FULL || j + e < n) & (int)((sw[r] >> e) & 1) & (int)probe_pred<OP, P>(pv[r][e], ps) & (int)(d[r][e] < range));
+      int64_t rel = (int64_t)(d[r][e] >> 6) - w0i;
+      inwin = inwin && (!go[r][e] || (rel >= 0 && rel < WAVE));
+    }
+  }
+  uint64_t word[PAIRS][2];
+  if (ballot64(!inwin) == 0) {
+    uint64_t win = (uint64_t)(w0i + lane) * 64 < range ? bitmap[w0i + lane] : 0ull;
+#pragma unroll
+    for (int r = 0; r < PAIRS; r++)
+#pragma unroll
+      for (int e = 0; e < 2; e++) word[r][e] = __shfl(win, (int)(((int64_t)(d[r][e] >> 6) - w0i) & 63), 64);
+  } else {
+#pragma unroll
+    for (int r = 0; r < PAIRS; r++)
+#pragma unroll
+      for (int e = 0; e < 2; e++) word[r][e] = bitmap[go[r][e] ? d[r][e] >> 6 : 0];
+  }
+#pragma unroll
+  for (int r = 0; r < PAIRS; r++) {
+    bool h0 = go[r][0] && ((word[r][0] >> (d[r][0] & 63)) & 1ull), h1 = go[r][1] && ((word[r][1] >> (d[r][1] & 63)) & 1ull);
+    uint64_t be = ballot64(h0), bo = ballot64(h1);
     uint64_t w0 = spread32(be) | (spread32(bo) << 1), w1 = spread32(be >> 32) | (spread32(bo >> 32) << 1);
     int64_t wbase = (base >> 6) + 2 * r;
     if (lane == 0) { if (FULL || base + r * 2 * WAVE < n) match_bits[wbase] = w0; if (FULL || base + r * 2 * WAVE + WAVE < n) match_bits[wbase + 1] = w1; }
   }
 }
-template <typename T, bool HAS_MASK, bool HAS_VALID>
-__global__ void __launch_bounds__(BLOCK) k_probe_match_bitmap(const T* keys, const uint64_t* key_valid, const uint64_t* mask, int64_t n, int64_t kmin, uint64_t range,
+template <typename T, typename P, int OP, bool HAS_MASK, bool HAS_VALID>
+__global__ void __launch_bounds__(BLOCK) k_probe_match_bitmap(const T* keys, const uint64_t* key_valid, const uint64_t* mask, const P* pred, P ps, int64_t n, int64_t kmin, uint64_t range,
                                                               const uint64_t* bitmap, uint64_t* match_bits) {
   int lane = lane_id();
   int64_t base = ((int64_t)blockIdx.x * (BLOCK / WAVE) + (threadIdx.x >> 6)) * (WAVE * PM_ROWS);
-  if (base + WAVE * PM_ROWS <= n) probe_match_chunk<T, HAS_MASK, HAS_VALID, true>(keys, key_valid, mask, n, kmin, range, bitmap, match_bits, base, lane);
-  else if (base < n) probe_match_chunk<T, HAS_MASK, HAS_VALID, false>(keys, key_valid, mask, n, kmin, range, bitmap, match_bits, base, lane);
+  if (base + WAVE * PM_ROWS <= n) probe_match_chunk<T, P, OP, HAS_MASK, HAS_VALID, true>(keys, key_valid, mask, pred, ps, n, kmin, range, bitmap, match_bits, base, lane);
+  else if (base < n) probe_match_chunk<T, P, OP, HAS_MASK, HAS_VALID, false>(keys, key_valid, mask, pred, ps, n, kmin, range, bitmap, match_bits, base, lane);
 }
 __global__ void __launch_bounds__(BLOCK) k_probe_lookup(KeySet bks, KeySet pks, const uint32_t* rows, int64_t m, int null_eq, int force_zero,
                                                         const uint64_t* slots, const uint32_t* slot_count, uint64_t cap_mask, int unique,
@@ -690,7 +721,28 @@
 #undef LR
   KERNEL_CHECK();
 }
-static bool match_bits_by_bitmap(dfgpu_ctx* ctx, const dfgpu_join_table* t, const dfgpu_array* pk, int64_t n, const uint64_t* mk, uint64_t* match_bits) {
+struct ProbePred { const dfgpu_array* col = nullptr; int op = 0; int64_t scalar = 0; };
+static bool probe_pred_ok(const dfgpu_join_table* t, const dfgpu_array* pk, const ProbePred& pp) {
+  auto w48 = [](int32_t ty) { return ty == DFGPU_INT32 || ty == DFGPU_DATE32 || ty == DFGPU_INT64; };
+  return pp.col && pp.op >= DFGPU_OP_EQ && pp.op <= DFGPU_OP_GTEQ && w48(pp.col->type) && !pp.col->validity && pp.col->length == pk->length && w48(pk->type) && !pk->validity &&
+         pk->type == t->keys[0]->type && (t->bitmap || (t->lazy_row_slot && t->range <= (uint64_t)pk->length * 16));
+}
+static const void* pair_aligned(dfgpu_ctx* ctx, const dfgpu_array* a, int64_t n, BufferPtr& keep) {
+  const void* p = a->values->ptr; const size_t w = (size_t)type_width(a->type);
+  if ((uintptr_t)p % (2 * w)) { keep = alloc_buffer(ctx, (size_t)n * w); HIP_CHECK(hipMemcpyAsync(keep->ptr, p, (size_t)n * w, hipMemcpyDeviceToDevice, ctx->stream)); p = keep->ptr; }
+  return p;
+}
+template <typename T, typename P>
+static void launch_probe_fused(dfgpu_ctx* ctx, int op, dim3 grid, const T* keys, const uint64_t* mk, const P* pred, P ps, int64_t n, int64_t kmin, uint64_t range, const uint64_t* bitmap, uint64_t* match_bits) {
+  switch (op) {
+#define PF_CASE(OP) case OP: if (mk) hipLaunchKernelGGL((k_probe_match_bitmap<T, P, OP, true, false>), grid, dim3(BLOCK), 0, ctx->stream, keys, (const uint64_t*)nullptr, mk, pred, ps, n, kmin, range, bitmap, match_bits); \
+                             else hipLaunchKernelGGL((k_probe_match_bitmap<T, P, OP, false, false>), grid, dim3(BLOCK), 0, ctx->stream, keys, (const uint64_t*)nullptr, mk, pred, ps, n, kmin, range, bitmap, match_bits); break;
+    PF_CASE(DFGPU_OP_EQ) PF_CASE(DFGPU_OP_NEQ) PF_CASE(DFGPU_OP_LT) PF_CASE(DFGPU_OP_LTEQ) PF_CASE(DFGPU_OP_GT) PF_CASE(DFGPU_OP_GTEQ)
+#undef PF_CASE
+    default: fail(DFGPU_INTERNAL, "fused probe: operator %d", op);
+  }
+}
+static bool match_bits_by_bitmap(dfgpu_ctx* ctx, const dfgpu_join_table* t, const dfgpu_array* pk, int64_t n, const uint64_t* mk, uint64_t* match_bits, const ProbePred& pp = ProbePred()) {
   const dfgpu_array* key0 = t->keys[0];
   if (pk->type != key0->type) return false;
   if (t->lazy_row_slot && t->range <= (uint64_t)n * 16) {
@@ -703,12 +755,21 @@
   }
   if (!t->bitmap) return false;
   KernelTimer kt_(ctx, "k_probe_match_bitmap");
-  int64_t rows_per_block = (int64_t)BLOCK * PM_ROWS;
+  const dim3 grid(grid_for(n, BLOCK * PM_ROWS));
   const uint64_t* kvp = pk->validity ? (const uint64_t*)pk->validity->ptr : nullptr;
-  const void* kptr = pk->values->ptr; BufferPtr aligned_keys; const size_t kw = (size_t)type_width(pk->type);
-  if ((uintptr_t)kptr % (2 * kw)) { aligned_keys = alloc_buffer(ctx, (size_t)n * kw); HIP_CHECK(hipMemcpyAsync(aligned_keys->ptr, kptr, (size_t)n * kw, hipMemcpyDeviceToDevice, ctx->stream)); kptr = aligned_keys->ptr; }
-#define PM_LAUNCH(HM, HV) DFGPU_INT_KEY_DISPATCH(pk->type, hipLaunchKernelGGL((k_probe_match_bitmap<T, HM, HV>), dim3(grid_for(n, (int)rows_per_block)), dim3(BLOCK), 0, ctx->stream, (const T*)kptr, \
-                                                          kvp, mk, n, t->key_min, t->range, (const uint64_t*)t->bitmap->ptr, match_bits))
+  BufferPtr aligned_keys, aligned_pred; const void* kptr = pair_aligned(ctx, pk, n, aligned_keys);
+  const uint64_t* bm = (const uint64_t*)t->bitmap->ptr;
+  if (pp.op) {
+    const void* pptr = pair_aligned(ctx, pp.col, n, aligned_pred);
+    const bool k8 = pk->type == DFGPU_INT64, p8 = pp.col->type == DFGPU_INT64;
+    if (k8 && p8) launch_probe_fused<int64_t, int64_t>(ctx, pp.op, grid, (const int64_t*)kptr, mk, (const int64_t*)pptr, pp.scalar, n, t->key_min, t->range, bm, match_bits);
+    else if (k8) launch_probe_fused<int64_t, int32_t>(ctx, pp.op, grid, (const int64_t*)kptr, mk, (const int32_t*)pptr, (int32_t)pp.scalar, n, t->key_min, t->range, bm, match_bits);
+    else if (p8) launch_probe_fused<int32_t, int64_t>(ctx, pp.op, grid, (const int32_t*)kptr, mk, (const int64_t*)pptr, pp.scalar, n, t->key_min, t->range, bm, match_bits);
+    else launch_probe_fused<int32_t, int32_t>(ctx, pp.op, grid, (const int32_t*)kptr, mk, (const int32_t*)pptr, (int32_t)pp.scalar, n, t->key_min, t->range, bm, match_bits);
+    return true;
+  }
+#define PM_LAUNCH(HM, HV) DFGPU_INT_KEY_DISPATCH(pk->type, hipLaunchKernelGGL((k_probe_match_bitmap<T, T, 0, HM, HV>), grid, dim3(BLOCK), 0, ctx->stream, (const T*)kptr, \
+                                                          kvp, mk, (const T*)nullptr, (T)0, n, t->key_min, t->range, bm, match_bits))
   if (mk && kvp) { PM_LAUNCH(true, true); } else if (mk) { PM_LAUNCH(true, false); } else if (kvp) { PM_LAUNCH(false, true); } else { PM_LAUNCH(false, false); }
 #undef PM_LAUNCH
   return true;
@@ -810,7 +871,8 @@
 int64_t dfgpu_join_table_memory(const dfgpu_join_table* t) { return t ? t->mem : 0; }
 
 static dfgpu_status join_probe_impl(dfgpu_ctx* ctx, const dfgpu_join_table* t, const dfgpu_array* const* probe_keys, int32_t nkeys,
-                                    const dfgpu_array* opt_mask, dfgpu_array** out_build_idx, dfgpu_array** out_probe_idx, bool may_defer, dfgpu_array** out_selection);
+                                    const dfgpu_array* opt_mask, dfgpu_array** out_build_idx, dfgpu_array** out_probe_idx, bool may_defer, dfgpu_array** out_selection,
+                                    const dfgpu::ProbePred* pred = nullptr);
 dfgpu_status dfgpu_join_probe(dfgpu_ctx* ctx, const dfgpu_join_table* t, const dfgpu_array* const* probe_keys, int32_t nkeys,
                               const dfgpu_array* opt_mask, dfgpu_array** out_build_idx, dfgpu_array** out_probe_idx) {
   return join_probe_impl(ctx, t, probe_keys, nkeys, opt_mask, out_build_idx, out_probe_idx, false, nullptr);
@@ -822,6 +884,19 @@
 dfgpu_status dfgpu_join_probe_selection(dfgpu_ctx* ctx, const dfgpu_join_table* t, const dfgpu_array* const* probe_keys, int32_t nkeys, const dfgpu_array* opt_mask, dfgpu_array** out_selection) {
   if (!out_selection) return DFGPU_INVALID_ARGUMENT;
   return join_probe_impl(ctx, t, probe_keys, nkeys, opt_mask, nullptr, nullptr, false, out_selection);
+}
+dfgpu_status dfgpu_join_probe_fused(dfgpu_ctx* ctx, const dfgpu_join_table* t, const dfgpu_array* const* probe_keys, int32_t nkeys, const dfgpu_array* opt_mask,
+                                    const dfgpu_array* pred_column, int32_t pred_op, const dfgpu_array* pred_scalar, int32_t out_form,
+                                    dfgpu_array** out_build_idx, dfgpu_array** out_probe_idx, dfgpu_array** out_selection) {
+  if (!pred_column || !pred_scalar || out_form < DFGPU_PROBE_PAIRS || out_form > DFGPU_PROBE_SELECTION) return DFGPU_INVALID_ARGUMENT;
+  const bool sel = out_form == DFGPU_PROBE_SELECTION;
+  if (sel && !out_selection) return DFGPU_INVALID_ARGUMENT;
+  dfgpu::ProbePred pp; pp.col = pred_column; pp.op = pred_op;
+  const int32_t pt = pred_column->type;
+  const bool scalar_ok = pred_scalar->type == pt && pred_scalar->length == 1 && pred_scalar->has_host_scalar && pred_scalar->host_scalar_valid && (pt == DFGPU_INT32 || pt == DFGPU_DATE32 || pt == DFGPU_INT64);
+  if (scalar_ok) { if (pt == DFGPU_INT64) memcpy(&pp.scalar, pred_scalar->host_scalar, 8); else { int32_t v; memcpy(&v, pred_scalar->host_scalar, 4); pp.scalar = v; } }
+  else pp.op = 0;
+  return join_probe_impl(ctx, t, probe_keys, nkeys, opt_mask, sel ? nullptr : out_build_idx, sel ? nullptr : out_probe_idx, out_form == DFGPU_PROBE_DEFERRED, sel ? out_selection : nullptr, &pp);
 }
 dfgpu_status dfgpu_join_lookup(dfgpu_ctx* ctx, const dfgpu_join_table* t, const dfgpu_array* const* probe_keys, int32_t nkeys, const dfgpu_array* rows, dfgpu_array** out_build_idx) {
   return guard(ctx, [&] {
@@ -839,12 +914,16 @@
   });
 }
 static dfgpu_status join_probe_impl(dfgpu_ctx* ctx, const dfgpu_join_table* t, const dfgpu_array* const* probe_keys, int32_t nkeys,
-                                    const dfgpu_array* opt_mask, dfgpu_array** out_build_idx, dfgpu_array** out_probe_idx, bool may_defer, dfgpu_array** out_selection) {
+                                    const dfgpu_array* opt_mask, dfgpu_array** out_build_idx, dfgpu_array** out_probe_idx, bool may_defer, dfgpu_array** out_selection,
+                                    const dfgpu::ProbePred* pred) {
   return guard(ctx, [&] {
     if (!t || !probe_keys || (!out_selection && (!out_build_idx || !out_probe_idx))) fail(DFGPU_INVALID_ARGUMENT, "join_probe: null argument");
     check_key_types(t, probe_keys, nkeys);
     const bool lookup_ok = rank_lookup_ok(t, probe_keys, nkeys);
     if (out_selection && !lookup_ok) fail(DFGPU_NOT_IMPLEMENTED, "join_probe_selection: only a unique rank-indexed build probed by one integer key column of the build's type without NULLs");
+    if (pred && (nkeys != 1 || t->pack_n || !probe_pred_ok(t, probe_keys[0], *pred) || pj_probe_eligible(ctx, t, probe_keys, nkeys, probe_keys[0]->length)))
+      fail(DFGPU_NOT_IMPLEMENTED, "join_probe_fused: only a table with a membership bitmap probed by one Int32 / Date32 / Int64 key column without NULLs, and a predicate `column <op> scalar` "
+                                  "(op EQ..GTEQ) over an Int32 / Date32 / Int64 column without NULLs");
     ArrayHolder packed_probe; const dfgpu_array* pk1 = nullptr;
     if (t->pack_n) {
       for (int c = 0; c < nkeys; c++) if (probe_keys[c]->type == DFGPU_DICTIONARY || probe_keys[c]->length != probe_keys[0]->length) fail(DFGPU_NOT_IMPLEMENTED, "probe of a packed multi-key table with dictionary-encoded keys");
@@ -861,7 +940,7 @@
       return;
     }
     BufferPtr match_bits = alloc_buffer(ctx, bitmap_bytes(n), n == 0);
-    const bool use_bitmap = n && match_bits_by_bitmap(ctx, t, probe_keys[0], n, mk, (uint64_t*)match_bits->ptr);
+    const bool use_bitmap = n && match_bits_by_bitmap(ctx, t, probe_keys[0], n, mk, (uint64_t*)match_bits->ptr, pred ? *pred : ProbePred());
     const BufferPtr found_slot = n && !use_bitmap ? match_bits_by_hash(ctx, t, probe_keys, nkeys, pks, n, mk, (uint64_t*)match_bits->ptr) : nullptr;
     KERNEL_CHECK();
     if (out_selection) {
diff --git a/datafusion-upstream_amd/device.py b/datafusion-upstream_amd/device.py
--- a/datafusion-upstream_amd/device.py
+++ b/datafusion-upstream_amd/device.py
@@ -329,6 +329,18 @@
             return None
         self.ctx.check(st)
         return Array(self.ctx, out)
+
+    def probe_fused(self, keys: Sequence[Array], pred_column: Array, pred_op: int, pred_scalar: Array, mask: Optional[Array] = None, form: int = 0):
+        hs, n = capi.handle_array([a.h.value for a in keys])
+        ob, op, sel = C.c_void_p(), C.c_void_p(), C.c_void_p()
+        st = self.ctx.lib.dfgpu_join_probe_fused(self.ctx.h, self.h, hs, n, mask.h if mask is not None else None, pred_column.h, pred_op, pred_scalar.h, form,
+                                                 C.byref(ob), C.byref(op), C.byref(sel))
+        if st == 4:
+            return None
+        self.ctx.check(st)
+        if form == 2:
+            return Array(self.ctx, sel)
+        return (Array(self.ctx, ob) if ob.value else None), Array(self.ctx, op)
 
     def lookup(self, keys: Sequence[Array], rows: Optional[Array] = None) -> Array:
         hs, n = capi.handle_array([a.h.value for a in keys])
diff --git a/include/dfgpu.h b/include/dfgpu.h
--- a/include/dfgpu.h
+++ b/include/dfgpu.h
@@ -126,6 +126,10 @@
                                                  const dfgpu_array *opt_mask, dfgpu_array **out_build_idx, dfgpu_array **out_probe_idx);
 DFGPU_API dfgpu_status dfgpu_join_probe_selection(dfgpu_ctx *ctx, const dfgpu_join_table *table, const dfgpu_array *const *probe_keys, int32_t nkeys,
                                                   const dfgpu_array *opt_mask, dfgpu_array **out_selection);
+enum { DFGPU_PROBE_PAIRS = 0, DFGPU_PROBE_DEFERRED = 1, DFGPU_PROBE_SELECTION = 2 };
+DFGPU_API dfgpu_status dfgpu_join_probe_fused(dfgpu_ctx *ctx, const dfgpu_join_table *table, const dfgpu_array *const *probe_keys, int32_t nkeys, const dfgpu_array *opt_mask,
+                                              const dfgpu_array *pred_column, int32_t pred_op, const dfgpu_array *pred_scalar, int32_t out_form,
+                                              dfgpu_array **out_build_idx, dfgpu_array **out_probe_idx, dfgpu_array **out_selection);
 DFGPU_API dfgpu_status dfgpu_join_lookup(dfgpu_ctx *ctx, const dfgpu_join_table *table, const dfgpu_array *const *probe_keys, int32_t nkeys, const dfgpu_array *rows,
                                          dfgpu_array **out_build_idx);
 DFGPU_API dfgpu_status dfgpu_join_mark_visited(dfgpu_ctx *ctx, dfgpu_join_table *t, const dfgpu_array *build_idx);
diff --git a/shim/src/ffi.rs b/shim/src/ffi.rs
--- a/shim/src/ffi.rs
+++ b/shim/src/ffi.rs
@@ -54,6 +54,9 @@
     pub fn dfgpu_join_probe_deferred(ctx: *mut dfgpu_ctx, table: *const dfgpu_join_table, probe_keys: *const *const dfgpu_array, nkeys: i32, opt_mask: *const dfgpu_array,
                                      out_build_idx: *mut *mut dfgpu_array, out_probe_idx: *mut *mut dfgpu_array) -> i32;
     pub fn dfgpu_join_probe_selection(ctx: *mut dfgpu_ctx, table: *const dfgpu_join_table, probe_keys: *const *const dfgpu_array, nkeys: i32, opt_mask: *const dfgpu_array, out_selection: *mut *mut dfgpu_array) -> i32;
+    pub fn dfgpu_join_probe_fused(ctx: *mut dfgpu_ctx, table: *const dfgpu_join_table, probe_keys: *const *const dfgpu_array, nkeys: i32, opt_mask: *const dfgpu_array,
+                                  pred_column: *const dfgpu_array, pred_op: i32, pred_scalar: *const dfgpu_array, out_form: i32,
+                                  out_build_idx: *mut *mut dfgpu_array, out_probe_idx: *mut *mut dfgpu_array, out_selection: *mut *mut dfgpu_array) -> i32;
     pub fn dfgpu_join_lookup(ctx: *mut dfgpu_ctx, table: *const dfgpu_join_table, probe_keys: *const *const dfgpu_array, nkeys: i32, rows: *const dfgpu_array, out_build_idx: *mut *mut dfgpu_array) -> i32;
     pub fn dfgpu_plan_sort_merge_join(left: *const dfgpu_plan, right: *const dfgpu_plan, on_l: *const *const dfgpu_expr, on_r: *const *const dfgpu_expr, non: i32, filter: *const dfgpu_expr,
                                       filter_sides: *const i32, filter_indices: *const i32, nfilter_cols: i32, join_type: i32, null_equals_null: i32, out: *mut *mut dfgpu_plan) -> i32;
```
